# ekimb/rust-mdbg

Measured on AMD Instinct MI355X. Metric: Gbases/s ingested to k-min-mer graph, higher is better.
Workload: dtype u64

## Files before the change

### include/mdbg_hip.h

```cpp
#ifndef MDBG_HIP_H
#define MDBG_HIP_H

#include <stddef.h>
#include <stdint.h>

#ifdef __cplusplus
extern "C" {
#endif

#define MDBG_ABI_VERSION 3

enum {
    MDBG_OK = 0,
    MDBG_E_PARAM = -1,
    MDBG_E_ALPHABET = -2,
    MDBG_E_CAPACITY = -3,
    MDBG_E_DEVICE = -4,
    MDBG_E_NOMEM = -5,
    MDBG_E_STATE = -6,
    MDBG_E_IO = -7
};

#define MDBG_MAX_L 255u
#define MDBG_MAX_MINABUND 65535u
#define MDBG_FLAG_FORCE_GENERIC 1u
#define MDBG_FLAG_KEEP_READS 2u
#define MDBG_SCHEME_DENSITY 0u
#define MDBG_SCHEME_SYNCMERS 1u

typedef struct mdbg_ctx mdbg_ctx;

typedef struct mdbg_params {
    uint32_t k;
    uint32_t l;
    double density;
    uint32_t min_abundance;
    uint32_t reads_already_hpc;
    int32_t device;
    uint32_t flags;
    uint64_t table_capacity_hint;
    uint32_t scheme;
    uint32_t syncmer_s;
    uint64_t reserved[3];
} mdbg_params;

typedef struct mdbg_nodes {
    uint64_t n;
    uint32_t k;
    const uint64_t* keys;
    const uint32_t* index;
    const uint16_t* abundance;
    const uint32_t* seqlen;
    const uint16_t* shift;
    const uint64_t* shift_full;
    const uint64_t* src_read;
    const uint64_t* src_start;
    const uint64_t* src_end;
    const uint8_t* reversed;
    uint64_t n_distinct;
    uint64_t n_wrapped;
} mdbg_nodes;

typedef struct mdbg_stats {
    uint64_t n_reads, n_bases, n_minimizers, n_windows, n_distinct, table_capacity;
    uint64_t n_slow_tiles;
    uint64_t n_tiles;
    double ms_sketch, ms_insert, ms_finalize;
    double ms_sketch_tile;
    uint64_t n_sketch_tile_launches;
    uint64_t n_sketch_tile_bases;
    uint64_t tile_bases;
    uint64_t n_link_matches;
    uint64_t reserved[3];
} mdbg_stats;

mdbg_ctx* mdbg_create(const mdbg_params* p, int* err);
void mdbg_destroy(mdbg_ctx* ctx);

int mdbg_ingest_batch(mdbg_ctx* ctx, const uint8_t* bases, const uint64_t* offsets, uint64_t n_reads,
                      uint64_t first_read_ordinal);
int mdbg_ingest_batch_device(mdbg_ctx* ctx, const uint8_t* d_bases, const uint64_t* d_offsets, uint64_t n_reads,
                             uint64_t n_bases, uint64_t first_read_ordinal);

typedef struct mdbg_packed_batch {
    const uint64_t* words;
    const uint64_t* offsets;
    uint64_t n_reads;
    const uint64_t* exc_pos;
    const uint8_t* exc_val;
    uint64_t n_exc;
} mdbg_packed_batch;
int mdbg_ingest_batch_packed(mdbg_ctx* ctx, const mdbg_packed_batch* batch, uint64_t first_read_ordinal);
int mdbg_ingest_batch_packed_device(mdbg_ctx* ctx, const mdbg_packed_batch* batch, uint64_t n_bases, uint64_t first_read_ordinal);
int mdbg_sketch_packed_device(mdbg_ctx* ctx, const mdbg_packed_batch* batch, uint64_t n_bases, uint64_t first_read_ordinal);
int mdbg_pack_device(mdbg_ctx* ctx, const uint8_t* d_bases, uint64_t n_bases, uint64_t* d_words, uint64_t* d_exc_pos,
                     uint8_t* d_exc_val, uint64_t exc_cap, uint64_t* n_exc);

int mdbg_sketch_only(mdbg_ctx* ctx, const uint8_t* bases, const uint64_t* offsets, uint64_t n_reads,
                     const uint64_t** hashes, const uint64_t** positions, const uint64_t** per_read_offsets,
                     uint64_t* n_minimizers);

int mdbg_query_batch(mdbg_ctx* ctx, const uint8_t* bases, const uint64_t* offsets, uint64_t n_reads, const uint32_t** counts,
                     const uint64_t** per_read_offsets, uint64_t* n_windows);

int mdbg_finalize(mdbg_ctx* ctx, mdbg_nodes* out);
int mdbg_finalize_device(mdbg_ctx* ctx, mdbg_nodes* out);
int mdbg_finalize_gfa(mdbg_ctx* ctx, mdbg_nodes* out);
int mdbg_nodes_digest(mdbg_ctx* ctx, const mdbg_nodes* nodes, uint64_t* sum, uint64_t* xr);
int mdbg_reset(mdbg_ctx* ctx, uint32_t new_k);
int mdbg_set_lmer_filter(mdbg_ctx* ctx, const uint64_t* codes, uint64_t n);
int mdbg_mark(mdbg_ctx* ctx, uint64_t* mark);
int mdbg_rewind(mdbg_ctx* ctx, uint64_t mark);

int mdbg_get_stats(mdbg_ctx* ctx, mdbg_stats* out);
int mdbg_set_timing(mdbg_ctx* ctx, uint32_t level);
const char* mdbg_strerror(int err);
const char* mdbg_last_error(mdbg_ctx* ctx);
uint32_t mdbg_abi_version(void);
uint32_t mdbg_build_flags(void);
uint64_t mdbg_release_cached_memory(void);
void* mdbg_host_alloc(size_t bytes);
void mdbg_host_free(void* p);
int mdbg_host_is_pinned(const void* p);

int mdbg_sketch_device(mdbg_ctx* ctx, const uint8_t* d_bases, const uint64_t* d_offsets, uint64_t n_reads,
                       uint64_t n_bases, uint64_t first_read_ordinal);
int mdbg_insert_resident(mdbg_ctx* ctx);
int mdbg_route_pack(mdbg_ctx* ctx, uint32_t world, const uint64_t** d_records, uint64_t* counts);
int mdbg_arena_reserve(mdbg_ctx* ctx, uint64_t n_records, uint64_t** d_tail);
int mdbg_insert_records(mdbg_ctx* ctx, const uint64_t* d_records, uint64_t n_records);
typedef struct mdbg_routed_lists {
    uint64_t n_all, n_solid;
    const uint64_t* d_first; const uint8_t* d_solid;
    const uint64_t* d_ath; const uint32_t* d_count; const uint64_t* d_slot; const uint64_t* d_idx_all;
    uint64_t counts_all[64], counts_solid[64];
} mdbg_routed_lists;
int mdbg_routed_export(mdbg_ctx* ctx, uint32_t world, const uint64_t* span_lo, const uint32_t* span_rank, uint32_t n_spans,
                       mdbg_routed_lists* out);
int mdbg_resolve_first(mdbg_ctx* ctx, const uint64_t* d_ord, const uint8_t* d_solid, uint64_t n, uint64_t* d_rank_first,
                       uint64_t* d_rank_solid, uint64_t* total_first, uint64_t* total_solid);
int mdbg_resolve_meta(mdbg_ctx* ctx, const uint64_t* d_ord, uint64_t n, uint64_t* d_meta);
int mdbg_routed_keys(mdbg_ctx* ctx, const uint64_t* d_slot, uint64_t n, uint64_t* d_keys);
typedef struct mdbg_edge_list {
    uint64_t n;
    const uint32_t* n1; const uint8_t* o1; const uint32_t* n2; const uint8_t* o2; const uint32_t* overlap;
    uint64_t presimp_removed;
} mdbg_edge_list;
int mdbg_graph_edges(mdbg_ctx* ctx, float presimp, mdbg_edge_list* out);
int mdbg_graph_edges_device(mdbg_ctx* ctx, float presimp, mdbg_edge_list* out);

typedef struct mdbg_unitig_list {
    uint64_t n_unitigs, n_entries;
    const uint64_t* offsets;
    const uint32_t* node; const uint8_t* ori;
    const uint64_t* src_read; const uint64_t* src_begin; const uint32_t* len; const uint8_t* revcomp; const uint64_t* dst_offset;
    const uint64_t* length; const uint64_t* kc_sum; const uint8_t* circular;
    mdbg_edge_list edges;
    uint32_t n_rounds, reserved;
} mdbg_unitig_list;
int mdbg_graph_unitigs(mdbg_ctx* ctx, mdbg_unitig_list* out);
int mdbg_graph_unitigs_device(mdbg_ctx* ctx, mdbg_unitig_list* out);

#define MDBG_SIMPLIFY_TIPS 1u
#define MDBG_SIMPLIFY_BUBBLES 2u
typedef struct mdbg_simplify_step { uint32_t kind, max_nodes; uint64_t max_bases; } mdbg_simplify_step;
typedef struct mdbg_simplify_stats {
    uint32_t n_steps, n_compactions;
    const uint64_t* unitigs_removed; const uint64_t* nodes_removed;
    uint64_t total_unitigs_removed, total_nodes_removed;
    uint32_t n_rounds_total, n_syncs;
} mdbg_simplify_stats;
int mdbg_graph_simplify(mdbg_ctx* ctx, const mdbg_simplify_step* steps, uint32_t n_steps, mdbg_unitig_list* out, mdbg_simplify_stats* stats);
int mdbg_graph_simplify_device(mdbg_ctx* ctx, const mdbg_simplify_step* steps, uint32_t n_steps, mdbg_unitig_list* out, mdbg_simplify_stats* stats);

typedef struct mdbg_contig_seqs {
    uint64_t n_contigs, n_bases;
    const uint8_t*  bases;
    const uint64_t* offsets;
    const uint64_t* unitig;
} mdbg_contig_seqs;
int mdbg_graph_contigs(mdbg_ctx* ctx, uint64_t min_len, mdbg_contig_seqs* out);
int mdbg_graph_contigs_device(mdbg_ctx* ctx, uint64_t min_len, mdbg_contig_seqs* out);
int mdbg_kept_reads(mdbg_ctx* ctx, uint64_t* n_reads, uint64_t* n_bases, uint64_t* bytes);
int mdbg_contigs_ms(mdbg_ctx* ctx, double* ms);

int mdbg_set_partition(mdbg_ctx* ctx, uint32_t world, uint32_t rank);
typedef struct mdbg_sketch_store {
    uint64_t n_minimizers, n_reads;
    const uint64_t* d_hashes;
    const uint32_t* d_positions;
    const uint64_t* d_read_offsets;
} mdbg_sketch_store;
int mdbg_sketch_view(mdbg_ctx* ctx, mdbg_sketch_store* out);
int mdbg_ingest_sketch(mdbg_ctx* ctx, const uint64_t* d_hashes, const uint32_t* d_positions, const uint64_t* d_read_offsets,
                       uint64_t n_reads, uint64_t first_read_ordinal);
int mdbg_store_reserve(mdbg_ctx* ctx, uint64_t n_minimizers_total, uint64_t n_reads_total);
int mdbg_sketch_reserve(mdbg_ctx* ctx, uint64_t n_minimizers, uint64_t** d_hashes, uint32_t** d_positions, uint64_t* region);
int mdbg_sketch_commit(mdbg_ctx* ctx, uint64_t region, uint64_t n_minimizers, const uint64_t* d_read_offsets, uint64_t n_reads,
                       uint64_t first_read_ordinal, uint64_t owned_windows);
int mdbg_owner_counts(mdbg_ctx* ctx, uint32_t world, uint64_t* counts);
int mdbg_owner_lists(mdbg_ctx* ctx, uint32_t world, uint64_t* counts, const uint32_t** d_lists);
int mdbg_sketch_commit_listed(mdbg_ctx* ctx, uint64_t region, uint64_t n_minimizers, const uint64_t* d_read_offsets, uint64_t n_reads,
                              uint64_t first_read_ordinal, const uint32_t* d_list, uint64_t n_list);
typedef struct mdbg_batch_info {
    uint64_t store_offset, n_minimizers, first_slot, n_reads, first_read_ordinal;
    const uint64_t* d_hashes;
    const uint32_t* d_positions;
    const uint64_t* d_read_offsets;
} mdbg_batch_info;
int mdbg_last_batch(mdbg_ctx* ctx, mdbg_batch_info* out);
int mdbg_finalize_begin(mdbg_ctx* ctx, uint64_t** d_bm_first, uint64_t** d_bm_solid, uint64_t* n_words);
int mdbg_finalize_end(mdbg_ctx* ctx, mdbg_nodes* out, const uint64_t** d_row, uint64_t* n_nodes_global);

int mdbg_sync(mdbg_ctx* ctx);
int mdbg_copy_to_host(mdbg_ctx* ctx, void* dst, const void* d_src, uint64_t nbytes);
int mdbg_copy_to_device(mdbg_ctx* ctx, void* d_dst, const void* src, uint64_t nbytes);

typedef struct mdbg_synth_params {
    uint64_t seed;
    uint64_t genome_len;
    uint64_t n_reads;
    uint32_t mean_len, sd_len, min_len, max_len;
    uint32_t err_ppm;
    uint32_t reserved;
} mdbg_synth_params;
int mdbg_synth_reads_device(mdbg_ctx* ctx, const mdbg_synth_params* sp, uint64_t first_read,
// ... 9 lines not shown
```

### rust_mdbg_amd/api.py

```python
import ctypes as C
import os

import numpy as np

_HERE = os.path.dirname(os.path.abspath(__file__))
_LIB = None

MDBG_OK, MDBG_E_PARAM, MDBG_E_ALPHABET, MDBG_E_CAPACITY, MDBG_E_DEVICE, MDBG_E_NOMEM, MDBG_E_STATE, MDBG_E_IO = 0, -1, -2, -3, -4, -5, -6, -7
FLAG_FORCE_GENERIC = 1
FLAG_KEEP_READS = 2


class MdbgError(RuntimeError):
    def __init__(self, code, msg):
        super().__init__("mdbg error %d: %s" % (code, msg))
        self.code = code


class Params(C.Structure):
    _fields_ = [("k", C.c_uint32), ("l", C.c_uint32), ("density", C.c_double), ("min_abundance", C.c_uint32),
                ("reads_already_hpc", C.c_uint32), ("device", C.c_int32), ("flags", C.c_uint32),
                ("table_capacity_hint", C.c_uint64), ("scheme", C.c_uint32), ("syncmer_s", C.c_uint32), ("reserved", C.c_uint64 * 3)]


class Nodes(C.Structure):
    _fields_ = [("n", C.c_uint64), ("k", C.c_uint32), ("keys", C.POINTER(C.c_uint64)), ("index", C.POINTER(C.c_uint32)),
                ("abundance", C.POINTER(C.c_uint16)), ("seqlen", C.POINTER(C.c_uint32)), ("shift", C.POINTER(C.c_uint16)),
                ("shift_full", C.POINTER(C.c_uint64)), ("src_read", C.POINTER(C.c_uint64)), ("src_start", C.POINTER(C.c_uint64)),
                ("src_end", C.POINTER(C.c_uint64)), ("reversed", C.POINTER(C.c_uint8)), ("n_distinct", C.c_uint64),
                ("n_wrapped", C.c_uint64)]


class Stats(C.Structure):
    _fields_ = [("n_reads", C.c_uint64), ("n_bases", C.c_uint64), ("n_minimizers", C.c_uint64), ("n_windows", C.c_uint64),
                ("n_distinct", C.c_uint64), ("table_capacity", C.c_uint64), ("n_slow_tiles", C.c_uint64), ("n_tiles", C.c_uint64),
                ("ms_sketch", C.c_double), ("ms_insert", C.c_double), ("ms_finalize", C.c_double), ("ms_sketch_tile", C.c_double),
                ("n_sketch_tile_launches", C.c_uint64), ("n_sketch_tile_bases", C.c_uint64), ("tile_bases", C.c_uint64),
                ("n_link_matches", C.c_uint64), ("reserved", C.c_uint64 * 3)]


class RoutedLists(C.Structure):
    _fields_ = [("n_all", C.c_uint64), ("n_solid", C.c_uint64), ("d_first", C.c_void_p), ("d_solid", C.c_void_p), ("d_ath", C.c_void_p),
                ("d_count", C.c_void_p), ("d_slot", C.c_void_p), ("d_idx_all", C.c_void_p), ("counts_all", C.c_uint64 * 64),
                ("counts_solid", C.c_uint64 * 64)]


class SketchStore(C.Structure):
    _fields_ = [("n_minimizers", C.c_uint64), ("n_reads", C.c_uint64), ("d_hashes", C.c_void_p), ("d_positions", C.c_void_p),
                ("d_read_offsets", C.c_void_p)]


class BatchInfo(C.Structure):
    _fields_ = [("store_offset", C.c_uint64), ("n_minimizers", C.c_uint64), ("first_slot", C.c_uint64), ("n_reads", C.c_uint64),
                ("first_read_ordinal", C.c_uint64), ("d_hashes", C.c_void_p), ("d_positions", C.c_void_p), ("d_read_offsets", C.c_void_p)]


class EdgeList(C.Structure):
    _fields_ = [("n", C.c_uint64), ("n1", C.POINTER(C.c_uint32)), ("o1", C.POINTER(C.c_uint8)), ("n2", C.POINTER(C.c_uint32)),
                ("o2", C.POINTER(C.c_uint8)), ("overlap", C.POINTER(C.c_uint32)), ("presimp_removed", C.c_uint64)]


class UnitigList(C.Structure):
    _fields_ = [("n_unitigs", C.c_uint64), ("n_entries", C.c_uint64), ("offsets", C.POINTER(C.c_uint64)), ("node", C.POINTER(C.c_uint32)),
                ("ori", C.POINTER(C.c_uint8)), ("src_read", C.POINTER(C.c_uint64)), ("src_begin", C.POINTER(C.c_uint64)), ("len", C.POINTER(C.c_uint32)),
                ("revcomp", C.POINTER(C.c_uint8)), ("dst_offset", C.POINTER(C.c_uint64)), ("length", C.POINTER(C.c_uint64)),
                ("kc_sum", C.POINTER(C.c_uint64)), ("circular", C.POINTER(C.c_uint8)), ("edges", EdgeList), ("n_rounds", C.c_uint32),
                ("reserved", C.c_uint32)]


UNITIG_FIELDS = (("offsets", np.uint64), ("node", np.uint32), ("ori", np.uint8), ("src_read", np.uint64), ("src_begin", np.uint64), ("len", np.uint32),
                 ("revcomp", np.uint8), ("dst_offset", np.uint64), ("length", np.uint64), ("kc_sum", np.uint64), ("circular", np.uint8))
EDGE_FIELDS = (("n1", np.uint32), ("o1", np.uint8), ("n2", np.uint32), ("o2", np.uint8), ("overlap", np.uint32))


def unitig_counts(u):
    nu, ne = int(u.n_unitigs), int(u.n_entries)
    return dict(offsets=nu + 1 if nu else 0, node=ne, ori=ne, src_read=ne, src_begin=ne, len=ne, revcomp=ne, dst_offset=ne, length=nu, kc_sum=nu, circular=nu)


class ContigSeqs(C.Structure):
    _fields_ = [("n_contigs", C.c_uint64), ("n_bases", C.c_uint64), ("bases", C.POINTER(C.c_uint8)), ("offsets", C.POINTER(C.c_uint64)),
                ("unitig", C.POINTER(C.c_uint64))]


class SimplifyStep(C.Structure):
    _fields_ = [("kind", C.c_uint32), ("max_nodes", C.c_uint32), ("max_bases", C.c_uint64)]


class SimplifyStats(C.Structure):
    _fields_ = [("n_steps", C.c_uint32), ("n_compactions", C.c_uint32), ("unitigs_removed", C.POINTER(C.c_uint64)), ("nodes_removed", C.POINTER(C.c_uint64)),
                ("total_unitigs_removed", C.c_uint64), ("total_nodes_removed", C.c_uint64), ("n_rounds_total", C.c_uint32), ("n_syncs", C.c_uint32)]


MDBG_SIMPLIFY_TIPS, MDBG_SIMPLIFY_BUBBLES = 1, 2
_T, _B = (MDBG_SIMPLIFY_TIPS, 10, 50000), (MDBG_SIMPLIFY_BUBBLES, 0, 100000)
MAGIC_SIMPLIFY_STEPS = [_T, _T, _B, _B, _T, _B, _B, _B, _T, _B, _T, (MDBG_SIMPLIFY_BUBBLES, 0, 1000000), (MDBG_SIMPLIFY_TIPS, 10, 150000),
                        (MDBG_SIMPLIFY_BUBBLES, 0, 1000000)]


def simplify_steps(steps):
    steps = [tuple(int(x) for x in s) for s in steps]
    if not steps:
        return None, 0
    return (SimplifyStep * len(steps))(*[SimplifyStep(k, mn, mb) for k, mn, mb in steps]), len(steps)


def unitig_name(i, circular):
    return "utg%07d%s" % (i + 1, "c" if circular else "l")


class PackedBatch(C.Structure):
    _fields_ = [("words", C.c_void_p), ("offsets", C.c_void_p), ("n_reads", C.c_uint64), ("exc_pos", C.c_void_p),
                ("exc_val", C.c_void_p), ("n_exc", C.c_uint64)]


class SynthParams(C.Structure):
    _fields_ = [("seed", C.c_uint64), ("genome_len", C.c_uint64), ("n_reads", C.c_uint64), ("mean_len", C.c_uint32),
                ("sd_len", C.c_uint32), ("min_len", C.c_uint32), ("max_len", C.c_uint32), ("err_ppm", C.c_uint32),
                ("reserved", C.c_uint32)]


EXPORTS = ["mdbg_abi_version", "mdbg_build_flags", "mdbg_create", "mdbg_destroy", "mdbg_finalize_device", "mdbg_finalize_gfa", "mdbg_nodes_digest", "mdbg_set_timing", "mdbg_ingest_batch", "mdbg_ingest_batch_device", "mdbg_sketch_only",
           "mdbg_finalize", "mdbg_reset", "mdbg_get_stats", "mdbg_strerror", "mdbg_last_error", "mdbg_sketch_device",
           "mdbg_insert_resident", "mdbg_route_pack", "mdbg_insert_records", "mdbg_sync", "mdbg_synth_reads_device", "mdbg_copy_to_host", "mdbg_copy_to_device",
           "mdbg_routed_export", "mdbg_resolve_first", "mdbg_resolve_meta", "mdbg_routed_keys", "mdbg_arena_reserve",
           "mdbg_set_partition", "mdbg_sketch_view", "mdbg_ingest_sketch", "mdbg_finalize_begin", "mdbg_finalize_end",
           "mdbg_store_reserve", "mdbg_sketch_reserve", "mdbg_sketch_commit", "mdbg_last_batch", "mdbg_owner_counts", "mdbg_graph_edges", "mdbg_graph_edges_device", "mdbg_graph_unitigs", "mdbg_graph_unitigs_device",
           "mdbg_graph_simplify", "mdbg_graph_simplify_device", "mdbg_graph_contigs", "mdbg_graph_contigs_device", "mdbg_kept_reads", "mdbg_contigs_ms",
           "mdbg_ingest_batch_packed", "mdbg_ingest_batch_packed_device", "mdbg_sketch_packed_device", "mdbg_pack_device", "mdbg_query_batch", "mdbg_owner_lists", "mdbg_sketch_commit_listed", "mdbg_mark", "mdbg_rewind", "mdbg_set_lmer_filter",
           "mdbg_release_cached_memory", "mdbg_host_alloc", "mdbg_host_free", "mdbg_host_is_pinned", "mdbg_dbg_segments_ms"]


def lib_path():
    return os.path.join(_HERE, "libmdbg_hip.so")


def load_library():
    global _LIB
    if _LIB is not None:
        return _LIB
    p = lib_path()
    if not os.path.exists(p):
        raise ImportError("libmdbg_hip.so not built (%s); run `make -C rust_mdbg_amd/csrc`" % p)
    import sys
    if "torch" not in sys.modules and not os.environ.get("MDBG_NO_TORCH_PRELOAD"):
        import importlib.util
        if importlib.util.find_spec("torch") is not None:
            import torch
    L = C.CDLL(p)
    vp, u64, u32 = C.c_void_p, C.c_uint64, C.c_uint32
    L.mdbg_abi_version.restype = u32
    L.mdbg_build_flags.restype = u32
    L.mdbg_release_cached_memory.restype = u64
    L.mdbg_host_alloc.restype = vp
    L.mdbg_host_alloc.argtypes = [C.c_size_t]
    L.mdbg_host_free.restype = None
    L.mdbg_host_free.argtypes = [vp]
    L.mdbg_host_is_pinned.argtypes = [vp]
    L.mdbg_create.restype = vp
    L.mdbg_create.argtypes = [C.POINTER(Params), C.POINTER(C.c_int)]
    L.mdbg_destroy.restype = None
    L.mdbg_destroy.argtypes = [vp]
    L.mdbg_ingest_batch.argtypes = [vp, vp, vp, u64, u64]
    L.mdbg_ingest_batch_device.argtypes = [vp, vp, vp, u64, u64, u64]
    L.mdbg_sketch_device.argtypes = [vp, vp, vp, u64, u64, u64]
    L.mdbg_insert_resident.argtypes = [vp]
    L.mdbg_ingest_batch_packed.argtypes = [vp, C.POINTER(PackedBatch), u64]
    L.mdbg_ingest_batch_packed_device.argtypes = [vp, C.POINTER(PackedBatch), u64, u64]
    L.mdbg_sketch_packed_device.argtypes = [vp, C.POINTER(PackedBatch), u64, u64]
    L.mdbg_pack_device.argtypes = [vp, vp, u64, vp, vp, vp, u64, C.POINTER(u64)]
    L.mdbg_query_batch.argtypes = [vp, vp, vp, u64, C.POINTER(C.POINTER(u32)), C.POINTER(C.POINTER(u64)), C.POINTER(u64)]
    L.mdbg_query_batch.restype = C.c_int
    L.mdbg_sketch_only.argtypes = [vp, vp, vp, u64, C.POINTER(C.POINTER(u64)), C.POINTER(C.POINTER(u64)), C.POINTER(C.POINTER(u64)), C.POINTER(u64)]
    L.mdbg_finalize.argtypes = [vp, C.POINTER(Nodes)]
    L.mdbg_finalize_device.argtypes = [vp, C.POINTER(Nodes)]
    L.mdbg_finalize_gfa.argtypes = [vp, C.POINTER(Nodes)]
    L.mdbg_set_timing.argtypes = [vp, u32]
    L.mdbg_nodes_digest.argtypes = [vp, C.POINTER(Nodes), C.POINTER(C.c_uint64), C.POINTER(C.c_uint64)]
    L.mdbg_reset.argtypes = [vp, u32]
    L.mdbg_get_stats.argtypes = [vp, C.POINTER(Stats)]
    L.mdbg_strerror.restype = C.c_char_p
    L.mdbg_strerror.argtypes = [C.c_int]
    L.mdbg_last_error.restype = C.c_char_p
    L.mdbg_last_error.argtypes = [vp]
    L.mdbg_route_pack.argtypes = [vp, u32, C.POINTER(vp), C.POINTER(u64)]
    L.mdbg_routed_export.argtypes = [vp, u32, vp, vp, u32, C.POINTER(RoutedLists)]
    L.mdbg_resolve_first.argtypes = [vp, vp, vp, u64, vp, vp, C.POINTER(u64), C.POINTER(u64)]
    L.mdbg_resolve_meta.argtypes = [vp, vp, u64, vp]
    L.mdbg_routed_keys.argtypes = [vp, vp, u64, vp]
    L.mdbg_arena_reserve.argtypes = [vp, u64, C.POINTER(vp)]
    L.mdbg_set_partition.argtypes = [vp, u32, u32]
# ... 389 lines not shown
```

### rust_mdbg_amd/csrc/context.inc

```
namespace {
struct KeptReads {
    void* blk = nullptr; size_t cap = 0; void* xblk = nullptr; size_t xcap = 0;
    u64 n_reads = 0, n_bases = 0, n_words = 0, n_exc = 0;
    KeptReads() = default; KeptReads(const KeptReads&) = delete; KeptReads& operator=(const KeptReads&) = delete;
    ~KeptReads() { if (blk) mdbg_block_free(blk, cap); if (xblk) mdbg_block_free(xblk, xcap); }
    uint2* planes() const { return (uint2*)blk; }
    u64* offsets() const { return (u64*)blk + n_words; }
    u64* exc_pos() const { return (u64*)xblk; }
    u8* exc_val() const { return (u8*)xblk + n_exc * 8; }
    u64 bytes() const { return n_words * 8 + (n_reads + 1) * 8 + n_exc * 9; }
};
struct Batch { u64 first_ordinal; u32 n_reads; u32 slot0; u64 m0, m1; u64 owned = ~0ull;
               u64 list_off = ~0ull;
               bool mread_ok = true;
               u32 src_rank = ~0u;
               u64 n_bases = 0;
               bool partial = false;
               std::shared_ptr<KeptReads> kept; };

enum { SH_DISTINCT = 0, SH_OWNED, SH_OWNINS, SH_FIN_WRAPPED, SH_FIN_DISTINCT, N_SHARD_ARRAYS };
enum { SC_CARRY = 0, SC_NDISTINCT, SC_NWINDOWS, SC_FIN0, SC_FIN1, SC_FIN2, SC_SLOWCOUNT , SC_ERRFLAG , SC_CAPERR , SC_SLOWTOTAL, SC_BATCHWIN, SC_IMPORTERR, SC_PROBEERR , SC_OWNINS, SC_OVERMAX , SC_TOTFIRST, SC_TOTSOLID, SC_SLICEFAIL, SC_DONE , SC_N };

}

struct Stage { DevBuf bases, off, exc_pos, exc_val; hipStream_t st = nullptr; bool busy = false; };

struct mdbg_ctx {
    std::recursive_mutex mu;
    std::mutex err_mu;
    Stage stage[2]; std::mutex stage_mu; std::condition_variable stage_cv;
    mdbg_params P{};
    int dev = 0; hipStream_t stream = nullptr; std::string err; int poisoned = 0;
    u64 scal_seq = 0; bool batchwin_zero = false;
    u64* h_scal = nullptr;
    u64 bound = 0; DevBuf d_t4;
    DevBuf mh, mpos, mread, roff; u64 M = 0; u64 mcap = 0; u32 n_slots = 0;
    u64 slot_end_m = 0;
    u64 pending_m = 0;
    std::vector<Batch> batches; size_t batches_inserted = 0;
    u64 h_known = 0;
    DevBuf bread, tile_recs, slab, n_valid, n_scan, last_read, tile_base, scan_tmp, gran_sum, tile_flags, scalars, phase_dbg, shards;
    u32 slab_cap_min = 0;
    DevBuf tab, mx; u64 cap = 0;
    DevBuf arena, route_out, route_tmp, route_h, route_f; u64 n_records = 0; bool routed = false;
    DevBuf by_maps;
    DevBuf link_ctr;
    DevBuf claim;
    bool claims_ok = false;
    DevBuf bm_first, bm_solid, pre_first, pre_solid, popc_tmp, bt_dev, fin_out, solid_list, fin_order;
    DevBuf bm_local, pre_local, pre_local2;
    HostRaw<u64> h_keys, h_shift_full, h_src_read, h_src_start, h_src_end; HostRaw<u32> h_index, h_seqlen; HostRaw<u16> h_abund, h_shift; HostRaw<u8> h_rev;
    std::vector<u64> so_hash, so_pos, so_off;
    std::vector<u32> q_counts; std::vector<u64> q_off; DevBuf q_dev;
    DevBuf syn_bases, syn_off, syn_lens;
    u64 n_reads = 0, n_bases = 0, n_windows = 0, n_distinct = 0, n_slow_tiles = 0, n_tiles = 0;
    double ms_sketch = 0, ms_insert = 0, ms_finalize = 0;
    hipEvent_t ev0 = nullptr, ev1 = nullptr, ev3 = nullptr;
    bool fin_dirty = false;
    int timing = 2;
    std::vector<u8> bt_sent; const void* bt_sent_at = nullptr;
    u32 own_world = 1, own_rank = 0;
    int (*before_emit)(void* self, FinArgs& F, u64 n_solid) = nullptr; void* before_emit_self = nullptr;
    FinArgs finF{}; u64 fin_words = 0, fin_bits = 0; bool fin_open = false;
    u64 fin_rows_guess = 0;
    std::vector<u8> bt_host;
    EdgeBuffers* eb = nullptr;
    DevBuf own_hist;
    DevBuf own_lists; u64 own_lists_n = 0;
    DevBuf listed_multi; std::vector<ListedBatch> listed_multi_host;
    DevBuf own_thr; u32 thr_world = 0, thr_k = 0; double thr_bound = 0;
    DevBuf ol_cnt, ol_off, ol_tot, ol_list, ol_owner;
    DevBuf lmer_set; u64 lmer_mask = 0; bool lmer_on = false; u32 lmer_all_ones = 0;
    DevBuf w_jstar, w_count, w_ctr, w_start, w_fill, w_occ, w_sorted, w_ath;
    u64 nodes_n = 0; bool nodes_ok = false;
    HostRaw<u32> he_n1, he_n2, he_ov; HostRaw<u8> he_o1, he_o2;
    EdgeResult last_edges{}; bool edges_ok = false;
    UnitigBuffers* ub = nullptr;
    HostRaw<u64> hu_off, hu_sread, hu_sbegin, hu_dst, hu_length, hu_kc; HostRaw<u32> hu_node, hu_len, hu_n1, hu_n2, hu_ov; HostRaw<u8> hu_ori, hu_rc, hu_circ, hu_o1, hu_o2;
    std::vector<u64> hs_unitigs, hs_nodes;
    UnitigResult last_ul{}; bool ulist_ok = false;
    ContigBuffers* cb = nullptr;
    DevBuf kp_exc_pos, kp_exc_val, kp_cnt;
    HostRaw<u8> hc_bases; HostRaw<u64> hc_off, hc_unitig;
    double ms_stitch = 0;
    std::vector<hipEvent_t> tile_ev; size_t tile_ev_used = 0; double ms_tile = 0; u64 n_tile_launches = 0, n_tile_bases = 0;
};

namespace {

int fail(mdbg_ctx* c, int code, const char* what, hipError_t e = hipSuccess) {
    char buf[512];
    if (e != hipSuccess) { snprintf(buf, sizeof buf, "%s: %s", what, hipGetErrorString(e)); (void)hipGetLastError(); }
    else snprintf(buf, sizeof buf, "%s", what);
    if (c) { std::lock_guard<std::mutex> g_(c->err_mu); c->err = buf; if (code == MDBG_E_DEVICE || code == MDBG_E_ALPHABET || code == MDBG_E_NOMEM) c->poisoned = code; }
    return code;
}
#define MDBG_LOCK(c) std::lock_guard<std::recursive_mutex> lock_((c)->mu)
#define HIPCHK(c, call) do { hipError_t e_ = (call); if (e_ != hipSuccess) return fail((c), e_ == hipErrorOutOfMemory ? MDBG_E_NOMEM : MDBG_E_DEVICE, #call, e_); } while (0)
template <class T> int copy_out(mdbg_ctx* c, HostRaw<T>& h, const T* dev, size_t n, const char* what, const T** host) {
    if (!h.resize(n)) return fail(c, MDBG_E_NOMEM, what);
    if (n) { const hipError_t e = hipMemcpy(h.data(), dev, n * sizeof(T), hipMemcpyDeviceToHost); if (e != hipSuccess) return fail(c, e == hipErrorOutOfMemory ? MDBG_E_NOMEM : MDBG_E_DEVICE, what, e); }
    *host = h.data();
    return MDBG_OK;
}

u64* scal(mdbg_ctx* c) { return c->scalars.as<u64>(); }
int read_scalars(mdbg_ctx* c, u64* host, bool with_fin = false, bool zero_batchwin = false) {
    if (!c->h_scal) { HIPCHK(c, hipHostMalloc((void**)&c->h_scal, (SC_N + 1) * 8, hipHostMallocMapped)); c->h_scal[SC_N] = 0; }
    const u64 seq = ++c->scal_seq;
    PublishArgs pa{};
    pa.shards[0] = c->shards.as<u64>() + SH_DISTINCT * CTR_SHARDS; pa.idx[0] = SC_NDISTINCT; pa.n_arrays = 1;
    pa.zero_mask = 0; pa.zero_arrays = 0;
    if (with_fin) {
        pa.shards[1] = c->shards.as<u64>() + SH_FIN_WRAPPED * CTR_SHARDS; pa.idx[1] = SC_FIN1; pa.shards[2] = c->shards.as<u64>() + SH_FIN_DISTINCT * CTR_SHARDS; pa.idx[2] = SC_FIN2; pa.n_arrays = 3;
        pa.zero_mask = (1ull << SC_FIN0) | (1ull << SC_FIN1) | (1ull << SC_FIN2); pa.zero_arrays = 0x6u;
    }
    pa.scalars = scal(c); pa.n = SC_N; pa.host = c->h_scal; pa.seq = seq; pa.zero_idx = zero_batchwin ? (u32)SC_BATCHWIN : (u32)SC_N;
    c->batchwin_zero = zero_batchwin;
    launch_publish_scalars(pa, c->stream);
    volatile u64* const flag = c->h_scal + SC_N;
    bool seen = false;
    const double t0 = now_ms();
    for (u32 spins = 0; !seen; ++spins) {
        seen = __atomic_load_n(flag, __ATOMIC_ACQUIRE) == seq;
        if (seen) break;
#if defined(__x86_64__)
        __builtin_ia32_pause();
#endif
        if ((spins & 0x3FFu) != 0x3FFu) continue;
        const double waited = now_ms() - t0;
        if (waited > 0.3) std::this_thread::yield();
        if (waited > 20.0) break;
        if ((spins & 0xFFFFu) == 0xFFFFu) { const hipError_t q = hipStreamQuery(c->stream); if (q != hipErrorNotReady) break; }
    }
    if (!seen) HIPCHK(c, hipStreamSynchronize(c->stream));
    memcpy(host, c->h_scal, SC_N * 8);
    if (with_fin) c->fin_dirty = false;
    return MDBG_OK;
}
int write_scalar(mdbg_ctx* c, int idx, u64 v) {
    HIPCHK(c, hipMemcpyAsync((u64*)c->scalars.p + idx, &v, 8, hipMemcpyHostToDevice, c->stream));
    HIPCHK(c, hipStreamSynchronize(c->stream));
    return MDBG_OK;
}

enum ResultsFrom { FROM_NODES, FROM_EDGES, FROM_UNITIGS };
void invalidate_results(mdbg_ctx* c, ResultsFrom from) { if (from <= FROM_NODES) c->nodes_ok = false; if (from <= FROM_EDGES) c->edges_ok = false; c->ulist_ok = false; }
static void fill_mread_of(mdbg_ctx* c, Batch& b);
double owner_hash_bound(const mdbg_ctx* c) {
    double b;
    if (c->P.scheme == MDBG_SCHEME_SYNCMERS) { b = c->P.density * ldexp(1.0, 2 * (int)c->P.l); if (b >= 18446744073709551616.0) b = 18446744073709551615.0; }
    else b = (double)c->bound;
    return b >= 1.0 ? b : 0.0;
}
const u64* owner_thr(mdbg_ctx* c, u32 world) {
    if (world <= 1) return nullptr;
    const double b = owner_hash_bound(c);
    if (!(b >= 1.0)) return nullptr;
    if (c->thr_world != world || c->thr_k != c->P.k || c->thr_bound != b) {
        if (c->own_thr.ensure((size_t)OWNER_PARAM_WORDS * 8, 0, c->stream) != hipSuccess) return nullptr;
        launch_owner_thresholds(b, c->P.k, world, c->own_thr.as<u64>(), c->stream);
        c->thr_world = world; c->thr_k = c->P.k; c->thr_bound = b;
    }
    return c->own_thr.as<u64>();
}
u64 owner_bin_mul(const mdbg_ctx* c) {
    const double b = owner_hash_bound(c);
    if (!(b >= (double)OWNER_BINS * 4.0)) return 0;
    u64 bi = b >= 18446744073709549568.0 ? ~0ull : (u64)b;
    const unsigned __int128 q = ((unsigned __int128)OWNER_BINS << 64) / ((unsigned __int128)bi + 1);
    return q > (unsigned __int128)~0ull ? 0 : (u64)q;
}
int owner_hist_batch(mdbg_ctx* c, size_t which, u64* d_hist) {
    const u64 mul = owner_bin_mul(c);
    if (!mul || c->batches.empty()) return MDBG_OK;
    Batch& b = which == ~(size_t)0 ? c->batches.back() : c->batches[which];
    fill_mread_of(c, b);
    launch_owner_bins(c->mh.as<u64>(), c->mread.as<u32>(), c->roff.as<u64>(), b.m0, b.m1, c->P.k, mul, d_hist, c->stream);
    return MDBG_OK;
}
int owner_set_table(mdbg_ctx* c, u32 world, const u8* tab) {
    const u64 mul = owner_bin_mul(c);
    if (!mul || !owner_thr(c, world)) return MDBG_OK;
    HIPCHK(c, hipMemcpyAsync(c->own_thr.as<u64>() + OWNER_TAB_AT, tab, OWNER_BINS, hipMemcpyHostToDevice, c->stream));
    HIPCHK(c, hipMemcpyAsync(c->own_thr.as<u64>(), &mul, 8, hipMemcpyHostToDevice, c->stream));
    HIPCHK(c, hipStreamSynchronize(c->stream));
    return MDBG_OK;
}
TableArgs table_args(mdbg_ctx* c) {
    TableArgs T;
    T.tab = c->tab.as<Slot>(); T.cap = c->cap; T.mx = c->mx.as<u64>(); T.A = cascade_of(c->P.min_abundance);
    T.n_distinct = c->shards.as<u64>() + SH_DISTINCT * CTR_SHARDS;
    T.ks.mh = c->mh.as<u64>(); T.ks.arena = c->arena.as<u64>(); T.ks.k = c->P.k;
    T.own_world = c->own_world; T.own_rank = c->own_rank; T.own_thr = owner_thr(c, c->own_world);
    T.probe_err = (u32*)(scal(c) + SC_PROBEERR); T.own_inserted = c->shards.as<u64>() + SH_OWNINS * CTR_SHARDS;
    T.claim = (!c->routed && c->claims_ok) ? c->claim.as<u8>() : nullptr;
    static const bool no_chain = getenv("MDBG_NO_CHAIN") != nullptr;
    T.no_chain = no_chain ? 1u : 0u;
    static const bool weak_fp = getenv("MDBG_WEAK_FP") != nullptr;
    T.fp_mask = weak_fp ? 0x3ull : 0x3FFFFFFFull;
    static const bool count_links = getenv("MDBG_COUNT_LINKS") != nullptr;
    T.link_ctr = nullptr;
    if (count_links) {
        if (!c->link_ctr.p && c->link_ctr.ensure(8, 0, c->stream) == hipSuccess) (void)hipMemsetAsync(c->link_ctr.p, 0, 8, c->stream);
        T.link_ctr = (unsigned long long*)c->link_ctr.p;
    }
    return T;
}

u64 slots_for(u64 n) { return n + n / 2 + 1024; }

int table_reserve(mdbg_ctx* c, u64 incoming) {
    u64 need = slots_for(c->n_distinct + incoming);
    const u32 A = cascade_of(c->P.min_abundance);
    if (c->cap == 0) {
        u64 want = need;
        if (c->P.table_capacity_hint) want = std::max(want, slots_for(c->P.table_capacity_hint));
        HIPCHK(c, c->tab.ensure(want * sizeof(Slot), 0, c->stream));
        if (A > 2) HIPCHK(c, c->mx.ensure(want * (A - 2) * 8, 0, c->stream));
        c->cap = want;
        launch_clear_table(c->tab.as<Slot>(), c->cap, c->mx.as<u64>(), A > 2 ? c->cap * (A - 2) : 0, c->stream);
        c->claims_ok = !c->routed && c->claim.p != nullptr;
        return MDBG_OK;
    }
    if (need <= c->cap) return MDBG_OK;
    need = std::max(need, 2 * c->cap);
    DevBuf ntab, nmx;
    HIPCHK(c, ntab.ensure(need * sizeof(Slot), 0, c->stream));
    if (A > 2) HIPCHK(c, nmx.ensure(need * (A - 2) * 8, 0, c->stream));
    launch_clear_table(ntab.as<Slot>(), need, nmx.as<u64>(), A > 2 ? need * (A - 2) : 0, c->stream);
    TableArgs T = table_args(c);
    T.tab = ntab.as<Slot>(); T.cap = need; T.mx = nmx.as<u64>();
    launch_rehash(c->tab.as<Slot>(), c->cap, c->mx.as<u64>(), T, c->stream);
    HIPCHK(c, hipStreamSynchronize(c->stream));
    std::swap(c->tab.p, ntab.p); std::swap(c->tab.cap, ntab.cap);
    std::swap(c->mx.p, nmx.p); std::swap(c->mx.cap, nmx.cap);
    c->cap = need;
    return MDBG_OK;
}

int clear_table(mdbg_ctx* c) {
    invalidate_results(c, FROM_NODES);
    ZeroList z{};
    z.p[0] = c->shards.as<u64>() + SH_DISTINCT * CTR_SHARDS; z.n[0] = CTR_SHARDS; z.p[1] = scal(c) + SC_NDISTINCT; z.n[1] = 2;
    z.p[2] = scal(c) + SC_IMPORTERR; z.n[2] = 1; z.p[3] = scal(c) + SC_PROBEERR; z.n[3] = 1;
    if (c->cap) launch_clear_table(c->tab.as<Slot>(), c->cap, c->mx.as<u64>(), cascade_of(c->P.min_abundance) > 2 ? c->cap * (cascade_of(c->P.min_abundance) - 2) : 0, c->stream, &z);
    else launch_zero_regions(z, c->stream);
    c->n_distinct = 0; c->n_windows = 0; c->batches_inserted = 0; c->n_records = 0; c->routed = false;
    c->claims_ok = c->claim.p != nullptr;
    return MDBG_OK;
}

#define STAGE_EVENT(c, ev, s) do { if ((c)->timing >= 2) HIPCHK((c), hipEventRecord((ev), (s))); } while (0)
hipEvent_t next_tile_event(mdbg_ctx* c) {
    if (c->timing < 1) return nullptr;
    if (c->tile_ev_used == c->tile_ev.size()) { hipEvent_t e = nullptr; if (hipEventCreate(&e) != hipSuccess) return nullptr; c->tile_ev.push_back(e); }
    return c->tile_ev[c->tile_ev_used++];
}
void collect_tile_events(mdbg_ctx* c) {
    for (size_t i = 0; i + 1 < c->tile_ev_used; i += 2) {
        float ms = 0;
        if (hipEventElapsedTime(&ms, c->tile_ev[i], c->tile_ev[i + 1]) == hipSuccess) c->ms_tile += ms;
        else (void)hipGetLastError();
    }
    c->tile_ev_used = 0;
}
float ev_ms(mdbg_ctx* c) {
    float ms = 0;
    if (c->timing < 2) return 0.0f;
    (void)hipEventSynchronize(c->ev1);
    if (hipEventElapsedTime(&ms, c->ev0, c->ev1) != hipSuccess) { (void)hipGetLastError(); ms = 0; }
    return ms;
}

int check_params(const mdbg_params* p) {
    if (!p) return MDBG_E_PARAM;
    if (p->k < 2 || p->k > 4096) return MDBG_E_PARAM;
    if (p->l < 2 || p->l > MDBG_MAX_L) return MDBG_E_PARAM;
    if (p->min_abundance < 1 || p->min_abundance > MDBG_MAX_MINABUND) return MDBG_E_PARAM;
    if (!(p->density == p->density)) return MDBG_E_PARAM;
    if (p->scheme > MDBG_SCHEME_SYNCMERS) return MDBG_E_PARAM;
    if (p->scheme == MDBG_SCHEME_SYNCMERS && (p->l > 31 || p->syncmer_s > 16 || p->syncmer_s > p->l || p->l - p->syncmer_s + 1 > 32)) return MDBG_E_PARAM;
    return MDBG_OK;
}
}

extern "C" {
uint32_t mdbg_abi_version(void) { return MDBG_ABI_VERSION; }
uint32_t mdbg_build_flags(void) { return 0; }

const char* mdbg_strerror(int err) {
    switch (err) {
        case MDBG_OK: return "ok";
        case MDBG_E_PARAM: return "invalid parameter";
        case MDBG_E_ALPHABET: return "Non-ACGTN nucleotide encountered";
        case MDBG_E_CAPACITY: return "capacity limit exceeded";
        case MDBG_E_DEVICE: return "HIP device error";
        case MDBG_E_NOMEM: return "out of memory";
        case MDBG_E_STATE: return "invalid state for this call";
        case MDBG_E_IO: return "file could not be opened or written";
        default: return "unknown error";
    }
}
const char* mdbg_last_error(mdbg_ctx* ctx) { return ctx ? ctx->err.c_str() : ""; }

mdbg_ctx* mdbg_create(const mdbg_params* p, int* err) {
    int e = check_params(p);
    if (e) { if (err) *err = e; return nullptr; }
    int ndev = 0;
    if (hipGetDeviceCount(&ndev) != hipSuccess || ndev == 0) { if (err) *err = MDBG_E_DEVICE; return nullptr; }
    mdbg_ctx* c = new mdbg_ctx();
    c->P = *p;
    auto bail = [&](int code) -> mdbg_ctx* { if (err) *err = code; mdbg_destroy(c); return nullptr; };
    if (p->device >= 0) { if (hipSetDevice(p->device) != hipSuccess) return bail(MDBG_E_DEVICE); c->dev = p->device; }
    else if (hipGetDevice(&c->dev) != hipSuccess) return bail(MDBG_E_DEVICE);
    if (hipStreamCreateWithFlags(&c->stream, hipStreamNonBlocking) != hipSuccess) return bail(MDBG_E_DEVICE);
    for (auto& g : c->stage) if (hipStreamCreateWithFlags(&g.st, hipStreamNonBlocking) != hipSuccess) return bail(MDBG_E_DEVICE);
    if (hipEventCreate(&c->ev0) != hipSuccess || hipEventCreate(&c->ev1) != hipSuccess) return bail(MDBG_E_DEVICE);
    c->bound = make_hash_bound(p->density);
    if (c->d_t4.ensure((2 << (2 * BS_GS)) * 8, 0, c->stream) != hipSuccess) return bail(MDBG_E_NOMEM);
    { u64 t4[2 << (2 * BS_GS)]; bs_make_table<BS_GS>(t4); if (hipMemcpy(c->d_t4.p, t4, sizeof t4, hipMemcpyHostToDevice) != hipSuccess) return bail(MDBG_E_DEVICE); }
    if (c->scalars.ensure(SC_N * 8, 0, c->stream) != hipSuccess) return bail(MDBG_E_NOMEM);
    if (c->shards.ensure(N_SHARD_ARRAYS * CTR_SHARDS * 8, 0, c->stream) != hipSuccess) return bail(MDBG_E_NOMEM);
    if (hipMemset(c->shards.p, 0, N_SHARD_ARRAYS * CTR_SHARDS * 8) != hipSuccess) return bail(MDBG_E_DEVICE);
    if (hipMemset(c->scalars.p, 0, SC_N * 8) != hipSuccess) return bail(MDBG_E_DEVICE);
    if (c->roff.ensure(1024, 0, c->stream) != hipSuccess) return bail(MDBG_E_NOMEM);
    if (hipMemset(c->roff.p, 0, 8) != hipSuccess) return bail(MDBG_E_DEVICE);
    if (err) *err = MDBG_OK;
    return c;
}

void mdbg_destroy(mdbg_ctx* c) {
    if (!c) return;
    (void)hipSetDevice(c->dev);
    if (c->stream) (void)hipStreamSynchronize(c->stream);
    if (c->ev3) (void)hipEventDestroy(c->ev3);
    if (c->ev0) (void)hipEventDestroy(c->ev0);
    if (c->ev1) (void)hipEventDestroy(c->ev1);
    for (auto e : c->tile_ev) (void)hipEventDestroy(e);
    if (c->eb) edge_buffers_destroy(c->eb);
    if (c->ub) unitig_buffers_destroy(c->ub);
    if (c->cb) contig_buffers_destroy(c->cb);
    if (c->h_scal) (void)hipHostFree(c->h_scal);
    for (auto& g : c->stage) if (g.st) (void)hipStreamDestroy(g.st);
    if (c->stream) (void)hipStreamDestroy(c->stream);
    delete c;
}

int mdbg_sync(mdbg_ctx* c) {
    if (!c) return MDBG_E_PARAM;
    MDBG_LOCK(c);
    HIPCHK(c, hipStreamSynchronize(c->stream));
    return MDBG_OK;
}

int mdbg_copy_to_host(mdbg_ctx* c, void* dst, const void* d_src, uint64_t nbytes) {
    if (!c || (nbytes && (!dst || !d_src))) return MDBG_E_PARAM;
    MDBG_LOCK(c);
    (void)hipSetDevice(c->dev);
    HIPCHK(c, hipStreamSynchronize(c->stream));
    if (nbytes) HIPCHK(c, hipMemcpy(dst, d_src, nbytes, hipMemcpyDeviceToHost));
    return MDBG_OK;
}
int mdbg_copy_to_device(mdbg_ctx* c, void* d_dst, const void* src, uint64_t nbytes) {
    if (!c || (nbytes && (!d_dst || !src))) return MDBG_E_PARAM;
    MDBG_LOCK(c);
    (void)hipSetDevice(c->dev);
    if (nbytes) HIPCHK(c, hipMemcpy(d_dst, src, nbytes, hipMemcpyHostToDevice));
    return MDBG_OK;
}
}
```

### rust_mdbg_amd/csrc/ingest_api.inc

```
namespace {
constexpr u64 SLAB_BUDGET = 6ull << 30;
int insert_resident_impl(mdbg_ctx* c, bool allow_pending = false);
int sketch_device_impl(mdbg_ctx* c, const SketchInput& in, const u64* d_offsets, u64 n_reads, u64 n_bases, u64 first_ordinal, bool then_insert = false, bool* inserted = nullptr) {
    if (inserted) *inserted = false;
    if (c->poisoned) return fail(c, MDBG_E_STATE, "context is in an error state");
    if (n_reads == 0) return MDBG_OK;
    if (in.fmt == FMT_ASCII && !in.d_bases && n_bases) return fail(c, MDBG_E_PARAM, "null bases");
    if (in.fmt == FMT_PLANES && !in.d_planes && n_bases) return fail(c, MDBG_E_PARAM, "null packed words");
    if (!d_offsets) return fail(c, MDBG_E_PARAM, "null offsets");
    if ((((uintptr_t)in.d_bases) | ((uintptr_t)in.d_planes)) & 15) return fail(c, MDBG_E_PARAM, "device bases pointer must be 16-byte aligned");
    if (in.n_exc && (!in.d_exc_pos || !in.d_exc_val)) return fail(c, MDBG_E_PARAM, "null exception list");
    if (in.n_exc >= 0xFFFFFFF0ull) return fail(c, MDBG_E_CAPACITY, "too many exceptions");
    if (n_reads >= 0xFFFFFFF0ull || (u64)c->n_slots + n_reads >= 0xFFFFFFF0ull) return fail(c, MDBG_E_CAPACITY, "too many reads");
    if (first_ordinal + n_reads >= (1ull << (64 - WIN_BITS))) return fail(c, MDBG_E_CAPACITY, "read ordinal too large");
    hipStream_t s = c->stream;
    const bool sync = c->P.scheme == MDBG_SCHEME_SYNCMERS;
    const u64 tile_bases = TILE_STRIDE;
    const u64 n_tiles_total = (n_bases + tile_bases - 1) / tile_bases;
    if (n_tiles_total >= 0x7FFFFFF0ull) return fail(c, MDBG_E_CAPACITY, "batch too large for one call");
    u32 slot0 = 0;
    { int e = next_slot0(c, c->M, n_reads, &slot0); if (e) return e; }
    double dens2 = 2.0 * c->P.density; if (dens2 > 1.0) dens2 = 1.0; if (dens2 < 0) dens2 = 0;
    u32 slab_cap = 0, gather_tiles = 1;
    {
        const double per_base = sync ? std::min(1.0, std::max(0.0, c->P.density)) / (c->P.syncmer_s ? std::max(1.0, (double)(c->P.l - c->P.syncmer_s + 1) / 2.0) : 1.0) : dens2;
        const double e = (double)tile_bases * per_base; double v = e * 1.25 + 6.0 * sqrt(e) + 32.0; if (v > (double)tile_bases) v = (double)tile_bases; slab_cap = ((u32)v + 7u) & ~7u;
        if (e < 128.0) gather_tiles = (u32)std::max(1.0, std::min(16.0, 256.0 / std::max(e, 1.0)));
    }
    if (slab_cap < c->slab_cap_min) slab_cap = c->slab_cap_min;
    static const u32 cap0_hook = getenv("MDBG_SLAB_CAP0") ? (u32)atoi(getenv("MDBG_SLAB_CAP0")) : 0u;
    static const u64 budget_hook = getenv("MDBG_SLAB_BUDGET_MB") ? (u64)atoll(getenv("MDBG_SLAB_BUDGET_MB")) << 20 : 0ull;
    if (cap0_hook && !c->slab_cap_min) slab_cap = std::max<u32>(8u, cap0_hook & ~7u);
    if (slab_cap > (u32)tile_bases) slab_cap = (u32)tile_bases;
    if (n_tiles_total) {
        HIPCHK(c, c->bread.ensure((n_tiles_total + 2) * 4, 0, s));
        HIPCHK(c, c->tile_recs.ensure(n_tiles_total * sizeof(TileRec), 0, s));
        HIPCHK(c, c->n_valid.ensure(n_tiles_total * 4, 0, s));
        HIPCHK(c, c->n_scan.ensure(n_tiles_total * 4, 0, s));
        HIPCHK(c, c->last_read.ensure(n_tiles_total * 4, 0, s));
        if (in.n_exc) HIPCHK(c, c->tile_flags.ensure(n_tiles_total, 0, s));
    }
    u64 want = c->M + (u64)((double)n_bases * dens2 * 1.15) + 65536;
    const bool phase_dbg = getenv("MDBG_PHASE_TIMING") != nullptr;
    for (int attempt = 0; attempt < 4; ++attempt) {
        { int e = store_ensure(c, want); if (e) return e; }
        const u64 chunk = std::max<u64>(1, std::min<u64>(n_tiles_total ? n_tiles_total : 1, (budget_hook ? budget_hook : SLAB_BUDGET) / ((u64)slab_cap * sizeof(Rec))));
        std::vector<u64> part_end;
        for (u64 t0 = 0; t0 < n_tiles_total; t0 += chunk) part_end.push_back(std::min<u64>(n_tiles_total, t0 + chunk));
        u64 max_part = 0; { u64 t0 = 0; for (u64 e : part_end) { max_part = std::max(max_part, e - t0); t0 = e; } }
        if (n_tiles_total) {
            HIPCHK(c, c->slab.ensure((size_t)chunk * slab_cap * sizeof(Rec), 0, s));
            HIPCHK(c, c->tile_base.ensure((size_t)max_part * 8, 0, s));
            HIPCHK(c, c->scan_tmp.ensure(((size_t)max_part / 1024 + 2) * 8, 0, s));
        }
        u64 init[1] = {c->M};
        STAGE_EVENT(c, c->ev0, s);
        SketchInit init0{};
        init0.zero[0] = scal(c) + SC_ERRFLAG; init0.zero[1] = scal(c) + SC_SLOWTOTAL; init0.zero[2] = scal(c) + SC_OVERMAX; init0.set_p = scal(c) + SC_CARRY; init0.set_v = c->M;
        const bool fused = then_insert && inserted && n_tiles_total && part_end.size() == 1 && !phase_dbg && c->cap && c->own_world <= 1 && !c->lmer_on && !c->routed && !c->pending_m &&
                           c->batches_inserted == c->batches.size() && c->mcap > c->M && c->mcap - c->M <= 2 * (want - c->M) + (1u << 20) &&
                           want - c->M <= (48ull << 20);
        if (fused) init0.zero[3] = scal(c) + SC_BATCHWIN;
        if (!n_tiles_total) {
            ZeroList z{};
            z.p[0] = init0.zero[0]; z.n[0] = 1; z.p[1] = init0.zero[1]; z.n[1] = 1; z.p[2] = init0.zero[2]; z.n[2] = 1; z.set_p = init0.set_p; z.set_v = init0.set_v;
            launch_zero_regions(z, s);
            launch_fill_u64(c->roff.as<u64>() + slot0, n_reads + 1, c->M, s);
        }
        SketchArgs A{};
        A.bases = in.d_bases; A.planes = in.d_planes; A.fmt = in.fmt; A.n_bases = n_bases; A.offsets = d_offsets; A.n_reads = (u32)n_reads;
        A.exc_pos = in.d_exc_pos; A.exc_val = in.d_exc_val; A.n_exc = (u32)in.n_exc;
        A.l = c->P.l; A.hpc = c->P.reads_already_hpc == 0 ? 1u : 0u;
        if (n_tiles_total) {
            A.bread = c->bread.as<u32>(); A.recs = c->tile_recs.as<TileRec>(); A.n_tiles = (u32)n_tiles_total;
            A.slab = c->slab.as<Rec>(); A.slab_cap = slab_cap; A.n_valid = c->n_valid.as<u32>(); A.n_scan = c->n_scan.as<u32>(); A.last_read = c->last_read.as<u32>(); A.over_max = (u32*)(scal(c) + SC_OVERMAX);
            A.t4 = c->d_t4.as<u64>();
            A.tile_flags = in.n_exc ? c->tile_flags.as<u8>() : nullptr;
            A.err_flag = (u32*)(scal(c) + SC_ERRFLAG); A.slow_total = (unsigned long long*)(scal(c) + SC_SLOWTOTAL);
            A.read_base = slot0; A.bound = c->bound; A.btop = (u32)(c->bound >> (64 - BS_B)); A.force_slow = ((c->P.flags & 1u) || c->P.l > (u32)BS_MAX_L) ? 1u : 0u;
            A.dbg = nullptr;
            { const char* sp = getenv("MDBG_STOP_PHASE"); A.stop_phase = sp ? (u32)atoi(sp) : 0u; }
            if (phase_dbg) { HIPCHK(c, c->phase_dbg.ensure((size_t)n_tiles_total * 128, 0, s)); HIPCHK(c, hipMemsetAsync(c->phase_dbg.p, 0, (size_t)n_tiles_total * 128, s)); A.dbg = c->phase_dbg.as<u64>(); }
            const u32 n_gran = (u32)((max_part + SCAN_GRAN - 1) / SCAN_GRAN);
            HIPCHK(c, c->gran_sum.ensure((size_t)n_gran * 8 + 64, 0, s));
            A.block_sum = (unsigned long long*)c->gran_sum.as<u64>();
            init0.zero_arr = c->gran_sum.as<u64>(); init0.zero_arr_n = n_gran;
            launch_bread(d_offsets, (u32)n_reads, n_bases, A.n_tiles, c->bread.as<u32>(), c->tile_recs.as<TileRec>(), init0, s);
            if (in.n_exc) {
                HIPCHK(c, hipMemsetAsync(c->tile_flags.p, 0, n_tiles_total, s));
                launch_tile_flags(in.d_exc_pos, (u32)in.n_exc, A.n_tiles, c->tile_flags.as<u8>(), s);
            }
            if (sync) {
                A.scheme = 1; A.s = c->P.syncmer_s; A.btop = 0;
                const double v = c->P.density * (double)(1ull << (2 * c->P.l));
                A.bound = !(v > 0.0) ? 0 : (v >= 18446744073709551616.0 ? ~0ull : (u64)v);
                A.force_slow = ((c->P.flags & 1u) || c->P.syncmer_s > 13) ? 1u : 0u;
            }
            u64 t0 = 0;
            for (size_t pi = 0; pi < part_end.size(); ++pi) {
                const u32 nt = (u32)(part_end[pi] - t0);
                Rec* const part_slab = c->slab.as<Rec>();
                A.tile0 = (u32)t0; A.slab = part_slab;
                if (pi) HIPCHK(c, hipMemsetAsync(c->gran_sum.p, 0, (size_t)n_gran * 8, s));
                { hipEvent_t tb = next_tile_event(c), te = next_tile_event(c); launch_sketch(A, nt, s, tb, te); }
                GatherArgs G{};
                G.tile0 = (u32)t0; G.n = nt; G.slab = part_slab; G.slab_cap = slab_cap; G.n_valid = A.n_valid; G.n_scan = A.n_scan; G.last_read = A.last_read;
                G.out_hash = c->mh.as<u64>(); G.out_pos = c->mpos.as<u32>(); G.out_read = c->mread.as<u32>(); G.out_cap = c->mcap;
                G.m0 = c->M; G.slot0 = slot0; G.n_reads = (u32)n_reads; G.off = c->roff.as<u64>(); G.last_launch = pi + 1 == part_end.size() ? 1u : 0u;
                G.tiles_per_wave = gather_tiles;
                launch_gather(G, c->scan_tmp.as<u64>(), c->tile_base.as<u64>(), scal(c) + SC_CARRY, s, c->gran_sum.as<u64>());
                c->n_tile_launches += 1;
                t0 = part_end[pi];
            }
            c->n_tile_bases += n_bases;
            if (phase_dbg) {
                std::vector<u64> h((size_t)A.n_tiles * 16);
                (void)hipStreamSynchronize(s);
                (void)hipMemcpy(h.data(), A.dbg, h.size() * 8, hipMemcpyDeviceToHost);
                double ph[7] = {0, 0, 0, 0, 0, 0, 0}, nc = 0, nv = 0; u64 nfast = 0;
                for (u32 t = 0; t < A.n_tiles; ++t) {
                    const u64* q = &h[(size_t)t * 16];
                    if (!q[7]) continue;
                    ++nfast;
                    ph[0] += (double)(q[1] - q[0]); ph[1] += (double)(q[2] - q[1]); ph[2] += (double)(q[3] - q[2]); ph[3] += (double)(q[4] - q[3]);
                    ph[4] += (double)(q[5] - q[4]); ph[5] += (double)(q[7] - q[5]);
                    nc += (double)q[9]; nv += (double)q[10];
                }
                const double n = nfast ? (double)nfast : 1.0;
                fprintf(stderr, "[mdbg phase timing] tiles=%u fast=%llu avg cycles: load=%.0f compact=%.0f hash=%.0f exact=%.0f rank=%.0f write=%.0f ; candidates=%.1f valid=%.1f slab_cap=%u\n",
                        A.n_tiles, (unsigned long long)nfast, ph[0] / n, ph[1] / n, ph[2] / n, ph[3] / n, ph[4] / n, ph[5] / n, nc / n, nv / n, slab_cap);
            }
        }
        STAGE_EVENT(c, c->ev1, s);
        u32* const ins_flags = (u32*)(scal(c) + SC_CAPERR);
        if (fused) {
            launch_count_reserve(c->roff.as<u64>(), slot0, (u32)n_reads, c->P.k, scal(c) + SC_BATCHWIN, (u32*)(scal(c) + SC_DONE), c->shards.as<u64>() + SH_DISTINCT * CTR_SHARDS, scal(c) + SC_NDISTINCT,
                                 c->cap, ins_flags + 1, scal(c) + SC_CARRY, c->mcap, (const u32*)(scal(c) + SC_OVERMAX), s);
            if (!c->ev3) HIPCHK(c, hipEventCreate(&c->ev3));
            launch_insert_windows(table_args(c), c->mh.as<u64>(), c->mread.as<u32>(), c->roff.as<u64>(), c->M, c->mcap, slot0, first_ordinal, scal(c) + SC_NWINDOWS, ins_flags, s, scal(c) + SC_CARRY);
            STAGE_EVENT(c, c->ev3, s);
        }
        u64 sc[SC_N];
        int e = read_scalars(c, sc, false, true); if (e) return e;
        c->ms_sketch += ev_ms(c);
        collect_tile_events(c);
        u64 m_new = sc[SC_CARRY];
        const u32 over = (u32)sc[SC_OVERMAX];
        if (over || m_new > c->mcap) {
            if (over) { slab_cap = std::min<u32>((u32)tile_bases, (over + over / 8 + 15u) & ~7u); c->slab_cap_min = slab_cap; }
            if (m_new > c->mcap) want = m_new + 65536;
            c->n_tile_launches -= part_end.size(); c->n_tile_bases -= n_tiles_total ? n_bases : 0;
            continue;
        }
        if (m_new >= 0xFFFFFFF0ull) return fail(c, MDBG_E_CAPACITY, "more than 2^32 minimizers resident on one device");
        if ((u32)sc[SC_ERRFLAG]) {
            u64 which = ~0ull;
            HIPCHK(c, hipMemcpyAsync(scal(c) + SC_SLOWTOTAL, &which, 8, hipMemcpyHostToDevice, s));
            launch_alphabet_rule(A, (unsigned long long*)(scal(c) + SC_SLOWTOTAL), s);
            HIPCHK(c, hipMemcpyAsync(&which, scal(c) + SC_SLOWTOTAL, 8, hipMemcpyDeviceToHost, s));
            HIPCHK(c, hipStreamSynchronize(s));
            if (which != ~0ull) {
                char buf[160]; snprintf(buf, sizeof buf, "Non-ACGTN nucleotide in read %llu of the batch (ordinal %llu)", (unsigned long long)which, (unsigned long long)(first_ordinal + which));
                return fail(c, MDBG_E_ALPHABET, buf);
            }
        }
        const u64 slow_total = sc[SC_SLOWTOTAL];
        if (c->lmer_on && m_new > c->M) {
            const u32 nb = lmer_filter_blocks(m_new - c->M);
            HIPCHK(c, c->slab.ensure((size_t)nb * 256 * sizeof(Rec), 0, s));
            HIPCHK(c, c->n_valid.ensure((size_t)nb * 4, 0, s)); HIPCHK(c, c->tile_base.ensure((size_t)nb * 8, 0, s)); HIPCHK(c, c->scan_tmp.ensure(((size_t)nb / 1024 + 2) * 8, 0, s));
            LmerFilterArgs L{};
            L.set = c->lmer_set.as<u64>(); L.set_mask = c->lmer_mask; L.has_all_ones = c->lmer_all_ones;
            L.mh = c->mh.as<u64>(); L.mpos = c->mpos.as<u32>(); L.mread = c->mread.as<u32>(); L.m0 = c->M; L.m1 = m_new;
            L.offsets = d_offsets; L.slot0 = slot0; L.l = c->P.l; L.hpc = c->P.reads_already_hpc == 0 ? 1u : 0u;
            L.slab = c->slab.as<Rec>(); L.n_valid = c->n_valid.as<u32>();
            launch_lmer_filter(L, in.fmt, in.d_bases, in.d_planes, in.d_exc_pos, in.d_exc_val, (u32)in.n_exc, s);
            HIPCHK(c, hipMemcpyAsync(scal(c) + SC_CARRY, init, 8, hipMemcpyHostToDevice, s));
            GatherArgs G{};
            G.tile0 = 0; G.n = nb; G.slab = L.slab; G.slab_cap = 256; G.n_valid = L.n_valid;
            G.out_hash = c->mh.as<u64>(); G.out_pos = c->mpos.as<u32>(); G.out_read = c->mread.as<u32>(); G.out_cap = c->mcap;
            G.m0 = c->M; G.slot0 = slot0; G.n_reads = (u32)n_reads; G.off = c->roff.as<u64>(); G.last_launch = 1; G.tiles_per_wave = 1;
            launch_gather(G, c->scan_tmp.as<u64>(), c->tile_base.as<u64>(), scal(c) + SC_CARRY, s);
            int e2 = read_scalars(c, sc); if (e2) return e2;
            m_new = sc[SC_CARRY];
        }
        Batch b; b.first_ordinal = first_ordinal; b.n_reads = (u32)n_reads; b.slot0 = slot0; b.m0 = c->M; b.m1 = m_new; b.n_bases = n_bases;
        invalidate_results(c, FROM_UNITIGS);
        if (c->P.flags & MDBG_FLAG_KEEP_READS) { int ke = keep_batch(c, in, d_offsets, n_reads, n_bases, b.kept); if (ke) return ke; }
        store_append(c, b);
        c->n_reads += n_reads; c->n_bases += n_bases; c->n_tiles += n_tiles_total; c->n_slow_tiles += slow_total;
        if (fused) {
            invalidate_results(c, FROM_NODES);
            if (sc[SC_CAPERR] >> 32) return MDBG_OK;
            c->batches_inserted = c->batches.size();
            *inserted = true;
            if ((u32)sc[SC_PROBEERR]) return fail(c, MDBG_E_PARAM, "the table filled up during insertion");
            float ms = 0;
            if (c->timing >= 2) { if (hipEventElapsedTime(&ms, c->ev1, c->ev3) == hipSuccess) c->ms_insert += ms; else (void)hipGetLastError(); }
            c->n_windows += sc[SC_BATCHWIN];
            c->n_distinct = sc[SC_NDISTINCT];
            if (sc[SC_IMPORTERR]) return fail(c, MDBG_E_PARAM, "read offsets of an imported sketch are not consistent with its size");
            if ((u32)sc[SC_CAPERR]) return fail(c, MDBG_E_CAPACITY, "a read has more than 2^26 minimizers");
        }
        return MDBG_OK;
    }
    return fail(c, MDBG_E_CAPACITY, "minimizer store could not be sized");
}
int sketch_device_impl(mdbg_ctx* c, const u8* d_bases, const u64* d_offsets, u64 n_reads, u64 n_bases, u64 first_ordinal, bool then_insert = false, bool* inserted = nullptr) {
    SketchInput in; in.fmt = FMT_ASCII; in.d_bases = d_bases;
    return sketch_device_impl(c, in, d_offsets, n_reads, n_bases, first_ordinal, then_insert, inserted);
}

int insert_resident_impl(mdbg_ctx* c, bool allow_pending) {
    if (c->poisoned) return fail(c, MDBG_E_STATE, "context is in an error state");
    if (c->routed) return fail(c, MDBG_E_STATE, "table holds routed records; local insertion is not allowed");
    if (c->pending_m && !allow_pending) return fail(c, MDBG_E_STATE, "reserved sketch regions have not been committed");
    hipStream_t s = c->stream;
    const size_t first = c->batches_inserted, last = c->batches.size();
    invalidate_results(c, FROM_NODES);
    bool any = false;
    for (size_t i = first; i < last; ++i) any = any || c->batches[i].m1 > c->batches[i].m0;
    c->batches_inserted = last;
    if (!any) return MDBG_OK;
    u64 sc[SC_N];
    bool counts_known = c->own_world > 1;
    u64 known = 0;
    for (size_t i = first; i < last; ++i) { const Batch& b = c->batches[i]; if (b.m1 == b.m0) continue; if (b.owned == ~0ull) counts_known = false; else known += b.owned; }
    for (size_t i = first; i < last; ++i) {
        Batch& b = c->batches[i];
        if (!counts_known || !(b.list_off != ~0ull && b.owned != ~0ull && c->own_world > 1)) fill_mread_of(c, b);
    }
    if (counts_known) {
        c->h_known = known;
        HIPCHK(c, hipMemcpyAsync(scal(c) + SC_BATCHWIN, &c->h_known, 8, hipMemcpyHostToDevice, s));
        HIPCHK(c, hipMemsetAsync(c->shards.as<u64>() + SH_OWNINS * CTR_SHARDS, 0, CTR_SHARDS * 8, s));
    } else {
        if (!c->batchwin_zero) HIPCHK(c, hipMemsetAsync(scal(c) + SC_BATCHWIN, 0, 8, s));
        if (c->own_world > 1) HIPCHK(c, hipMemsetAsync(c->shards.as<u64>() + SH_OWNED * CTR_SHARDS, 0, 2 * CTR_SHARDS * 8, s));
        for (size_t i = first; i < last; ++i) {
            const Batch& b = c->batches[i];
            if (b.m1 == b.m0) continue;
            if (c->own_world > 1)
                launch_count_owned_windows(c->mh.as<u64>(), c->mread.as<u32>(), c->roff.as<u64>(), b.m0, b.m1, c->P.k, c->own_world, owner_thr(c, c->own_world), c->own_rank,
                                           c->shards.as<u64>() + SH_OWNED * CTR_SHARDS, s);
            else launch_count_windows(c->roff.as<u64>(), b.slot0, b.n_reads, c->P.k, scal(c) + SC_BATCHWIN, s);
        }
        if (c->own_world > 1) launch_sum_shards(c->shards.as<u64>() + SH_OWNED * CTR_SHARDS, 1, scal(c) + SC_BATCHWIN, s);
    }
    c->batchwin_zero = false;
    int e;
    u32* const flags = (u32*)(scal(c) + SC_CAPERR);
    u64 total_idx = 0;
    for (size_t i = first; i < last; ++i) total_idx += c->batches[i].m1 - c->batches[i].m0;
    u64 slice = 32ull << 20;
    { const char* sv = getenv("MDBG_INSERT_SLICE"); if (sv) { const u64 v = strtoull(sv, nullptr, 10); if (v) slice = std::max<u64>(v, (u64)OWN_SPAN); } }
    slice = (slice + OWN_SPAN - 1) / OWN_SPAN * OWN_SPAN;
    if (c->own_world <= 1 && total_idx > 2 * slice) {
        struct Sl { size_t b; u64 a, hi; };
        std::vector<Sl> sl;
        for (size_t i = first; i < last; ++i) { const Batch& b = c->batches[i]; for (u64 a = b.m0; a < b.m1; a += slice) sl.push_back({i, a, std::min(a + slice, b.m1)}); }
        if (c->cap < slots_for(c->n_distinct + slice)) { e = table_reserve(c, slice); if (e) return e; }
        size_t next = 0;
        for (;;) {
            { ZeroList z{}; z.p[0] = scal(c) + SC_CAPERR; z.n[0] = 0; z.set_p = scal(c) + SC_SLICEFAIL; z.set_v = ~0ull; launch_zero_regions(z, s); }
            HIPCHK(c, hipMemsetAsync(flags + 1, 0, 4, s));
            STAGE_EVENT(c, c->ev0, s);
            for (size_t j = next; j < sl.size(); ++j) {
                const Batch& b = c->batches[sl[j].b];
                launch_slice_check(c->shards.as<u64>(), scal(c) + SC_NDISTINCT, sl[j].hi - sl[j].a, c->cap, flags + 1, scal(c) + SC_SLICEFAIL, (u64)j, s);
                launch_insert_windows(table_args(c), c->mh.as<u64>(), c->mread.as<u32>(), c->roff.as<u64>(), sl[j].a, b.m1, b.slot0, b.first_ordinal,
                                      scal(c) + SC_NWINDOWS, flags, s, nullptr, sl[j].hi - sl[j].a);
            }
            STAGE_EVENT(c, c->ev1, s);
            e = read_scalars(c, sc); if (e) return e;
            c->ms_insert += ev_ms(c);
            c->n_distinct = sc[SC_NDISTINCT];
            if (!(sc[SC_CAPERR] >> 32)) break;
            if (sc[SC_SLICEFAIL] >= sl.size() || sc[SC_SLICEFAIL] < next) return fail(c, MDBG_E_DEVICE, "slice bookkeeping of the insertion is inconsistent");
            next = (size_t)sc[SC_SLICEFAIL];
            e = table_reserve(c, slice); if (e) return e;
        }
        if ((u32)sc[SC_PROBEERR]) return fail(c, MDBG_E_PARAM, "the table filled up during insertion");
        c->n_windows += sc[SC_BATCHWIN];
        if (sc[SC_IMPORTERR]) return fail(c, MDBG_E_PARAM, "read offsets of an imported sketch are not consistent with its size");
        if ((u32)sc[SC_CAPERR]) return fail(c, MDBG_E_CAPACITY, "a read has more than 2^26 minimizers");
        return MDBG_OK;
    }
    if (c->cap == 0) {
        e = read_scalars(c, sc); if (e) return e;
        c->n_distinct = sc[SC_NDISTINCT];
        if (sc[SC_IMPORTERR]) return fail(c, MDBG_E_PARAM, "read offsets of an imported sketch are not consistent with its size");
        if (!sc[SC_BATCHWIN]) {
            if (c->claim.p) for (size_t i = first; i < last; ++i) { const Batch& b = c->batches[i]; if (b.m1 > b.m0) HIPCHK(c, hipMemsetAsync(c->claim.as<u8>() + b.m0, 0, b.m1 - b.m0, s)); }
            return MDBG_OK;
        }
        e = table_reserve(c, sc[SC_BATCHWIN]); if (e) return e;
    }
    for (;;) {
        launch_reserve_check(c->shards.as<u64>(), scal(c) + SC_NDISTINCT, scal(c) + SC_BATCHWIN, c->cap, flags + 1, s);
        STAGE_EVENT(c, c->ev0, s);
        auto list_of = [&](const Batch& b) { return c->own_lists.as<u32>() + b.list_off; };
        auto seg_of = [&](const Batch& b) { return c->own_lists.as<u32>() + b.list_off + 2 * b.owned; };
        auto per_entry = [&](const Batch& b) { return listed_per_entry(table_args(c), b.m0, b.m1, b.owned, seg_of(b) != nullptr); };
        std::vector<ListedBatch> multi; u64 multi_total = 0;
        for (size_t i = first; i < last; ++i) {
            const Batch& b = c->batches[i];
            if (b.list_off != ~0ull && b.owned != ~0ull && b.owned && c->own_world > 1 && per_entry(b)) {
                ListedBatch lb{}; lb.start = multi_total; lb.m0 = b.m0; lb.m1 = b.m1; lb.first_ordinal = b.first_ordinal; lb.list = list_of(b);
                lb.slot0 = b.slot0; lb.n_reads = b.n_reads;
                multi.push_back(lb); multi_total += b.owned;
            }
        }
        if (multi.size() < 2) { multi.clear(); multi_total = 0; }
        if (c->claims_ok && c->claim.p && c->own_world > 1)
            for (size_t i = first; i < last; ++i) {
                const Batch& b = c->batches[i];
                if (b.list_off != ~0ull && b.owned != ~0ull && b.m1 > b.m0 && (!b.owned || per_entry(b)))
                    HIPCHK(c, hipMemsetAsync(c->claim.as<u8>() + b.m0, 0, b.m1 - b.m0, s));
            }
        if (!multi.empty()) {
            ListedBatch end{}; end.start = multi_total; multi.push_back(end);
            HIPCHK(c, c->listed_multi.ensure(multi.size() * sizeof(ListedBatch), 0, s));
            c->listed_multi_host = multi;
            HIPCHK(c, hipMemcpyAsync(c->listed_multi.p, c->listed_multi_host.data(), multi.size() * sizeof(ListedBatch), hipMemcpyHostToDevice, s));
            launch_insert_listed_multi(table_args(c), c->mh.as<u64>(), c->mread.as<u32>(), c->roff.as<u64>(), c->listed_multi.as<ListedBatch>(), (u32)multi.size() - 1, multi_total, flags, s);
        }
        for (size_t i = first; i < last; ++i) {
            const Batch& b = c->batches[i];
            if (multi_total && b.list_off != ~0ull && b.owned != ~0ull && b.owned && c->own_world > 1 && per_entry(b)) continue;
            if (b.list_off != ~0ull && b.owned != ~0ull && c->own_world > 1)
                launch_insert_listed(table_args(c), c->mh.as<u64>(), c->mread.as<u32>(), c->roff.as<u64>(), b.m0, b.m1, list_of(b), seg_of(b), b.owned, b.slot0, b.n_reads, b.first_ordinal, flags, s);
            else
                launch_insert_windows(table_args(c), c->mh.as<u64>(), c->mread.as<u32>(), c->roff.as<u64>(), b.m0, b.m1, b.slot0, b.first_ordinal,
                                      scal(c) + SC_NWINDOWS, flags, s);
        }
        STAGE_EVENT(c, c->ev1, s);
        if (c->own_world > 1) launch_sum_shards(c->shards.as<u64>() + SH_OWNINS * CTR_SHARDS, 1, scal(c) + SC_OWNINS, s);
        e = read_scalars(c, sc); if (e) return e;
        if (!(sc[SC_CAPERR] >> 32)) break;
// ... 174 lines not shown
    if (!c) return MDBG_E_PARAM;
    u64 nb = 0;
    StageHold hold;
    if (n_reads) { int e = stage_host_batch(c, bases, offsets, n_reads, &nb, hold); if (e) return e; }
    MDBG_LOCK(c);
    (void)hipSetDevice(c->dev);
    if (c->poisoned) return fail(c, MDBG_E_STATE, "context is in an error state");
    c->so_hash.clear(); c->so_pos.clear(); c->so_off.assign(n_reads + 1, 0);
    if (n_reads) {
        const StoreRollback tmp(c); const u64 M0 = tmp.s.M;
        const int e = sketch_device_impl(c, hold.g->bases.as<u8>(), hold.g->off.as<u64>(), n_reads, nb, 0);
        if (e) { if (e == MDBG_E_ALPHABET) c->poisoned = 0; return e; }
        const u64 m = c->M - M0;
        c->so_hash.resize(m); std::vector<u32> p32(m);
        bool ok = hipStreamSynchronize(c->stream) == hipSuccess;
        if (ok && m) ok = hipMemcpy(c->so_hash.data(), c->mh.as<u64>() + M0, m * 8, hipMemcpyDeviceToHost) == hipSuccess &&
                          hipMemcpy(p32.data(), c->mpos.as<u32>() + M0, m * 4, hipMemcpyDeviceToHost) == hipSuccess;
        if (ok) ok = hipMemcpy(c->so_off.data(), c->roff.as<u64>() + c->batches.back().slot0, (n_reads + 1) * 8, hipMemcpyDeviceToHost) == hipSuccess;
        if (!ok) return fail(c, MDBG_E_DEVICE, "sketch_only: copy to the host");
        c->so_pos.resize(m);
        for (u64 i = 0; i < m; ++i) c->so_pos[i] = p32[i];
        for (auto& o : c->so_off) o -= M0;
    }
    if (hashes) *hashes = c->so_hash.data();
    if (positions) *positions = c->so_pos.data();
    if (per_read_offsets) *per_read_offsets = c->so_off.data();
    if (n_minimizers) *n_minimizers = c->so_hash.size();
    return MDBG_OK;
}

int mdbg_query_batch(mdbg_ctx* c, const uint8_t* bases, const uint64_t* offsets, uint64_t n_reads, const uint32_t** counts,
                     const uint64_t** per_read_offsets, uint64_t* n_windows) {
    if (!c) return MDBG_E_PARAM;
    u64 nb = 0;
    StageHold hold;
    if (n_reads) { int e = stage_host_batch(c, bases, offsets, n_reads, &nb, hold); if (e) return e; }
    MDBG_LOCK(c);
    (void)hipSetDevice(c->dev);
    if (c->poisoned) return fail(c, MDBG_E_STATE, "context is in an error state");
    if (c->routed) return fail(c, MDBG_E_STATE, "not available for a routed table");
    if (c->own_world > 1) return fail(c, MDBG_E_STATE, "not available for a partitioned table: k-min-mers owned by other ranks would read as absent");
    c->q_counts.clear(); c->q_off.assign(n_reads + 1, 0);
    if (n_reads) {
        const StoreRollback tmp(c); const u64 M0 = tmp.s.M;
        const int e = sketch_device_impl(c, hold.g->bases.as<u8>(), hold.g->off.as<u64>(), n_reads, nb, 0);
        if (e) { if (e == MDBG_E_ALPHABET) c->poisoned = 0; return e; }
        const Batch b = c->batches.back();
        const u64 m = b.m1 - b.m0;
        hipStream_t s = c->stream;
        std::vector<u32> per_min(m);
        std::vector<u64> roffs(n_reads + 1);
        if (m) {
            if (c->q_dev.ensure(m * 4, 0, s) != hipSuccess) return fail(c, MDBG_E_NOMEM, "query buffer");
            launch_query_windows(table_args(c), c->P.min_abundance, c->mh.as<u64>(), c->mread.as<u32>(), c->roff.as<u64>(), b.m0, b.m1, c->q_dev.as<u32>(), s);
            if (hipMemcpyAsync(per_min.data(), c->q_dev.p, m * 4, hipMemcpyDeviceToHost, s) != hipSuccess) return fail(c, MDBG_E_DEVICE, "copy");
        }
        if (hipMemcpyAsync(roffs.data(), c->roff.as<u64>() + b.slot0, (n_reads + 1) * 8, hipMemcpyDeviceToHost, s) != hipSuccess ||
            hipStreamSynchronize(s) != hipSuccess) return fail(c, MDBG_E_DEVICE, "copy");
        const u64 k = c->P.k;
        for (u64 r = 0; r < n_reads; ++r) {
            const u64 rs = roffs[r] - M0, re = roffs[r + 1] - M0;
            if (re - rs > k) for (u64 i = rs; i + k <= re; ++i) c->q_counts.push_back(per_min[i]);
            c->q_off[r + 1] = c->q_counts.size();
        }
    }
    if (counts) *counts = c->q_counts.data();
    if (per_read_offsets) *per_read_offsets = c->q_off.data();
    if (n_windows) *n_windows = c->q_counts.size();
    return MDBG_OK;
}

int mdbg_reset(mdbg_ctx* c, uint32_t new_k) {
    if (!c) return MDBG_E_PARAM;
    MDBG_LOCK(c);
    (void)hipSetDevice(c->dev);
    if (c->poisoned == MDBG_E_DEVICE) return fail(c, MDBG_E_STATE, "context is in an error state");
    if (new_k != 0 && new_k != c->P.k) for (const Batch& b : c->batches) if (b.partial)
        return fail(c, MDBG_E_STATE, "a resident foreign sketch holds only the hashes of this k's windows (mdbg_dist segments): ingest again, or exchange whole sketches (mdbg_dist_set_exchange)");
    c->poisoned = 0;
    int e = clear_table(c); if (e) return e;
    c->ms_sketch = c->ms_insert = c->ms_finalize = 0; c->ms_tile = 0; c->n_tile_launches = 0; c->n_tile_bases = 0;
    if (c->link_ctr.p) (void)hipMemsetAsync(c->link_ctr.p, 0, 8, c->stream);
    if (new_k == 0) { store_truncate(c, 0); c->n_tiles = c->n_slow_tiles = 0; return MDBG_OK; }
    if (new_k < 2 || new_k > 4096) return fail(c, MDBG_E_PARAM, "bad k");
    if (new_k != c->P.k) for (Batch& b : c->batches) { b.owned = ~0ull; b.list_off = ~0ull; }
    c->P.k = new_k;
    return insert_resident_impl(c);
}

int mdbg_set_lmer_filter(mdbg_ctx* c, const uint64_t* codes, uint64_t n) {
    if (!c || (n && !codes)) return MDBG_E_PARAM;
    MDBG_LOCK(c);
    (void)hipSetDevice(c->dev);
    if (c->poisoned) return fail(c, MDBG_E_STATE, "context is in an error state");
    if (!c->batches.empty()) return fail(c, MDBG_E_STATE, "set the l-mer filter before the first batch (or after mdbg_reset(ctx, 0))");
    if (!codes) { c->lmer_on = false; return MDBG_OK; }
    if (c->P.scheme != MDBG_SCHEME_DENSITY) return fail(c, MDBG_E_PARAM, "the l-mer filter belongs to the density scheme (src/read.rs:200-205)");
    if (c->P.l > 32) return fail(c, MDBG_E_PARAM, "the l-mer filter needs l <= 32");
    if (n >= (1ull << 40)) return fail(c, MDBG_E_CAPACITY, "l-mer set too large");
    u64 cap = 1024; while (cap < 2 * n + 2) cap <<= 1;
    std::vector<u64> tab(cap, LMERSET_EMPTY);
    const u64 mask = cap - 1, code_mask = c->P.l == 32 ? ~0ull : ((1ull << (2 * c->P.l)) - 1);
    u32 all_ones = 0;
    for (u64 i = 0; i < n; ++i) {
        const u64 code = codes[i];
        if (code & ~code_mask) return fail(c, MDBG_E_PARAM, "an l-mer code has bits above 2*l");
        if (code == LMERSET_EMPTY) { all_ones = 1; continue; }
        for (u64 h = lmerset_home(code, mask);; h = (h + 1) & mask) { if (tab[h] == code) break; if (tab[h] == LMERSET_EMPTY) { tab[h] = code; break; } }
    }
    HIPCHK(c, c->lmer_set.ensure(cap * 8, 0, c->stream));
    HIPCHK(c, hipMemcpyAsync(c->lmer_set.p, tab.data(), cap * 8, hipMemcpyHostToDevice, c->stream));
    HIPCHK(c, hipStreamSynchronize(c->stream));
    c->lmer_mask = mask; c->lmer_all_ones = all_ones; c->lmer_on = true;
    return MDBG_OK;
}

int mdbg_mark(mdbg_ctx* c, uint64_t* mark) {
    if (!c || !mark) return MDBG_E_PARAM;
    MDBG_LOCK(c);
    if (c->pending_m) return fail(c, MDBG_E_STATE, "reserved sketch regions have not been committed");
    *mark = c->batches.size();
    return MDBG_OK;
}

int mdbg_rewind(mdbg_ctx* c, uint64_t mark) {
    if (!c) return MDBG_E_PARAM;
    MDBG_LOCK(c);
    (void)hipSetDevice(c->dev);
    if (c->poisoned == MDBG_E_DEVICE) return fail(c, MDBG_E_STATE, "context is in an error state");
    if (c->pending_m) return fail(c, MDBG_E_STATE, "reserved sketch regions have not been committed");
    if (mark > c->batches.size()) return fail(c, MDBG_E_PARAM, "not a mark of this context");
    c->poisoned = 0;
    int e = clear_table(c); if (e) return e;
    store_truncate(c, (size_t)mark);
    return MDBG_OK;
}

int mdbg_set_timing(mdbg_ctx* c, uint32_t level) {
    if (!c || level > 2) return MDBG_E_PARAM;
    MDBG_LOCK(c);
    c->timing = (int)level;
    return MDBG_OK;
}

int mdbg_get_stats(mdbg_ctx* c, mdbg_stats* o) {
    if (!c || !o) return MDBG_E_PARAM;
    MDBG_LOCK(c);
    memset(o, 0, sizeof *o);
    o->n_reads = c->n_reads; o->n_bases = c->n_bases; o->n_minimizers = c->M; o->n_windows = c->n_windows; o->n_distinct = c->n_distinct;
    o->table_capacity = c->cap; o->n_slow_tiles = c->n_slow_tiles; o->n_tiles = c->n_tiles;
    o->ms_sketch = c->ms_sketch; o->ms_insert = c->ms_insert; o->ms_finalize = c->ms_finalize;
    o->ms_sketch_tile = c->ms_tile; o->n_sketch_tile_launches = c->n_tile_launches; o->n_sketch_tile_bases = c->n_tile_bases;
    o->tile_bases = TILE_STRIDE;
    if (c->link_ctr.p) {
        (void)hipSetDevice(c->dev);
        HIPCHK(c, hipStreamSynchronize(c->stream));
        HIPCHK(c, hipMemcpy(&o->n_link_matches, c->link_ctr.p, 8, hipMemcpyDeviceToHost));
    }
    return MDBG_OK;
}

int mdbg_synth_reads_device(mdbg_ctx* c, const mdbg_synth_params* sp, uint64_t first_read, const uint8_t** d_bases, const uint64_t** d_offsets, uint64_t* n_bases) {
    if (!c || !sp) return MDBG_E_PARAM;
    MDBG_LOCK(c);
    (void)hipSetDevice(c->dev);
    if (sp->n_reads == 0 || sp->n_reads > 0x7FFFFFFFull || sp->genome_len == 0 || sp->min_len == 0 || sp->min_len > sp->max_len) return fail(c, MDBG_E_PARAM, "bad synth parameters");
    SynthP P; P.seed = sp->seed; P.genome_len = sp->genome_len; P.first_read = first_read; P.mean_len = sp->mean_len; P.sd_len = sp->sd_len;
    P.min_len = sp->min_len; P.max_len = sp->max_len; P.thr24 = (u32)(((u64)sp->err_ppm << 24) / 1000000ull);
    hipStream_t s = c->stream;
    HIPCHK(c, c->syn_lens.ensure(sp->n_reads * 8, 0, s));
    HIPCHK(c, c->syn_off.ensure((sp->n_reads + 1) * 8, 0, s));
    launch_synth(P, sp->n_reads, c->syn_lens.as<u64>(), c->syn_off.as<u64>(), nullptr, 0, s);
    u64 nb = 0;
    HIPCHK(c, hipMemcpyAsync(&nb, c->syn_off.as<u64>() + sp->n_reads, 8, hipMemcpyDeviceToHost, s));
    HIPCHK(c, hipStreamSynchronize(s));
    HIPCHK(c, c->syn_bases.ensure(nb + 64, 0, s));
    launch_synth(P, sp->n_reads, c->syn_lens.as<u64>(), c->syn_off.as<u64>(), c->syn_bases.as<u8>(), 1, s);
    HIPCHK(c, hipStreamSynchronize(s));
    if (d_bases) *d_bases = c->syn_bases.as<u8>();
    if (d_offsets) *d_offsets = c->syn_off.as<u64>();
    if (n_bases) *n_bases = nb;
    return MDBG_OK;
}
}
```

### rust_mdbg_amd/csrc/sketch.hip

```cpp
#include "mdbg_dev.h"
#include "bs_core.h"

enum { FMT_ASCII = 0, FMT_PLANES = 1 };
constexpr int SCAN_GRAN_LOG = 6, SCAN_GRAN = 1 << SCAN_GRAN_LOG;
struct TileRec;

struct SketchArgs {
    const u8* bases;
    const uint2* planes;
    u32 fmt;
    u64 n_bases;
    const u64* offsets; u32 n_reads;
    const u32* bread;
    const TileRec* recs;
    u32 n_tiles;
    u32 tile0, tile_end;
    Rec* slab; u32 slab_cap;
    u32* n_valid;
    u32* n_scan;
    u32* last_read;
    u32* over_max;
    unsigned long long* block_sum;
    const u64* t4;
    const u8* tile_flags;
    const u64* exc_pos; const u8* exc_val; u32 n_exc;
    u32* err_flag; unsigned long long* slow_total;
    u32 read_base;
    u64 bound; u32 l; u32 hpc; u32 btop;
    u32 scheme, s;
    u32 force_slow;
    u64* dbg;
    u32 stop_phase;
};

__device__ inline u32 find_read(const u64* __restrict__ off, u32 lo, u32 hi, u64 p) {
    while (lo < hi) { u32 mid = lo + ((hi - lo + 1) >> 1); if (off[mid] <= p) lo = mid; else hi = mid - 1; }
    return lo;
}


constexpr int TREC_N = 7;
struct __attribute__((aligned(16))) TileRec { u32 rl, rh; int64_t start0; int32_t rel[TREC_N - 1]; int64_t first_base; };
static_assert(sizeof(TileRec) == 48, "three 16-byte words");
struct SketchInit { u64* zero[4]; u64* set_p; u64 set_v; u64* zero_arr; u32 zero_arr_n; };
__global__ void tile_rec_kernel(const u64* __restrict__ off, u32 n_reads, u64 n_bases, u32 n_tiles, u32* __restrict__ bread, TileRec* __restrict__ recs, SketchInit init,
                                int64_t stride, int64_t halo) {
    const u32 t = blockIdx.x * blockDim.x + threadIdx.x;
    if (t == 0) { for (int i = 0; i < 4; ++i) if (init.zero[i]) *init.zero[i] = 0; if (init.set_p) *init.set_p = init.set_v; }
    if (t < init.zero_arr_n) init.zero_arr[t] = 0;
    if (t >= n_tiles + 2) return;
    auto first_pos = [&](u32 e) -> u64 {
        int64_t p = (int64_t)e * stride - halo;
        if (p < 0) p = 0;
        if ((u64)p >= n_bases) p = n_bases ? (int64_t)n_bases - 1 : 0;
        return (u64)p;
    };
    const u64 p0 = first_pos(t), p2 = first_pos(t + 2);
    u32 lo0 = 0, hi0 = n_reads - 1, lo2 = 0, hi2 = n_reads - 1;
    while (lo0 < hi0 || lo2 < hi2) {
        const u32 m0 = lo0 + ((hi0 - lo0 + 1) >> 1), m2 = lo2 + ((hi2 - lo2 + 1) >> 1);
        const u64 v0 = off[m0], v2 = off[m2];
        if (lo0 < hi0) { if (v0 <= p0) lo0 = m0; else hi0 = m0 - 1; }
        if (lo2 < hi2) { if (v2 <= p2) lo2 = m2; else hi2 = m2 - 1; }
    }
    bread[t] = lo0;
    if (t >= n_tiles) return;
    const int64_t raw0 = (int64_t)t * stride - halo;
    TileRec r;
    r.rl = lo0; r.rh = lo2;
    r.start0 = (int64_t)off[r.rl] - raw0;
    for (int i = 0; i < TREC_N - 1; ++i) {
        int64_t v = r.rl + 1 + i <= r.rh ? (int64_t)off[r.rl + 1 + i] - raw0 : 0x7FFFFFFF;
        r.rel[i] = (int32_t)(v > 0x7FFFFFFF ? 0x7FFFFFFF : v);
    }
    r.first_base = (int64_t)off[0];
    recs[t] = r;
}

struct AsciiSrc {
    const u8* b;
    __device__ u8 at(u64 q) const { return b[q]; }
    __device__ void chunk16(u64 q0, u64 n_bases, u64& lo, u64& hi) const {
        if (q0 + 16 <= n_bases) { const uint4 v = *(const uint4*)(b + q0); lo = (u64)v.x | (u64)v.y << 32; hi = (u64)v.z | (u64)v.w << 32; return; }
        lo = hi = 0;
        for (int i = 0; i < 16 && q0 + i < n_bases; ++i) { const u64 c = b[q0 + i]; if (i < 8) lo |= c << (8 * i); else hi |= c << (8 * (i - 8)); }
    }
};
struct PlaneSrc {
    const uint2* w; const u64* exc_pos; const u8* exc_val; u32 n_exc;
    __device__ u8 at(u64 q) const {
        if (n_exc) {
            u32 lo = 0, hi = n_exc;
            while (lo < hi) { const u32 mid = (lo + hi) >> 1; if (exc_pos[mid] < q) lo = mid + 1; else hi = mid; }
            if (lo < n_exc && exc_pos[lo] == q) return exc_val[lo];
        }
        const uint2 p = w[q >> 5];
        const u32 c = ((p.x >> (q & 31)) & 1u) | (((p.y >> (q & 31)) & 1u) << 1);
        return (u8)(0x47544341u >> (8 * c));
    }
    __device__ void chunk16(u64 q0, u64 n_bases, u64& lo, u64& hi) const {
        lo = hi = 0;
        if (n_exc) { for (int i = 0; i < 16 && q0 + i < n_bases; ++i) { const u64 c = at(q0 + i); if (i < 8) lo |= c << (8 * i); else hi |= c << (8 * (i - 8)); } return; }
        const uint2 p = w[q0 >> 5];
        const u32 sh = (u32)(q0 & 31), p0 = p.x >> sh, p1 = p.y >> sh;
#pragma unroll
        for (int i = 0; i < 16; ++i) {
            const u32 c = ((p0 >> i) & 1u) | (((p1 >> i) & 1u) << 1);
            const u64 ch = (0x47544341u >> (8 * c)) & 0xFFu;
            if (i < 8) lo |= ch << (8 * i); else hi |= ch << (8 * (i - 8));
        }
    }
};

template <bool HPC, class Src>
__device__ inline bool kept_at(const Src& s, u64 rlo, u64 p) {
    if (!HPC || p == rlo) return true;
    const u8 c = s.at(p);
    return !(c == s.at(p - 1) && in_hpc_set(c));
}
template <bool HPC, class Src>
__device__ inline bool walk_lmer(const Src& s, u64 rlo, u64 p, u32 l, u64& start, u64& hash) {
    u64 q = p, fh = 0, rh = 0;
    for (int j = (int)l - 1;; --j) {
        const u8 c = s.at(q);
        fh ^= rol64(nt_h_ascii(c), l - 1 - j);
        rh ^= rol64(nt_rc_ascii(c), j);
        if (j == 0) break;
        if (q == rlo) return false;
        u64 q2 = q - 1;
        if (HPC) { const u8 c2 = s.at(q2); if (in_hpc_set(c2)) while (q2 > rlo && s.at(q2 - 1) == c2) --q2; }
        q = q2;
    }
    start = q; hash = fh < rh ? fh : rh;
    return true;
}

constexpr int WPT = TILE_WPT;
constexpr int DPAD = 4;
constexpr int TILE_HW = TILE_HALO / 32;
constexpr int TILE_QCAP = 704;
constexpr int TILE_RS_CAP = 32;
static_assert(TILE_RAW_WORDS == WPT * TILE_THREADS && TILE_HW % WPT == 0 && TILE_HW % 2 == 0 && (TILE_RAW_WORDS - TILE_HW) % 2 == 0,
              "the halo is a whole number of threads; 16-byte aligned word pairs per thread");

struct __attribute__((aligned(16))) TileLds {
    u32 dense[2 * (DPAD + TILE_RAW_WORDS + 4)];
    u32 kw[TILE_RAW_WORDS];
    u16 rpre[TILE_RAW_WORDS + 8];
    struct { u32 cand[TILE_RAW_WORDS + 8]; u16 cpre[TILE_RAW_WORDS + 8]; u16 list[TILE_QCAP]; u16 surv[TILE_THREADS]; } c;
    int64_t rs0;
    int32_t rs_rel[TILE_RS_CAP];
    u32 misc[32];
};
constexpr int T3_WORDS = 2 << (2 * BS_GS);
template <int SCHEME> struct TileLdsS : TileLds {};
template <> struct TileLdsS<1> : TileLds {
    u32 dstart[TILE_RAW_WORDS + 8];
};
constexpr int SYNC_SLOW_THREADS = 128;
static_assert(sizeof(TileLdsS<1>) >= 32 * SYNC_SLOW_THREADS * 4, "the ring of the generic syncmer machine fits the tile state");
constexpr int TILE_STAGE_AT = 2 * (DPAD + TILE_RAW_WORDS + 4) + TILE_RAW_WORDS - 2 * TILE_RAW_WORDS;
static_assert(TILE_STAGE_AT >= TILE_RAW_WORDS && TILE_STAGE_AT % 4 == 0 && offsetof(TileLds, kw) == sizeof(u32) * 2 * (DPAD + TILE_RAW_WORDS + 4), "stage = dense[AT ..) + kw[]");
static_assert((2 * (DPAD + TILE_RAW_WORDS + 4) - TILE_STAGE_AT) == 4 * TILE_THREADS, "one 16-byte store per thread");
static_assert((sizeof(TileLds) + T3_WORDS * 8) * 6 <= 160 * 1024, "6 workgroups per CU");
static_assert((TILE_RAW_WORDS + 8) * 2 >= TILE_THREADS * 8 && ((TILE_RAW_WORDS + 8) * 4) % 8 == 0 && offsetof(TileLds, c) % 16 == 0, "cpre holds one u64 per thread");
static_assert(TILE_RS_CAP > TREC_N, "the read starts of a tile record fit rs_rel");

__device__ inline u32 ascii16_to_hp(uint4 v, u32& bad) {
    const u32 w[4] = {v.x, v.y, v.z, v.w};
    u32 a0h = 0, a0l = 0, a1h = 0, a1l = 0;
#pragma unroll
    for (int d = 0; d < 4; ++d) {
        const u32 sel = w[d] & 0x06060606u;
        const u32 recon = __builtin_amdgcn_perm(0x00470054u, 0x00430041u, sel);
        bad |= recon ^ w[d];
        const u32 m0 = w[d] & 0x02020202u, m1 = w[d] & 0x04040404u;
        const u32 wt = (d & 1) ? 0x01020408u : 0x10204080u;
        if (d < 2) { a0h = __builtin_amdgcn_udot4(m0, wt, a0h, false); a1h = __builtin_amdgcn_udot4(m1, wt, a1h, false); }
        else       { a0l = __builtin_amdgcn_udot4(m0, wt, a0l, false); a1l = __builtin_amdgcn_udot4(m1, wt, a1l, false); }
    }
    const u32 t0 = (a0h << 8) + a0l;
    const u32 t1 = (a1h << 8) + a1l;
    return (t0 << 15) | (t1 >> 2);
}

__device__ inline u32 range_mask(int64_t a, int64_t b) {
    if (a < 0) a = 0;
    if (b > 32) b = 32;
    if (a >= b) return 0;
    const u32 from_a = 0xFFFFFFFFu >> (u32)a;
    const u32 from_b = b == 32 ? 0u : 0xFFFFFFFFu >> (u32)b;
    return from_a & ~from_b;
}

__device__ inline u32 dpp_wave_shr1(u32 x) {
    return (u32)__builtin_amdgcn_mov_dpp((int)x, 0x138 , 0xF, 0xF, true);
}

__device__ inline u32 lds_fetch_add(u32* p, u32 v) {
    u32 r;
    const u32 addr = (u32)(uintptr_t)(__attribute__((address_space(3))) u32*)p;
    asm volatile("ds_add_rtn_u32 %0, %1, %2\n\ts_waitcnt lgkmcnt(0)" : "=v"(r) : "v"(addr), "v"(v) : "memory");
    return r;
}

__device__ inline void put_rec(const SketchArgs& a, Rec* slab, u32 rank, u64 hash, u32 pos, u32 read) {
    if (rank < a.slab_cap) { Rec r; r.hash = hash; r.pos = pos; r.read = read; slab[rank] = r; }
}
constexpr u32 LAST_NONE = 0xFFFFFFFFu, LAST_IN_SLAB = 0xFFFFFFFEu;
__device__ inline void put_count(const SketchArgs& a, u32 gt, u32 n, bool last_known = false) {
    a.n_valid[gt] = n;
    if (a.block_sum && n) atomicAdd(a.block_sum + ((gt - a.tile0) >> SCAN_GRAN_LOG), (unsigned long long)n);
    if (a.last_read && !(last_known && n)) a.last_read[gt] = n ? LAST_IN_SLAB : LAST_NONE;
    if (a.n_scan) a.n_scan[gt] = 0;
    if (n > a.slab_cap) atomicMax(a.over_max, n);
}

template <bool HPC, class Src>
__device__ void slow_tile(const SketchArgs& a, const Src& src, u32 gt, Rec* slab, TileLds& S) {
    constexpr int TT = TILE_THREADS;
    const int tid = threadIdx.x % TT;
    const u64 t_lo = (u64)gt * TILE_STRIDE;
    u64 t_hi = t_lo + TILE_STRIDE; if (t_hi > a.n_bases) t_hi = a.n_bases;
    const u32 rl = a.bread[gt], rh_ = a.bread[gt + 2];
    const u64 first_base = a.offsets[0];
    u32* tmp = S.misc;
    if (tid == 0) atomicAdd(a.slow_total, 1ull);
    u32 running = 0;
    for (u64 p0 = t_lo; p0 < t_hi; p0 += TT) {
        const u64 p = p0 + tid;
        u32 sel = 0; u64 hash = 0, start = 0; u32 r = 0; u64 rlo = 0;
        if (p < t_hi && p >= first_base) {
            r = find_read(a.offsets, rl, rh_, p);
            rlo = a.offsets[r];
            const u8 c = src.at(p);
            if (c != 'A' && c != 'C' && c != 'G' && c != 'T' && c != 'N') *a.err_flag = 1;
            if (kept_at<HPC>(src, rlo, p) && walk_lmer<HPC>(src, rlo, p, a.l, start, hash) && hash <= a.bound) sel = 1;
        }
        u32 total;
        const u32 rank = tile_excl_scan(sel, tmp, total);
        if (sel) put_rec(a, slab, running + rank, hash, (u32)(start - rlo), r + a.read_base);
        running += total;
    }
    if (tid == 0) put_count(a, gt, running);
}

constexpr int SYNC_KEEP = 8;
__device__ inline u64 sync_hash(u64 key, u64 mask) {
    key = (~key + (key << 21)) & mask;
    key = key ^ key >> 24;
    key = ((key + (key << 3)) + (key << 8)) & mask;
    key = key ^ key >> 14;
    key = ((key + (key << 2)) + (key << 4)) & mask;
    key = key ^ key >> 28;
    key = (key + (key << 31)) & mask;
    return key;
}
__device__ inline u32 sync_hash32(u32 key, u32 mask) {
    key = (~key + (key << 21)) & mask;
    key = key ^ key >> 24;
    key = ((key + (key << 3)) + (key << 8)) & mask;
    key = key ^ key >> 14;
    key = ((key + (key << 2)) + (key << 4)) & mask;
    key = key ^ key >> 28;
    key = (key + (key << 31)) & mask;
    return key;
}
__device__ inline u32 nt4_code(u8 c) {
    switch (c) {
        case 0: case 'A': case 'a': return 0;
        case 1: case 'C': case 'c': return 1;
        case 2: case 'G': case 'g': return 2;
        case 3: case 'T': case 't': case 'U': case 'u': return 3;
        default: return 4;
    }
}

template <bool HPC, class Src>
__device__ __attribute__((noinline)) void sync_slow_tile(const SketchArgs& a, const Src& src, u32 gt, Rec* slab, u32 (*dq)[SYNC_SLOW_THREADS], u32* sc_tmp) {
    constexpr int TT = SYNC_SLOW_THREADS;
    constexpr u32 SEG = (TILE_STRIDE + TT - 1) / TT;
    u32& any_over = sc_tmp[8];
    const int tid = threadIdx.x;
    if (tid == 0) atomicAdd(a.slow_total, 1ull);
    const u32 l = a.l, sm = a.s, w = l - sm + 1, t = (w + 1) / 2;
    const u64 smask = sm ? ((1ull << (2 * sm)) - 1) : 0, lmask = (1ull << (2 * l)) - 1;
    const u64 lshift = (u64)(l - 1) * 2, sshift = sm ? (u64)(sm - 1) * 2 : 0;
    const u64 first_base = a.offsets[0];
    const u64 t_lo = (u64)gt * TILE_STRIDE; u64 t_hi = t_lo + TILE_STRIDE; if (t_hi > a.n_bases) t_hi = a.n_bases;
    u64 own_lo = t_lo + (u64)tid * SEG, own_hi = own_lo + SEG;
    if (own_lo < first_base) own_lo = first_base;
    if (own_hi > t_hi) own_hi = t_hi;
    if (tid >= TT) own_lo = own_hi = t_hi;
    if (tid == 0) any_over = 0;
    __syncthreads();

    Rec keep[SYNC_KEEP]; u32 n_mine = 0;
    auto run = [&](bool write, u32 base) {
        n_mine = 0;
        if (own_lo >= own_hi) return;
        u32 r = find_read(a.offsets, 0, a.n_reads - 1, own_lo);
        for (u64 look = 96;; look *= 4) {
            u64 rlo = a.offsets[r], rhi = a.offsets[r + 1];
            u64 q = own_lo > rlo + look ? own_lo - look : rlo;
            bool conv = q == rlo;
            u32 rr = r;
            u64 xl0 = 0, xl1 = 0, min_val = ~0ull; u32 xs0 = 0, xs1 = 0, lp = 0, cnt = 0, min_idx = 0, warm = 0;
            u8 prev = q > rlo ? src.at(q - 1) : 0;
            bool restart = false;
            u64 clo = 0, chi = 0, cbase = ~0ull;
            for (; q < own_hi; ++q) {
                while (q >= rhi) { ++rr; rlo = rhi; rhi = a.offsets[rr + 1]; lp = 0; cnt = 0; xl0 = xl1 = xs0 = xs1 = 0; min_val = ~0ull; conv = true; }
                if (q == own_lo && !conv) { restart = true; break; }
                if ((q & ~15ull) != cbase) { cbase = q & ~15ull; src.chunk16(cbase, a.n_bases, clo, chi); }
                const u32 bi = (u32)(q & 15);
                const u8 c = (u8)(((bi & 8) ? chi : clo) >> (8 * (bi & 7)));
                const bool kept = !HPC || q == rlo || !(c == prev && in_hpc_set(c));
                prev = c;
                if (!kept) continue;
                const u32 code = nt4_code(c);
                if (code >= 4) { lp = 0; cnt = 0; xl0 = xl1 = xs0 = xs1 = 0; min_val = ~0ull; conv = true; continue; }
                xl0 = (xl0 << 2 | code) & lmask; xl1 = xl1 >> 2 | (u64)(3 - code) << lshift;
                if (sm) { xs0 = (xs0 << 2 | code) & (u32)smask; xs1 = xs1 >> 2 | (3 - code) << (u32)sshift; }
                ++lp; ++warm;
                bool cand = false;
                if (sm == 0) cand = lp >= l;
                else if (lp >= sm) {
                    const u32 hs = sync_hash32(xs0 < xs1 ? xs0 : xs1, (u32)smask);
                    ++cnt;
                    dq[cnt & 31][tid] = hs;
                    if (cnt >= w) {
                        if (cnt == w) {
                            min_val = ~0ull;
                            for (u32 j = cnt - w + 1; j <= cnt; ++j) { const u32 v = dq[j & 31][tid]; if (v < min_val) { min_val = v; min_idx = j; } }
                        } else if (min_idx == cnt - w) {
                            min_val = ~0ull;
                            for (u32 j = cnt; j + w > cnt; --j) { const u32 v = dq[j & 31][tid]; if (v < min_val) { min_val = v; min_idx = j; } }
                        } else if (hs < min_val) { min_val = hs; min_idx = cnt; }
                        if (!conv && warm > l) {
                            u32 ties = 0;
                            for (u32 j = cnt - w + 1; j <= cnt; ++j) ties += dq[j & 31][tid] == (u32)min_val;
                            conv = ties == 1;
                        }
                        cand = min_idx == cnt - w + t;
                    }
                }
                if (sm == 0 && !conv && warm > l) conv = true;
                if (cand && q >= own_lo) {
                    const u64 hl = sync_hash(xl0 < xl1 ? xl0 : xl1, lmask);
                    if (hl <= a.bound) {
                        u64 st = q;
                        for (u32 j = 1; j < l; ++j) {
                            u64 q2 = st - 1;
                            if (HPC) { const u8 c2 = src.at(q2); if (in_hpc_set(c2)) while (q2 > rlo && src.at(q2 - 1) == c2) --q2; }
                            st = q2;
                        }
                        Rec rec; rec.hash = hl; rec.pos = (u32)(st - rlo); rec.read = rr + a.read_base;
                        if (write) { if (base + n_mine < a.slab_cap) slab[base + n_mine] = rec; }
                        else if (n_mine < SYNC_KEEP) keep[n_mine] = rec;
                        ++n_mine;
                    }
                }
            }
            if (!restart) break;
            n_mine = 0;
        }
    };
    run(false, 0);
    if (n_mine > SYNC_KEEP) any_over = 1;
    u32 total;
    const u32 base = block_excl_scan_256(n_mine, sc_tmp, total);
    if (!any_over) {
        for (u32 i = 0; i < n_mine; ++i) if (base + i < a.slab_cap) slab[base + i] = keep[i];
    } else run(true, base);
    if (tid == 0) put_count(a, gt, total);
}


struct CandOut { u64 hash; u32 pos, read; };

#define MDBG_HOT(cond, value) (cond)
template <int L, int SCHEME = 0, int WMAX = 1>
__global__ __launch_bounds__(TILE_THREADS, SCHEME ? 5 : 6) void sketch_bs_kernel(SketchArgs a) {
    constexpr int TT = TILE_THREADS, RW = TILE_RAW_WORDS, HW = TILE_HW, QCAP = TILE_QCAP, RS_CAP = TILE_RS_CAP, STAGE_AT = TILE_STAGE_AT;
    __shared__ TileLdsS<SCHEME> S;
    __shared__ __attribute__((aligned(16))) u64 S_t3[T3_WORDS];
    __shared__ u32 sync_tmp[SCHEME ? 16 : 1];
    const u32 Lr = SCHEME ? a.l : (u32)L;
    const int tid = (int)threadIdx.x, lane = tid & 63, wv = tid >> 6;
    const int64_t nb = (int64_t)a.n_bases;
    const int64_t n_pairs = (nb + 31) >> 5;
    const bool hpc = MDBG_HOT(a.hpc != 0, true);
    typedef u32 u32x4 __attribute__((ext_vector_type(4)));
    const u32 wg = blockIdx.x, gt = a.tile0 + wg;
    Rec* const slab = a.slab + (size_t)wg * a.slab_cap;
#define MDBG_STAMP(i) do { if (a.dbg && tid == 0) a.dbg[(size_t)gt * 16 + (i)] = __builtin_readcyclecounter(); } while (0)
    MDBG_STAMP(0);
    const int64_t raw0 = (int64_t)gt * TILE_STRIDE - TILE_HALO;
    const bool interior = MDBG_HOT(raw0 >= 0 && raw0 + RW * 32 <= nb, true);
    const TileRec* const rec = a.recs + gt;
    auto uniform64 = [](int64_t v) -> int64_t {
        return (int64_t)((u64)(u32)__builtin_amdgcn_readfirstlane((int)((u64)v >> 32)) << 32 | (u32)__builtin_amdgcn_readfirstlane((int)(u32)(u64)v));
    };
    const int64_t first_base = uniform64(rec->first_base);

    u32 x0[WPT], x1[WPT], pv0 = 0, pv1 = 0;
    constexpr int CPT = RW * 2 / TT;
    uint4 av[CPT]; uint2 pr[WPT];
    const int64_t pi0 = raw0 / 32 + (int64_t)WPT * tid;
    if (MDBG_HOT(a.fmt == FMT_ASCII, false)) {
        if (interior) {
            const u32x4* src = (const u32x4*)(a.bases + raw0);
#pragma unroll
            for (int g = 0; g < CPT; ++g) { const u32x4 q = __builtin_nontemporal_load(src + tid + TT * g); av[g] = make_uint4(q.x, q.y, q.z, q.w); }
        }
    } else {
        if (interior) {
            const u32x4* src = (const u32x4*)(a.planes + pi0);
#pragma unroll
            for (int i = 0; i < WPT / 2; ++i) { const u32x4 q = __builtin_nontemporal_load(src + i); pr[2 * i] = make_uint2(q.x, q.y); pr[2 * i + 1] = make_uint2(q.z, q.w); }
        } else {
#pragma unroll
            for (int i = 0; i < WPT; ++i) { const int64_t pi = pi0 + i; pr[i] = (pi >= 0 && pi < n_pairs) ? a.planes[pi] : make_uint2(0u, 0u); }
        }
        if (tid && pi0 - 1 >= 0 && pi0 - 1 < n_pairs) { const uint2 q = a.planes[pi0 - 1]; pv0 = q.x >> 31; pv1 = q.y >> 31; }
    }
    const u32 rl = (u32)__builtin_amdgcn_readfirstlane((int)rec->rl), rh_ = (u32)__builtin_amdgcn_readfirstlane((int)rec->rh);
    static_assert((2 * (DPAD + RW + 4)) % 4 == 0, "the dense stream is a whole number of 16-byte words");
    for (int i = tid; i < 2 * (DPAD + RW + 4) / 4; i += TT) ((uint4*)S.dense)[i] = make_uint4(0u, 0u, 0u, 0u);
    if (SCHEME == 0) {
        static_assert(T3_WORDS % 128 == 0, "the table is copied 16 bytes per lane");
        for (int i = tid; i < T3_WORDS / 2; i += TT) ((uint4*)S_t3)[i] = ((const uint4*)a.t4)[i];
    } else {
        u32 v = 0;
        for (int i = 0; i < 8; ++i) v |= ((u32)tid >> i & 1u) << (2 * i);
        ((u16*)S_t3)[tid] = (u16)v;
    }
    if (tid == 0) { S.misc[8] = a.force_slow | ((a.tile_flags && a.tile_flags[gt]) ? 1u : 0u); S.misc[9] = 0; S.misc[11] = 0; S.misc[17] = 0; S.misc[18] = 0; S.misc[19] = 0; S.misc[20] = 0; }
    __syncthreads();
    if (MDBG_HOT(rh_ - rl < (u32)TREC_N, true)) {
        if ((u32)tid <= rh_ - rl) {
            const int64_t rel = tid == 0 ? rec->start0 : (int64_t)rec->rel[tid - 1];
            if (tid == 0) S.rs0 = rel; else S.rs_rel[tid] = (int32_t)rel;
            if (rel >= 0 && rel < RW * 32) atomicOr(&S.dense[rel >> 5], 0x80000000u >> (rel & 31));
        }
    } else for (u32 r = rl + tid; r <= rh_ && r < a.n_reads; r += TT) {
        const int64_t rel = (int64_t)a.offsets[r] - raw0;
        if (r == rl) S.rs0 = rel; else if (r - rl < RS_CAP) S.rs_rel[r - rl] = (int32_t)(rel > 0x7FFFFFFF ? 0x7FFFFFFF : rel);
        if (rel >= 0 && rel < RW * 32) atomicOr(&S.dense[rel >> 5], 0x80000000u >> (rel & 31));
    }
    u32* const stage = S.dense + STAGE_AT;
    if (MDBG_HOT(a.fmt == FMT_ASCII, false)) {
        u32 bad_any = 0;
        if (interior) {
#pragma unroll
            for (int g = 0; g < CPT; ++g) stage[tid + TT * g] = ascii16_to_hp(av[g], bad_any);
        } else {
#pragma unroll 1
            for (int g = 0; g < CPT; ++g) {
                const int ci = tid + TT * g;
                const int64_t pos = raw0 + 16 * (int64_t)ci;
                u32 w4[4] = {0x41414141u, 0x41414141u, 0x41414141u, 0x41414141u};
                if (pos >= 0 && pos + 16 <= nb) { const uint4 q = *(const uint4*)(a.bases + pos); w4[0] = q.x; w4[1] = q.y; w4[2] = q.z; w4[3] = q.w; }
                else for (int i = 0; i < 16; ++i) if (pos + i >= 0 && pos + i < nb) w4[i >> 2] = (w4[i >> 2] & ~(0xFFu << (8 * (i & 3)))) | ((u32)a.bases[pos + i] << (8 * (i & 3)));
                stage[ci] = ascii16_to_hp(make_uint4(w4[0], w4[1], w4[2], w4[3]), bad_any);
            }
        }
        if (bad_any) {
            S.misc[8] = 1;
            for (int g = 0; g < CPT; ++g) {
                const int64_t pos = raw0 + 16 * (int64_t)(tid + TT * g);
                for (int i = 0; i < 16; ++i) {
                    const int64_t q = pos + i;
                    if (SCHEME == 0 && q >= 0 && q < nb) { const u8 c = a.bases[q]; if (c != 'A' && c != 'C' && c != 'G' && c != 'T' && c != 'N') *a.err_flag = 1; }
                }
            }
        }
        __syncthreads();
#pragma unroll
        for (int i = 0; i < WPT; ++i) {
            const uint2 h = *(const uint2*)(stage + 2 * (WPT * tid + i));
            x0[i] = (h.x & 0xFFFF0000u) | (h.y >> 16); x1[i] = (h.x << 16) | (h.y & 0xFFFFu);
        }
        if (tid) { const u32 hp = stage[2 * WPT * tid - 1]; pv0 = hp >> 16; pv1 = hp; }
        __syncthreads();
        static_assert((2 * (DPAD + RW + 4) - STAGE_AT) == 4 * TT && STAGE_AT % 4 == 0, "one 16-byte store per thread");
        ((uint4*)(S.dense + STAGE_AT))[tid] = make_uint4(0u, 0u, 0u, 0u);
    } else {
#pragma unroll
        for (int i = 0; i < WPT; ++i) { x0[i] = __brev(pr[i].x); x1[i] = __brev(pr[i].y); }
        __syncthreads();
    }
    MDBG_STAMP(1);
    if (MDBG_HOT(a.stop_phase == 1, false)) { if (tid == 0) a.n_valid[gt] = x0[0] == 0x12345u; return; }

    u32 kw[WPT], n_kept[WPT], mine = 0;
    {
        const int64_t lo = first_base - raw0, hi = nb - raw0;
        if (MDBG_HOT(interior && lo <= 0 && hpc, true)) {
            const uint4 st = *(const uint4*)(S.dense + WPT * tid);
            *(uint4*)(S.dense + WPT * tid) = make_uint4(0u, 0u, 0u, 0u);
            const u32 sb[WPT] = {st.x, st.y, st.z, st.w};
#pragma unroll
            for (int i = 0; i < WPT; ++i) {
                const u32 d0 = bs_alignbit(i ? x0[i - 1] : pv0, x0[i], 1), d1 = bs_alignbit(i ? x1[i - 1] : pv1, x1[i], 1);
                u32 k = (x0[i] ^ d0) | (x1[i] ^ d1) | sb[i];
                if (i == 0) k |= tid == 0 ? 0x80000000u : 0u;
                kw[i] = k; n_kept[i] = bs_popc(k); mine += n_kept[i];
            }
        } else {
#pragma unroll
        for (int i = 0; i < WPT; ++i) {
            const int w = WPT * tid + i;
            const u32 vm = interior && lo <= 0 ? 0xFFFFFFFFu : range_mask(lo - 32 * (int64_t)w, hi - 32 * (int64_t)w);
            u32 k = vm;
            if (hpc) {
                const u32 d0 = bs_alignbit(i ? x0[i - 1] : pv0, x0[i], 1), d1 = bs_alignbit(i ? x1[i - 1] : pv1, x1[i], 1);
                k = ((x0[i] ^ d0) | (x1[i] ^ d1) | S.dense[w]) & vm;
                if (w == 0) k |= 0x80000000u & vm;
            }
            S.dense[w] = 0;
            kw[i] = k; n_kept[i] = bs_popc(k); mine += n_kept[i];
        }
        }
        if (hpc) {
#pragma unroll
            for (int i = 0; i < WPT; ++i) bs_compress2(kw[i], x0[i], x1[i]);
        } else {
#pragma unroll
            for (int i = 0; i < WPT; ++i) if (kw[i] != 0xFFFFFFFFu) bs_compress2(kw[i], x0[i], x1[i]);
        }
    }
    u32 H;
    u32 off = tile_excl_scan(mine, S.misc, H);
    static_assert(HW % WPT == 0, "the halo is a whole number of threads");
    if (tid == HW / WPT) S.misc[11] = off;
    if (tid == TT - 1) S.rpre[RW] = (u16)H;
    static_assert(WPT == 4, "one 16-byte store of keep masks and one 8-byte store of prefixes per thread");
    *(uint4*)(S.kw + WPT * tid) = make_uint4(kw[0], kw[1], kw[2], kw[3]);
    {
        const u32 o1 = off + n_kept[0], o2 = o1 + n_kept[1], o3 = o2 + n_kept[2];
        *(uint2*)(S.rpre + WPT * tid) = make_uint2(off | o1 << 16, o2 | o3 << 16);
    }
#pragma unroll
    for (int i = 0; i < WPT; ++i) {
        const u32 n = n_kept[i];
        {
            const u32 wi = off >> 5, s = off & 31;
            unsigned long long* dst = (unsigned long long*)(S.dense + 2 * (DPAD + wi));
            atomicOr(dst, (unsigned long long)(x0[i] >> s) | ((unsigned long long)(x1[i] >> s) << 32));
            atomicOr(dst + 1, (unsigned long long)bs_alignbit(x0[i], 0u, s) | ((unsigned long long)bs_alignbit(x1[i], 0u, s) << 32));
        }
        off += n;
    }
    __syncthreads();
    MDBG_STAMP(2);
    if (MDBG_HOT(a.stop_phase == 2, false)) { if (tid == 0) a.n_valid[gt] = 0; return; }
    const u32 Hh = S.misc[11];
    const bool true_start = raw0 <= first_base;
    auto run_slow_tile = [&]() {
        if constexpr (SCHEME == 0) {
            if (a.fmt == FMT_ASCII) { AsciiSrc src{a.bases}; if (hpc) slow_tile<true>(a, src, gt, slab, S); else slow_tile<false>(a, src, gt, slab, S); }
            else { PlaneSrc src{a.planes, a.exc_pos, a.exc_val, a.tile_flags && a.tile_flags[gt] ? a.n_exc : 0u}; if (hpc) slow_tile<true>(a, src, gt, slab, S); else slow_tile<false>(a, src, gt, slab, S); }
        } else {
            if (a.fmt == FMT_ASCII) { AsciiSrc src{a.bases}; if (hpc) sync_slow_tile<true>(a, src, gt, slab, (u32(*)[SYNC_SLOW_THREADS])&S, sync_tmp); else sync_slow_tile<false>(a, src, gt, slab, (u32(*)[SYNC_SLOW_THREADS])&S, sync_tmp); }
            else { PlaneSrc src{a.planes, a.exc_pos, a.exc_val, a.tile_flags && a.tile_flags[gt] ? a.n_exc : 0u}; if (hpc) sync_slow_tile<true>(a, src, gt, slab, (u32(*)[SYNC_SLOW_THREADS])&S, sync_tmp); else sync_slow_tile<false>(a, src, gt, slab, (u32(*)[SYNC_SLOW_THREADS])&S, sync_tmp); }
        }
    };
    if (MDBG_HOT(S.misc[8] || (!true_start && Hh < Lr), false)) { __syncthreads(); run_slow_tile(); return; }

    const u32 e_lo = Hh > Lr - 1 ? Hh : Lr - 1;
    const u32 n_out = H ? ((H + BS_B - 2) >> 5) + 1 : 0;
    const u32 n_rs = rh_ - rl + 1;
    if constexpr (SCHEME == 0) {
        u32 bmask[BS_B];
#pragma unroll
        for (int i = 0; i < BS_B; ++i) bmask[i] = ((a.btop >> (BS_B - 1 - i)) & 1u) ? 0xFFFFFFFFu : 0u;
        const u32 n_steps = (n_out + 62) / 63;
        const bool zero_test = MDBG_HOT(a.btop == 0, true);
        const u32 wv_s = (u32)__builtin_amdgcn_readfirstlane(wv);
        const int nb_addr = 4 * ((lane + 63) & 63);
        const int x_lo = __builtin_amdgcn_readfirstlane((int)e_lo + BS_B - 1), x_hi = __builtin_amdgcn_readfirstlane((int)H + BS_B - 1);
        for (u32 st = wv_s; st < n_steps; st += TT / 64) {
            const int D = (int)(63 * st) + lane - 1;
            const u32* dw = S.dense + 2 * (DPAD + (D < RW + 3 ? D : RW + 3));
            const uint2 c = *(const uint2*)dw, p = *(const uint2*)(dw - 2);
            uint2 q = make_uint2(0u, 0u);
            if (L + BS_B - 2 >= 32) q = *(const uint2*)(dw - 4);
            u32 W[BS_B], Wp[BS_B], inv;
            bs_strand_planes<L, true>(c.x, c.y, p.x, p.y, q.x, q.y, W, inv);
#pragma unroll
            for (int i = 0; i < BS_B - 1; ++i) Wp[i] = (u32)__builtin_amdgcn_ds_bpermute(nb_addr, (int)W[i]);
            Wp[BS_B - 1] = 0;
            u32 cand = zero_test ? bs_strand_compare<true, true>(W, Wp, inv, bmask) : bs_strand_compare<true, false>(W, Wp, inv, bmask);
            bs_strand_planes<L, false>(c.x, c.y, p.x, p.y, q.x, q.y, W, inv);
            Wp[0] = 0;
#pragma unroll
            for (int i = 1; i < BS_B; ++i) Wp[i] = (u32)__builtin_amdgcn_ds_bpermute(nb_addr, (int)W[i]);
            cand |= zero_test ? bs_strand_compare<false, true>(W, Wp, inv, bmask) : bs_strand_compare<false, false>(W, Wp, inv, bmask);
            const int Dw0 = (int)(63 * st) - 1;
            if (32 * Dw0 < x_lo || 32 * (Dw0 + 64) > x_hi) cand &= range_mask((int64_t)x_lo - 32 * (int64_t)D, (int64_t)x_hi - 32 * (int64_t)D);
            if (lane && (u32)D < n_out) S.c.cand[D] = cand;
        }
        for (u32 D = n_out + tid; D < RW + 8; D += TT) S.c.cand[D] = 0;
    } else {
        const u32 l = a.l, sm = a.s, w = l - sm + 1, t = (w + 1) / 2;
        const u32 smask = sm ? (sm >= 16 ? 0xFFFFFFFFu : (1u << (2 * sm)) - 1u) : 0u, sshift = sm ? 2 * (sm - 1) : 0;
        for (int i = tid; i < RW + 8; i += TT) { S.dstart[i] = 0; S.c.cand[i] = 0; }
        __syncthreads();
        auto mark_start = [&](int64_t rel) {
            if (rel < 0 || rel >= (int64_t)RW * 32) return;
            const u32 rw = (u32)rel >> 5, rb = (u32)rel & 31;
            const u32 dp = S.rpre[rw] + (rb ? bs_popc(S.kw[rw] >> (32 - rb)) : 0u);
            if (dp < H && ((S.kw[rw] << rb) & 0x80000000u)) atomicOr(&S.dstart[dp >> 5], 0x80000000u >> (dp & 31));
        };
        if (n_rs <= RS_CAP) { for (u32 i = tid; i < n_rs; i += TT) mark_start(i ? (int64_t)S.rs_rel[i] : S.rs0); }
        else for (u32 r = rl + tid; r <= rh_ && r < a.n_reads; r += TT) mark_start((int64_t)a.offsets[r] - raw0);
        __syncthreads();
        constexpr int SG = 16;
        constexpr int NH = WMAX + SG - 1;
        const bool use_lut = sm != 0 && sm <= 4;
        u16* const lut = (u16*)S_t3 + 256;
        u32* const lut32 = (u32*)S.c.list;
        static_assert(sizeof(S.c.list) >= 256 * 4 && offsetof(TileLds, c) % 4 == 0 && (sizeof(S.c.cand) + sizeof(S.c.cpre)) % 4 == 0, "the packed s-mer table fits the candidate list");
        if (use_lut) {
            const u32 ia = (u32)tid >> sm, ib = (u32)tid & ((1u << sm) - 1u);
            u32 fw = 0, rc = 0;
            for (u32 j = 0; j < sm; ++j) {
                const u32 c = ((ia >> (sm - 1 - j)) & 1u) << 1 | ((ib >> (sm - 1 - j)) & 1u);
                fw |= c << (2 * (sm - 1 - j)); rc |= (3u - c) << (2 * j);
            }
            const u32 hv = sync_hash32(fw < rc ? fw : rc, smask);
            lut[tid] = (u16)hv;
            lut32[tid] = (hv << 6) * 0x10001u;
        }
        __syncthreads();
        {
            const u32 n_own = H > e_lo ? H - e_lo : 0u;
            const u32 Qw = (((n_own + TT / 64 - 1) / (TT / 64)) + (64u * SG - 1u)) & ~(64u * SG - 1u);
            const u32 wv_s = (u32)__builtin_amdgcn_readfirstlane(wv);
            const u32 Awv = e_lo + wv_s * Qw, Bwv = Awv + Qw < H ? Awv + Qw : H;
            int32_t carry = 4096;
            bool need_slow = false;
            auto word64 = [](u32 x, u32 y, u32 z, u32 r) -> u64 {
                const u32 hi = r ? (x << r) | (y >> (32u - r)) : x, lo = r ? (y << r) | (z >> (32u - r)) : y;
                return (u64)hi << 32 | lo;
            };
            const u32 fm = sm ? (1u << sm) - 1u : 0u;
            auto put_cands = [&](u32 bits, int32_t p0_) {
                if (!bits) return;
                const u32 x0c = (u32)p0_ + BS_B - 1;
                const u64 cb = ((u64)__brev(bits) << 32) >> (x0c & 31u);
                if ((u32)(cb >> 32)) atomicOr(&S.c.cand[x0c >> 5], (u32)(cb >> 32));
                if ((u32)cb) atomicOr(&S.c.cand[(x0c >> 5) + 1], (u32)cb);
            };
            if (Awv < H) for (int32_t rd = -1; (int64_t)Awv + (int64_t)rd * (64 * SG) < (int64_t)Bwv; ++rd) {
                const int32_t p0 = (int32_t)Awv + rd * (64 * SG) + lane * SG;
                const int32_t qb = p0 - (int32_t)(l - 1);
                const int32_t wi = qb >> 5; const u32 rr = (u32)qb & 31u;
                u32 pl1[3], pl0[3], stw[3];
#pragma unroll
                for (int j = 0; j < 3; ++j) {
                    const int32_t D = wi + j;
                    const int32_t Dc = D < -DPAD ? -DPAD : D > RW + 3 ? RW + 3 : D, Ds = D < 0 ? 0 : D > RW + 3 ? RW + 3 : D;
                    const uint2 dw = *(const uint2*)(S.dense + 2 * (DPAD + Dc));
                    const u32 st = S.dstart[Ds];
                    pl1[j] = D == Dc ? dw.y : 0u; pl0[j] = D == Dc ? dw.x ^ dw.y : 0u;
                    stw[j] = D == Ds ? st : 0u;
                }
                const u64 W1 = word64(pl1[0], pl1[1], pl1[2], rr), W0 = word64(pl0[0], pl0[1], pl0[2], rr), WS = word64(stw[0], stw[1], stw[2], rr);
                const int32_t n_mine = (int32_t)Bwv - p0;
                const u32 own = n_mine >= SG ? (1u << SG) - 1u : n_mine <= 0 ? 0u : (1u << n_mine) - 1u;
                const int32_t i_hi = (int32_t)H - qb;
                const u64 LIVE = (qb <= -64 ? 0ull : qb < 0 ? ~0ull >> (u32)(-qb) : ~0ull) & (i_hi >= 64 ? ~0ull : i_hi <= 0 ? 0ull : ~(~0ull >> (u32)i_hi));
                auto andrun = [](u64 V, u32 n) -> u64 {
                    if (n == 0) return ~0ull;
                    u32 pw = 1;
                    for (; 2 * pw <= n; pw *= 2) V &= V << pw;
                    return V & (V << (n - pw));
                };
                u32 vmask = (1u << SG) - 1u, fmask = 0;
                const bool rare = __any((int)(LIVE != ~0ull || WS != 0ull)) != 0;
                if (rare) {
                    const u64 OKW = andrun(LIVE, l) & andrun(~(WS << 1), l - 1);
                    vmask = __brev((u32)(OKW >> 32)) & ((1u << SG) - 1u);
                    fmask = vmask & __brev((u32)(WS >> 32));
                }
                if (sm == 0) {
                    if (rd >= 0) put_cands(vmask & own, p0);
                    continue;
                }
                if (use_lut && !rare) {
                    typedef unsigned short us2 __attribute__((ext_vector_type(2)));
                    auto pkmin = [](u32 x, u32 y) -> u32 { return __builtin_bit_cast(u32, __builtin_elementwise_min(__builtin_bit_cast(us2, x), __builtin_bit_cast(us2, y))); };
                    constexpr int32_t ANY = 1 << 20;
                    const u64 Z1 = W1 >> (14u - sm), Z0 = W0 >> (14u - sm);
                    u32 e[NH];
#pragma unroll
                    for (int ii = 0; ii < NH; ++ii) {
                        const u32 ka = (u32)(Z1 >> (48 - ii)) & (fm << 2), kb = (u32)(Z0 >> (48 - ii)) & (fm << 2);
                        e[ii] = *(const u32*)((const char*)lut32 + (ka << sm | kb)) | ((u32)(63 - ii) << 16 | (u32)ii);
                    }
                    u32 m[SG];
                    if constexpr (WMAX > 2) {
                        constexpr int B = WMAX - 1;
                        u32 sx[NH], px[NH];
#pragma unroll
                        for (int i = NH - 1; i >= 0; --i) sx[i] = (i % B == B - 1 || i == NH - 1) ? e[i] : pkmin(e[i], sx[(i + 1) % NH]);
#pragma unroll
                        for (int i = 0; i < NH; ++i) px[i] = i % B == 0 ? e[i] : pkmin(e[i], px[(i + NH - 1) % NH]);
#pragma unroll
                        for (int jj = 0; jj < SG; ++jj) m[jj] = pkmin(sx[jj], px[jj + B]);
                    } else {
#pragma unroll
                        for (int jj = 0; jj < SG; ++jj) { u32 x = e[jj]; for (int d = 1; d < WMAX; ++d) x = pkmin(x, e[jj + d]); m[jj] = x; }
                    }
// ... 116 lines not shown
                    for (;;) {
                        bool chg = false;
                        if (!indep) { int32_t tt = Tin; u32 c2 = 0, u2 = 0;
#pragma unroll
                            for (int jj = 0; jj < SG; ++jj) step(jj, tt, c2, u2);
                            chg = tt != Tout; Tout = tt; }
                        if (!__any((int)chg)) break;
                        Tin = shift_in(Tout);
                    }
                }
                carry = __builtin_amdgcn_readlane(Tout, 63);
                if (rd >= 0) {
                    const u32 k8 = K & ((1u << SG) - 1u);
                    const u32 dep = k8 ? (k8 & (0u - k8)) - 1u : (1u << SG) - 1u;
                    if (Tin != UNKI && dep) {
                        int32_t tt = Tin; u32 c2 = 0, u2 = 0;
#pragma unroll
                        for (int jj = 0; jj < SG; ++jj) { if (!__any((int)((dep >> jj) & 1u))) break; if ((dep >> jj) & 1u) step(jj, tt, c2, u2); }
                        cbits |= c2 & dep; ubits = (ubits & ~dep) | (u2 & dep);
                    }
                    need_slow = need_slow || (ubits & vmask & own) != 0u;
                    put_cands(cbits & vmask & own, p0);
                }
            }
            if (need_slow) S.misc[9] = 1;
        }
        __syncthreads();
        if (S.misc[9]) { __syncthreads(); run_slow_tile(); return; }
    }
    __syncthreads();
    auto expand_list = [&]() {
        const uint4 cw = *(const uint4*)(S.c.cand + WPT * tid);
        const u32 w5[5] = {cw.x, cw.y, cw.z, cw.w, tid == TT - 1 ? S.c.cand[RW] : 0u};
        const u32 c = bs_popc(cw.x) + bs_popc(cw.y) + bs_popc(cw.z) + bs_popc(cw.w) + bs_popc(w5[4]);
        const u32 inc_c = wave_incl_scan(c);
        u32 wbase = 0;
        if (lane == 63) wbase = lds_fetch_add(&S.misc[17], inc_c);
        wbase = (u32)__builtin_amdgcn_readlane((int)wbase, 63);
        if (c) {
            u32 slot = wbase + inc_c - c;
#pragma unroll
            for (int i = 0; i < 5; ++i) {
                u32 w = w5[i];
                while (w) {
                    const u32 b = (u32)__clz(w); w &= ~(0x80000000u >> b);
                    if (slot < QCAP) S.c.list[slot] = (u16)(32 * (WPT * tid + i) + b - (BS_B - 1));
                    ++slot;
                }
            }
        }
    };
    expand_list();
    __syncthreads();
    MDBG_STAMP(3);
    if (MDBG_HOT(a.stop_phase == 3, false)) { if (tid == 0) a.n_valid[gt] = 0; return; }

    auto count_words = [&]() -> u32 {
        const uint4 cw = *(const uint4*)(S.c.cand + WPT * tid);
        const u32 c0 = bs_popc(cw.x), c1 = bs_popc(cw.y), c2 = bs_popc(cw.z), c3 = bs_popc(cw.w);
        const u32 last = tid == TT - 1 ? bs_popc(S.c.cand[RW]) : 0u;
        u32 total;
        const u32 o = tile_excl_scan(c0 + c1 + c2 + c3 + last, S.misc, total);
        const u32 o1 = o + c0, o2 = o1 + c1, o3 = o2 + c2;
        *(uint2*)(S.c.cpre + WPT * tid) = make_uint2(o | o1 << 16, o2 | o3 << 16);
        if (tid == TT - 1) S.c.cpre[RW] = (u16)(o3 + c3);
        __syncthreads();
        return total;
    };
    const float raw_per_dense = (float)RW / (float)(H ? H : 1u);
    auto dense_to_raw = [&](u32 r) -> u32 {
        u32 w = (u32)((float)r * raw_per_dense);
        w = w < (u32)RW - 1u ? w : (u32)RW - 1u;
        while (S.rpre[w] > r) --w;
        while (S.rpre[w + 1] <= r) ++w;
        return 32 * w + bs_select_msb(S.kw[w], r - S.rpre[w]);
    };
    auto exact = [&](u32 e) -> u64 {
        const u32 wi = e >> 5, s = e & 31;
        const u32* dw = S.dense + 2 * (DPAD + wi);
        const u32 v0 = bs_alignbit(dw[-2], dw[0], 31 - s), v1 = bs_alignbit(dw[-1], dw[1], 31 - s);
        if constexpr (SCHEME == 0) return bs_exact_hash<BS_GS, L>(v0, v1, S_t3);
        else {
            const u32 lm = Lr >= 32 ? 0xFFFFFFFFu : (1u << Lr) - 1u;
            const u32 r0 = (v0 ^ v1) & lm, r1 = v1 & lm;
            const u16* sp = (const u16*)S_t3;
            const u32 lo = ((u32)sp[r0 & 255u] | (u32)sp[(r0 >> 8) & 255u] << 16) | ((u32)sp[r1 & 255u] | (u32)sp[(r1 >> 8) & 255u] << 16) << 1;
            const u32 hi = ((u32)sp[(r0 >> 16) & 255u] | (u32)sp[r0 >> 24] << 16) | ((u32)sp[(r1 >> 16) & 255u] | (u32)sp[r1 >> 24] << 16) << 1;
            const u64 lmask = (1ull << (2 * Lr)) - 1ull;
            const u64 xl0 = (u64)hi << 32 | lo;
            const u64 cm = ~xl0 & lmask;
            u64 y = (u64)__brev((u32)cm) << 32 | (u64)__brev((u32)(cm >> 32));
            y = ((y >> 1) & 0x5555555555555555ull) | ((y & 0x5555555555555555ull) << 1);
            const u64 xl1 = y >> (64 - 2 * Lr);
            return sync_hash(xl0 < xl1 ? xl0 : xl1, lmask);
        }
    };
    auto place = [&](u32 e, u64 h, CandOut& o) -> bool {
        const u32 sd = e - (Lr - 1);
        const int64_t rel_start = dense_to_raw(sd);
        u32 r; int64_t q0, q1;
        if (MDBG_HOT(n_rs <= RS_CAP, true)) {
            u32 i = 0;
            while (i + 1 < n_rs && (int64_t)S.rs_rel[i + 1] <= rel_start) ++i;
            r = rl + i; q0 = i ? (int64_t)S.rs_rel[i] : S.rs0; q1 = i + 1 < n_rs ? (int64_t)S.rs_rel[i + 1] : (int64_t)RW * 32;
        } else {
            r = find_read(a.offsets, rl, rh_, (u64)(raw0 + rel_start)); q0 = (int64_t)a.offsets[r] - raw0;
            q1 = r < rh_ ? (int64_t)a.offsets[r + 1] - raw0 : (int64_t)RW * 32;
        }
        bool crosses = false;
        if (q1 < (int64_t)RW * 32) {
            const u32 w = (u32)q1 >> 5, b = (u32)q1 & 31;
            const u32 ds = S.rpre[w] + (b ? bs_popc(S.kw[w] >> (32 - b)) : 0u);
            crosses = ds <= e;
        }
        o.hash = h; o.pos = (u32)(rel_start - q0); o.read = r + a.read_base;
        return !crosses;
    };
    auto clear_bit = [&](u32 e) { const u32 x = e + BS_B - 1; atomicAnd(&S.c.cand[x >> 5], ~(0x80000000u >> (x & 31))); };
    auto rank_of = [&](u32 e) -> u32 { const u32 x = e + BS_B - 1, D = x >> 5, b = x & 31; return S.c.cpre[D] + (b ? bs_popc(S.c.cand[D] >> (32 - b)) : 0u); };

    auto process_list = [&](u32 n) -> u32 {
        constexpr int NR = (QCAP + TT - 1) / TT;
        CandOut keep[NR] = {}; u32 keep_e[NR] = {}; u32 keep_ok = 0;
        u64* const s_h = (u64*)S.c.cpre;
#pragma unroll
        for (int i = 0; i < NR; ++i) {
            if ((u32)(TT * i) < n) {
                if (i) __syncthreads();
                const u32 j = tid + TT * i;
                bool pass = false; u32 e = 0; u64 h = 0;
                if (j < n) { e = S.c.list[j]; h = exact(e); pass = h <= a.bound; if (!pass) clear_bit(e); }
                const u64 bal = __ballot(pass);
                if (bal) {
                    u32 base = 0;
                    if (lane == 0) base = atomicAdd(&S.misc[18 + i], (u32)__popcll(bal));
                    base = (u32)__builtin_amdgcn_readfirstlane((int)base);
                    if (pass) { const u32 slot = base + __builtin_amdgcn_mbcnt_hi((u32)(bal >> 32), __builtin_amdgcn_mbcnt_lo((u32)bal, 0u)); S.c.surv[slot] = (u16)e; s_h[slot] = h; }
                }
                __syncthreads();
                const u32 n_surv = S.misc[18 + i];
                if ((u32)tid < n_surv) {
                    e = S.c.surv[tid];
                    keep_e[i] = e;
                    if (place(e, s_h[tid], keep[i])) keep_ok |= 1u << i; else clear_bit(e);
                }
            }
        }
        __syncthreads();
        MDBG_STAMP(4);
        if (MDBG_HOT(a.stop_phase == 4, false)) return 0u;
        const u32 left = count_words();
        MDBG_STAMP(5);
        if (MDBG_HOT(a.stop_phase == 5, false)) return 0u;
#pragma unroll
        for (int i = 0; i < NR; ++i) if ((keep_ok >> i) & 1u) {
            const u32 rank = rank_of(keep_e[i]);
            put_rec(a, slab, rank, keep[i].hash, keep[i].pos, keep[i].read);
            if (rank + 1 == left && a.last_read) a.last_read[gt] = keep[i].read;
        }
        return left;
    };

    const u32 n_cand = S.misc[17];
    if (MDBG_HOT(n_cand <= QCAP, true)) {
        const u32 nv = n_cand ? process_list(n_cand) : 0;
        if (tid == 0) { put_count(a, gt, nv, true); if (a.dbg) { a.dbg[(size_t)gt * 16 + 9] = n_cand; a.dbg[(size_t)gt * 16 + 10] = nv; } }
    } else {
        __syncthreads();
        if constexpr (SCHEME == 1) {
            {
                const uint4 cw = *(const uint4*)(S.c.cand + WPT * tid);
                u32 w5[5] = {cw.x, cw.y, cw.z, cw.w, tid == TT - 1 ? S.c.cand[RW] : 0u};
#pragma unroll
                for (int i = 0; i < 5; ++i) {
                    u32 w = w5[i], keep = w;
                    while (w) {
                        const u32 b = (u32)__clz(w), bit = 0x80000000u >> b; w &= ~bit;
                        if (exact((u32)(32 * (WPT * tid + i)) + b - (BS_B - 1)) > a.bound) keep &= ~bit;
                    }
                    w5[i] = keep;
                }
                *(uint4*)(S.c.cand + WPT * tid) = make_uint4(w5[0], w5[1], w5[2], w5[3]);
                if (tid == TT - 1) S.c.cand[RW] = w5[4];
                if (tid == 0) S.misc[17] = 0;
            }
            __syncthreads();
            expand_list();
            __syncthreads();
            const u32 n2 = S.misc[17];
            if (n2 <= QCAP) {
                const u32 nv = n2 ? process_list(n2) : 0;
                if (tid == 0) { put_count(a, gt, nv, true); if (a.dbg) { a.dbg[(size_t)gt * 16 + 9] = n_cand; a.dbg[(size_t)gt * 16 + 10] = nv; } }
                return;
            }
            __syncthreads();
        }
        const u32 C = count_words();
        const u32 per = (C + TT - 1) / TT;
        const u32 r0 = (u32)tid * per < C ? (u32)tid * per : C, r1 = r0 + per < C ? r0 + per : C;
        u32 surv = 0;
        if (r0 < r1) {
            u32 lo = 0, hi = RW;
            while (lo < hi) { const u32 mid = (lo + hi + 1) >> 1; if (S.c.cpre[mid] <= r0) lo = mid; else hi = mid - 1; }
            u32 D = lo, w = S.c.cand[D];
            for (u32 skip = r0 - S.c.cpre[D]; skip; --skip) w &= ~(0x80000000u >> (u32)__clz(w));
            for (u32 r = r0; r < r1; ++r) {
                while (!w) { ++D; w = S.c.cand[D]; }
                const u32 b = (u32)__clz(w); w &= ~(0x80000000u >> b);
                const u32 e = 32 * D + b - (BS_B - 1);
                const u64 h = exact(e);
                CandOut o{}; bool ok = false;
                if (h <= a.bound) ok = place(e, h, o);
                Rec rec; rec.hash = ok ? o.hash : 0ull; rec.pos = ok ? o.pos : 0u; rec.read = ok ? o.read : 0xFFFFFFFFu;
                surv += ok ? 1u : 0u;
                if (r < a.slab_cap) slab[r] = rec;
            }
        }
        u32 nv;
        tile_excl_scan(surv, S.misc, nv);
        if (tid == 0) {
            a.n_valid[gt] = nv; if (a.n_scan) a.n_scan[gt] = C;
            if (a.block_sum && nv) atomicAdd(a.block_sum + ((gt - a.tile0) >> SCAN_GRAN_LOG), (unsigned long long)nv);
            if (a.last_read) a.last_read[gt] = nv ? LAST_IN_SLAB : LAST_NONE;
            if (C > a.slab_cap) atomicMax(a.over_max, C);
            if (a.dbg) { a.dbg[(size_t)gt * 16 + 9] = n_cand; a.dbg[(size_t)gt * 16 + 10] = nv; }
        }
    }
    MDBG_STAMP(7);
#undef MDBG_STAMP
}

__global__ __launch_bounds__(256) void tile_scan_sums_kernel(u32 n, const u32* __restrict__ n_valid, u64* __restrict__ block_sum) {
    __shared__ u32 ws[4];
    const u32 i0 = blockIdx.x * 1024 + threadIdx.x * 4;
    u32 v = 0;
#pragma unroll
    for (int q = 0; q < 4; ++q) if (i0 + q < n) v += n_valid[i0 + q];
    for (int d = 32; d; d >>= 1) v += __shfl_down(v, d, 64);
    if ((threadIdx.x & 63) == 0) ws[threadIdx.x >> 6] = v;
    __syncthreads();
    if (threadIdx.x == 0) block_sum[blockIdx.x] = (u64)ws[0] + ws[1] + ws[2] + ws[3];
}
__global__ __launch_bounds__(256) void tile_scan_top_kernel(u32 n_blocks, u64* __restrict__ block_sum, u64* __restrict__ carry) {
    __shared__ u64 ws[4]; __shared__ u64 run;
    const int tid = threadIdx.x, lane = tid & 63, wv = tid >> 6;
    if (tid == 0) run = carry[0];
    __syncthreads();
    for (u32 i0 = 0; i0 < n_blocks; i0 += 256) {
        const u32 i = i0 + tid;
        const u64 v = i < n_blocks ? block_sum[i] : 0;
        u64 inc = v;
        for (int d = 1; d < 64; d <<= 1) { const u64 o = __shfl_up(inc, d, 64); if (lane >= d) inc += o; }
        if (lane == 63) ws[wv] = inc;
        __syncthreads();
        u64 b = run, tot = 0;
        for (int q = 0; q < 4; ++q) { if (q < wv) b += ws[q]; tot += ws[q]; }
        if (i < n_blocks) block_sum[i] = b + inc - v;
        __syncthreads();
        if (tid == 0) run += tot;
        __syncthreads();
    }
    if (tid == 0) carry[0] = run;
}
__global__ __launch_bounds__(256) void tile_scan_final_kernel(u32 n, const u32* __restrict__ n_valid, const u64* __restrict__ block_base, u64* __restrict__ tile_base,
                                                              u32 self_base, const u64* __restrict__ carry) {
    __shared__ u32 tmp[8];
    __shared__ u64 ws[4];
    const u32 i0 = blockIdx.x * 1024 + threadIdx.x * 4;
    u32 v[4], mine = 0;
#pragma unroll
    for (int q = 0; q < 4; ++q) { v[q] = i0 + q < n ? n_valid[i0 + q] : 0u; mine += v[q]; }
    u64 bb;
    if (self_base) {
        u64 x = 0;
        if (self_base == 2) { const u32 ng = blockIdx.x * (1024 / SCAN_GRAN); for (u32 g = threadIdx.x; g < ng; g += 256) x += block_base[g]; }
        else {
#pragma unroll
            for (u32 q = 0; q < 4; ++q) if (4 * threadIdx.x + q < blockIdx.x) x += block_base[4 * threadIdx.x + q];
        }
        for (int d = 32; d; d >>= 1) x += __shfl_down(x, d, 64);
        if ((threadIdx.x & 63) == 0) ws[threadIdx.x >> 6] = x;
        __syncthreads();
        bb = carry[0] + ws[0] + ws[1] + ws[2] + ws[3];
    } else bb = block_base[blockIdx.x];
    u32 total;
    u64 b = bb + block_excl_scan_256(mine, tmp, total);

#pragma unroll
    for (int q = 0; q < 4; ++q) { if (i0 + q < n) tile_base[i0 + q] = b; b += v[q]; }
}
struct GatherArgs {
    u32 tile0, n; const Rec* slab; u32 slab_cap; const u32* n_valid; const u32* n_scan; const u64* tile_base;
    const u32* last_read;
    u64* out_hash; u32* out_pos; u32* out_read; u64 out_cap;
    u64 m0; u32 slot0, n_reads; u64* off; u32 last_launch;
    u64* carry;
    u32 tiles_per_wave;
};
constexpr u32 REC_REJECTED = 0xFFFFFFFFu;
__global__ __launch_bounds__(256) void gather_kernel(GatherArgs g) {
    const u32 b = blockIdx.x * 4 + (threadIdx.x >> 6);
    if (b >= g.n) return;
    const u32 lane = threadIdx.x & 63;
    const Rec* s = g.slab + (size_t)b * g.slab_cap;
    const u32 nv = g.n_valid[g.tile0 + b];
    const u32 ns = g.n_scan ? g.n_scan[g.tile0 + b] : 0u;
    const u64 base = g.tile_base[b];
    u32 lr = LAST_IN_SLAB;
    if (g.last_read && b) lr = g.last_read[g.tile0 + b - 1];
    Rec pre[2];
#pragma unroll
    for (int u = 0; u < 2; ++u) { pre[u] = Rec{}; if (64 * u + lane < g.slab_cap) pre[u] = s[64 * u + lane]; }
    const u32 slots = ns ? ns : nv;
    const bool tail = g.last_launch && b == g.n - 1;
    if (g.carry && b == g.n - 1 && lane == 0) *g.carry = base + nv;
    if ((!nv && !tail) || slots > g.slab_cap) return;
    int64_t prev = (int64_t)g.slot0 - 1;
    if (b && lr < LAST_IN_SLAB) prev = (int64_t)lr;
    else {
        int64_t q = (int64_t)b - 1;
        while (q >= 0 && g.n_valid[g.tile0 + q] == 0) --q;
        if (q >= 0) {
            const u32 lq = g.last_read ? g.last_read[g.tile0 + q] : LAST_IN_SLAB;
            if (lq < LAST_IN_SLAB) prev = (int64_t)lq;
            else {
                const u32 cq = g.n_valid[g.tile0 + q], sq = g.n_scan ? g.n_scan[g.tile0 + q] : 0u;
                int64_t j = (int64_t)(sq ? sq : cq) - 1;
                if (j < (int64_t)g.slab_cap) {
                    const Rec* t = g.slab + (size_t)q * g.slab_cap;
                    while (j >= 0 && t[j].read == REC_REJECTED) --j;
                    if (j >= 0) prev = (int64_t)t[j].read;
                }
            }
        } else { const u64 b0 = g.tile_base[0]; if (b0 > g.m0 && b0 <= g.out_cap) prev = (int64_t)g.out_read[b0 - 1]; }
    }
    const int64_t lo = (int64_t)g.slot0 - 1, hi = (int64_t)g.slot0 + g.n_reads;
    if (prev < lo) prev = lo;
    u64 out = base;
    for (u32 j0 = 0; j0 < slots; j0 += 64) {
        const u32 j = j0 + lane;
        Rec r{}; r.read = REC_REJECTED;
        if (j < slots) r = pre[0];
        pre[0] = pre[1];
        if (j + 128 < slots && j + 128 < g.slab_cap) pre[1] = s[j + 128];
        const bool valid = r.read != REC_REJECTED;
        const u64 bal = __ballot(valid);
        const u64 lower = bal & ((1ull << lane) - 1ull);
        const u32 from_lane = __shfl(r.read, lower ? 63 - __clzll((long long)lower) : 0, 64);
        const int64_t pr = lower ? (int64_t)from_lane : prev;
        const u32 last_valid = __shfl(r.read, bal ? 63 - __clzll((long long)bal) : 0, 64);
        if (valid) {
            const u64 idx = out + (u64)__popcll(lower);
            if (idx < g.out_cap) { g.out_hash[idx] = r.hash; g.out_pos[idx] = r.pos; g.out_read[idx] = r.read; }
            int64_t cur = (int64_t)r.read; if (cur > hi) cur = hi;
            for (int64_t x = pr + 1; x <= cur; ++x) g.off[x] = idx;
        }
        if (bal) prev = (int64_t)last_valid;
        out += (u64)__popcll(bal);
    }
    if (tail) {
        int64_t last = prev < lo ? lo : prev;
        for (int64_t x = last + 1 + lane; x <= hi; x += 64) g.off[x] = out;
    }
}

__global__ __launch_bounds__(256) void gather_multi_kernel(GatherArgs g) {
    const u32 T0 = g.tiles_per_wave;
    const u32 b0 = (blockIdx.x * 4 + (threadIdx.x >> 6)) * T0;
    if (b0 >= g.n) return;
    const u32 lane = threadIdx.x & 63;
    const u32 T = g.n - b0 < T0 ? g.n - b0 : T0;
    u32 nv = 0, ns = 0;
    if (lane < T) { nv = g.n_valid[g.tile0 + b0 + lane]; ns = g.n_scan ? g.n_scan[g.tile0 + b0 + lane] : 0u; }
    const u64 base = g.tile_base[b0];
    u32 lr = LAST_IN_SLAB;
    if (g.last_read && b0) lr = g.last_read[g.tile0 + b0 - 1];
    u32 slots = ns ? ns : nv;
    if (slots > g.slab_cap) slots = 0;
    const u32 inc = wave_incl_scan(slots);
    const u32 S = (u32)__builtin_amdgcn_readlane((int)inc, 63);
    const u32 nv_all = (u32)__builtin_amdgcn_readlane((int)wave_incl_scan(nv), 63);
    const bool tail = g.last_launch && b0 + T == g.n;
    if (g.carry && b0 + T == g.n && lane == 0) *g.carry = base + nv_all;
    if (!S && !tail) return;
    const Rec* const s0 = g.slab + (size_t)b0 * g.slab_cap;
    auto fetch = [&](u32 j) -> Rec {
        Rec r{}; r.read = REC_REJECTED;
        u32 ti = 0, ex = 0;
        for (u32 t = 0; t + 1 < T; ++t) { const u32 it = (u32)__builtin_amdgcn_readlane((int)inc, (int)t); if (j >= it) { ti = t + 1; ex = it; } }
        if (j < S) r = s0[(size_t)ti * g.slab_cap + (j - ex)];
        return r;
    };
    Rec cur = fetch(lane);
    int64_t prev = (int64_t)g.slot0 - 1;
    if (b0 && lr < LAST_IN_SLAB) prev = (int64_t)lr;
    else {
        int64_t q = (int64_t)b0 - 1;
        while (q >= 0 && g.n_valid[g.tile0 + q] == 0) --q;
        if (q >= 0) {
            const u32 lq = g.last_read ? g.last_read[g.tile0 + q] : LAST_IN_SLAB;
            if (lq < LAST_IN_SLAB) prev = (int64_t)lq;
            else {
                const u32 cq = g.n_valid[g.tile0 + q], sq = g.n_scan ? g.n_scan[g.tile0 + q] : 0u;
                int64_t j = (int64_t)(sq ? sq : cq) - 1;
                if (j < (int64_t)g.slab_cap) {
                    const Rec* t = g.slab + (size_t)q * g.slab_cap;
                    while (j >= 0 && t[j].read == REC_REJECTED) --j;
                    if (j >= 0) prev = (int64_t)t[j].read;
                }
            }
        } else { const u64 bb = g.tile_base[0]; if (bb > g.m0 && bb <= g.out_cap) prev = (int64_t)g.out_read[bb - 1]; }
    }
    const int64_t lo = (int64_t)g.slot0 - 1, hi = (int64_t)g.slot0 + g.n_reads;
    if (prev < lo) prev = lo;
    u64 out = base;
    for (u32 j0 = 0; j0 < S; j0 += 64) {
        const Rec r = cur;
        if (j0 + 64 < S) cur = fetch(j0 + 64 + lane);
        const bool valid = r.read != REC_REJECTED;
        const u64 bal = __ballot(valid);
        const u64 lower = bal & ((1ull << lane) - 1ull);
        const u32 from_lane = __shfl(r.read, lower ? 63 - __clzll((long long)lower) : 0, 64);
        const int64_t pr = lower ? (int64_t)from_lane : prev;
        const u32 last_valid = __shfl(r.read, bal ? 63 - __clzll((long long)bal) : 0, 64);
        if (valid) {
            const u64 idx = out + (u64)__popcll(lower);
            if (idx < g.out_cap) { g.out_hash[idx] = r.hash; g.out_pos[idx] = r.pos; g.out_read[idx] = r.read; }
            int64_t c = (int64_t)r.read; if (c > hi) c = hi;
            for (int64_t x = pr + 1; x <= c; ++x) g.off[x] = idx;
        }
        if (bal) prev = (int64_t)last_valid;
        out += (u64)__popcll(bal);
    }
    if (tail) {
        int64_t last = prev < lo ? lo : prev;
        for (int64_t x = last + 1 + lane; x <= hi; x += 64) g.off[x] = out;
    }
}

template <class Src>
__global__ __launch_bounds__(256) void alphabet_rule_kernel(Src src, const u64* __restrict__ off, u32 n_reads, u32 l, u32 hpc,
                                                            unsigned long long* __restrict__ which) {
    const u32 r = blockIdx.x * 4 + (threadIdx.x >> 6);
    if (r >= n_reads) return;
    const u32 lane = threadIdx.x & 63;
    const u64 a = off[r], b = off[r + 1];
    u64 kept = 0; bool bad = false;
    for (u64 p = a + lane; p < b; p += 64) {
        const u8 c = src.at(p);
        bad |= !(c == 'A' || c == 'C' || c == 'G' || c == 'T' || c == 'N');
        if (!hpc || p == a || !(c == src.at(p - 1) && in_hpc_set(c))) ++kept;
    }
    for (int d = 32; d; d >>= 1) kept += __shfl_down(kept, d, 64);
    const bool any_bad = __ballot(bad) != 0;
    if (lane == 0 && any_bad && kept >= l) atomicMin(which, (unsigned long long)r);
}

__global__ void tile_flags_kernel(const u64* __restrict__ exc_pos, u32 n_exc, u32 n_tiles, u8* __restrict__ flags, u64 stride, u64 halo) {
    const u32 i = blockIdx.x * blockDim.x + threadIdx.x;
    if (i >= n_exc) return;
    const u64 p = exc_pos[i];
    const u64 t = p / stride;
    if (t < n_tiles) flags[t] = 1;
    if (t + 1 < n_tiles && p + halo >= (t + 1) * stride) flags[t + 1] = 1;
}

__global__ __launch_bounds__(256) void pack_planes_kernel(const u8* __restrict__ bases, u64 n_bases, uint2* __restrict__ words,
                                                          u64* __restrict__ exc_pos, u8* __restrict__ exc_val, u64 exc_cap,
                                                          unsigned long long* __restrict__ n_exc) {
    const u64 w = (u64)blockIdx.x * blockDim.x + threadIdx.x;
    const u64 p0 = w * 32;
    if (p0 >= n_bases) return;
    u32 bad = 0, hp[2];
#pragma unroll
    for (int h = 0; h < 2; ++h) {
        const u64 p = p0 + 16 * h;
        u32 w4[4] = {0x41414141u, 0x41414141u, 0x41414141u, 0x41414141u};
        if (p + 16 <= n_bases) { const uint4 q = *(const uint4*)(bases + p); w4[0] = q.x; w4[1] = q.y; w4[2] = q.z; w4[3] = q.w; }
        else for (int i = 0; i < 16; ++i) if (p + i < n_bases) w4[i >> 2] = (w4[i >> 2] & ~(0xFFu << (8 * (i & 3)))) | ((u32)bases[p + i] << (8 * (i & 3)));
        hp[h] = ascii16_to_hp(make_uint4(w4[0], w4[1], w4[2], w4[3]), bad);
    }
    words[w] = make_uint2(__brev((hp[0] & 0xFFFF0000u) | (hp[1] >> 16)), __brev((hp[0] << 16) | (hp[1] & 0xFFFFu)));
    if (bad) {
        for (int i = 0; i < 32 && p0 + i < n_bases; ++i) {
            const u8 c = bases[p0 + i];
            if (c != 'A' && c != 'C' && c != 'G' && c != 'T') {
                const u64 slot = atomicAdd(n_exc, 1ull);
                if (slot < exc_cap) { exc_pos[slot] = p0 + i; exc_val[slot] = c; }
            }
        }
    }
}
void launch_pack_planes(const u8* bases, u64 n_bases, uint2* words, u64* exc_pos, u8* exc_val, u64 exc_cap, unsigned long long* n_exc, hipStream_t s) {
    const u64 nw = (n_bases + 31) / 32;
    if (nw) hipLaunchKernelGGL(pack_planes_kernel, dim3((unsigned)((nw + 255) / 256)), dim3(256), 0, s, bases, n_bases, words, exc_pos, exc_val, exc_cap, n_exc);
}

void launch_bread(const u64* offsets, u32 n_reads, u64 n_bases, u32 n_tiles, u32* bread, TileRec* recs, const SketchInit& init, hipStream_t s) {
    const u32 n = n_tiles + 2;
    hipLaunchKernelGGL(tile_rec_kernel, dim3((n + 255) / 256), dim3(256), 0, s, offsets, n_reads, n_bases, n_tiles, bread, recs, init, (int64_t)TILE_STRIDE, (int64_t)TILE_HALO);
}
void launch_tile_flags(const u64* exc_pos, u32 n_exc, u32 n_tiles, u8* flags, hipStream_t s) {
    if (n_exc) hipLaunchKernelGGL(tile_flags_kernel, dim3((n_exc + 255) / 256), dim3(256), 0, s, exc_pos, n_exc, n_tiles, flags, (u64)TILE_STRIDE, (u64)TILE_HALO);
}
void launch_alphabet_rule(const SketchArgs& a, unsigned long long* which, hipStream_t s) {
    if (!a.n_reads) return;
    const dim3 g((a.n_reads + 3) / 4), b(256);
    if (a.fmt == FMT_ASCII) hipLaunchKernelGGL(alphabet_rule_kernel<AsciiSrc>, g, b, 0, s, AsciiSrc{a.bases}, a.offsets, a.n_reads, a.l, a.hpc, which);
    else hipLaunchKernelGGL(alphabet_rule_kernel<PlaneSrc>, g, b, 0, s, PlaneSrc{a.planes, a.exc_pos, a.exc_val, a.n_exc}, a.offsets, a.n_reads, a.l, a.hpc, which);
}

void launch_sketch(SketchArgs a, u32 n_tiles, hipStream_t s, hipEvent_t ev_begin, hipEvent_t ev_end) {
    if (!n_tiles) return;
    a.tile_end = a.tile0 + n_tiles;
    if (ev_begin) (void)hipEventRecord(ev_begin, s);
    if (a.scheme == 1) {
        switch (a.l - a.s + 1) {
#define MDBG_W(n) case n: hipLaunchKernelGGL((sketch_bs_kernel<0, 1, n>), dim3(n_tiles), dim3(TILE_THREADS), 0, s, a); break;
            MDBG_W(1) MDBG_W(2) MDBG_W(3) MDBG_W(4) MDBG_W(5) MDBG_W(6) MDBG_W(7) MDBG_W(8) MDBG_W(9) MDBG_W(10) MDBG_W(11) MDBG_W(12) MDBG_W(13) MDBG_W(14) MDBG_W(15) MDBG_W(16)
            MDBG_W(17) MDBG_W(18) MDBG_W(19) MDBG_W(20) MDBG_W(21) MDBG_W(22) MDBG_W(23) MDBG_W(24) MDBG_W(25) MDBG_W(26) MDBG_W(27) MDBG_W(28) MDBG_W(29) MDBG_W(30) MDBG_W(31)
#undef MDBG_W
            default: hipLaunchKernelGGL((sketch_bs_kernel<0, 1, 32>), dim3(n_tiles), dim3(TILE_THREADS), 0, s, a); break;
        }
    }
    else switch (a.l) {
#define MDBG_L(n) case n: hipLaunchKernelGGL((sketch_bs_kernel<n>), dim3(n_tiles), dim3(TILE_THREADS), 0, s, a); break;
        MDBG_L(2) MDBG_L(3) MDBG_L(4) MDBG_L(5) MDBG_L(6) MDBG_L(7) MDBG_L(8) MDBG_L(9) MDBG_L(10) MDBG_L(11) MDBG_L(12) MDBG_L(13)
        MDBG_L(14) MDBG_L(15) MDBG_L(16) MDBG_L(17) MDBG_L(18) MDBG_L(19) MDBG_L(20) MDBG_L(21) MDBG_L(22) MDBG_L(23) MDBG_L(24)
        MDBG_L(25) MDBG_L(26) MDBG_L(27) MDBG_L(28) MDBG_L(29) MDBG_L(30) MDBG_L(31) MDBG_L(32)
#undef MDBG_L
        default: hipLaunchKernelGGL((sketch_bs_kernel<32>), dim3(n_tiles), dim3(TILE_THREADS), 0, s, a); break;
    }
    if (ev_end) (void)hipEventRecord(ev_end, s);
}

void launch_excl_scan_u32(const u32* v, u32 n, u64* scan_tmp, u64* out, u64* carry, hipStream_t s) {
    if (!n) return;
    const u32 nb = (n + 1023) / 1024;
    hipLaunchKernelGGL(tile_scan_sums_kernel, dim3(nb), dim3(256), 0, s, n, v, scan_tmp);
    hipLaunchKernelGGL(tile_scan_top_kernel, dim3(1), dim3(256), 0, s, nb, scan_tmp, carry);
    hipLaunchKernelGGL(tile_scan_final_kernel, dim3(nb), dim3(256), 0, s, n, v, scan_tmp, out, 0u, carry);
}
void launch_gather(const GatherArgs& g, u64* scan_tmp, u64* tile_base, u64* carry, hipStream_t s, const u64* gran_sum = nullptr) {
    if (!g.n) return;
    const u32 n = g.n, nb = (n + 1023) / 1024;
    const u32 self_base = nb <= 1024 ? 1u : 0u;
    if (gran_sum && self_base) hipLaunchKernelGGL(tile_scan_final_kernel, dim3(nb), dim3(256), 0, s, n, g.n_valid + g.tile0, gran_sum, tile_base, 2u, carry);
    else {
        hipLaunchKernelGGL(tile_scan_sums_kernel, dim3(nb), dim3(256), 0, s, n, g.n_valid + g.tile0, scan_tmp);
        if (!self_base) hipLaunchKernelGGL(tile_scan_top_kernel, dim3(1), dim3(256), 0, s, nb, scan_tmp, carry);
        hipLaunchKernelGGL(tile_scan_final_kernel, dim3(nb), dim3(256), 0, s, n, g.n_valid + g.tile0, scan_tmp, tile_base, self_base, carry);
    }
    GatherArgs a = g; a.tile_base = tile_base; a.carry = self_base ? carry : nullptr;
    if (a.tiles_per_wave > 1) { const u32 nw = (n + a.tiles_per_wave - 1) / a.tiles_per_wave; hipLaunchKernelGGL(gather_multi_kernel, dim3((nw + 3) / 4), dim3(256), 0, s, a); }
    else hipLaunchKernelGGL(gather_kernel, dim3((n + 3) / 4), dim3(256), 0, s, a);
}

constexpr u64 LMERSET_EMPTY = ~0ull;
struct LmerFilterArgs {
    const u64* set; u64 set_mask; u32 has_all_ones;
    const u64* mh; const u32* mpos; const u32* mread; u64 m0, m1;
    const u64* offsets; u32 slot0; u32 l; u32 hpc;
    Rec* slab; u32* n_valid;
};
__host__ __device__ inline u64 lmerset_home(u64 code, u64 mask) { return fmix64(code) & mask; }
template <bool HPC, class Src>
__device__ inline bool lmer_code_at(const Src& s, u64 rlo, u64 rhi, u64 p, u32 l, u64& code) {
    u64 q = p, c64 = 0;
    for (u32 j = 0; j < l; ++j) {
        if (q >= rhi) return false;
        const u8 c = s.at(q);
        if (c != 'A' && c != 'C' && c != 'G' && c != 'T') return false;
        c64 = (c64 << 2) | (u64)((c >> 1) & 3);
        ++q;
        if (HPC) while (q < rhi && s.at(q) == c) ++q;
    }
    code = c64;
    return true;
}
template <bool HPC, class Src>
__global__ __launch_bounds__(256) void lmer_filter_kernel(LmerFilterArgs a, Src src) {
    __shared__ u32 tmp[8];
    const u64 i = a.m0 + (u64)blockIdx.x * 256 + threadIdx.x;
    u32 keep = 0; Rec rec{};
    if (i < a.m1) {
        rec.hash = a.mh[i]; rec.pos = a.mpos[i]; rec.read = a.mread[i];
        const u32 r = rec.read - a.slot0;
        const u64 rlo = a.offsets[r], rhi = a.offsets[r + 1];
        u64 code;
        if (lmer_code_at<HPC>(src, rlo, rhi, rlo + rec.pos, a.l, code)) {
            if (code == LMERSET_EMPTY) keep = a.has_all_ones;
            else for (u64 h = lmerset_home(code, a.set_mask);; h = (h + 1) & a.set_mask) {
                const u64 v = a.set[h];
                if (v == code) { keep = 1; break; }
                if (v == LMERSET_EMPTY) break;
            }
        }
    }
    u32 total;
    const u32 rank = block_excl_scan_256(keep, tmp, total);
    if (keep) a.slab[(size_t)blockIdx.x * 256 + rank] = rec;
    if (threadIdx.x == 0) a.n_valid[blockIdx.x] = total;
}
u32 lmer_filter_blocks(u64 n_minimizers) { return (u32)((n_minimizers + 255) / 256); }
void launch_lmer_filter(const LmerFilterArgs& a, u32 fmt, const u8* bases, const uint2* planes, const u64* exc_pos, const u8* exc_val, u32 n_exc, hipStream_t s) {
    const u32 nb = lmer_filter_blocks(a.m1 - a.m0);
    if (!nb) return;
    if (fmt == FMT_ASCII) {
        const AsciiSrc src{bases};
        if (a.hpc) hipLaunchKernelGGL((lmer_filter_kernel<true, AsciiSrc>), dim3(nb), dim3(256), 0, s, a, src);
        else hipLaunchKernelGGL((lmer_filter_kernel<false, AsciiSrc>), dim3(nb), dim3(256), 0, s, a, src);
    } else {
        const PlaneSrc src{planes, exc_pos, exc_val, n_exc};
        if (a.hpc) hipLaunchKernelGGL((lmer_filter_kernel<true, PlaneSrc>), dim3(nb), dim3(256), 0, s, a, src);
        else hipLaunchKernelGGL((lmer_filter_kernel<false, PlaneSrc>), dim3(nb), dim3(256), 0, s, a, src);
    }
}

u64 make_hash_bound(double density) {
    const double v = density * 18446744073709551616.0;
    return !(v > 0.0) ? 0 : (v >= 18446744073709551616.0 ? ~0ull : (u64)v);
}
```

### rust_mdbg_amd/csrc/store.inc

```
namespace {
int store_ensure(mdbg_ctx* c, u64 want_m) {
    if (want_m <= c->mcap) return MDBG_OK;
    if (c->pending_m) return fail(c, MDBG_E_STATE, "the sketch store would have to move while reserved regions are pending (commit them, or size the store up front with mdbg_store_reserve)");
    hipStream_t s = c->stream;
    HIPCHK(c, c->mh.ensure(want_m * 8, c->M * 8, s));
    HIPCHK(c, c->mpos.ensure(want_m * 4, c->M * 4, s));
    HIPCHK(c, c->mread.ensure(want_m * 4, c->M * 4, s));
    HIPCHK(c, c->claim.ensure(want_m + 128, c->M, s));
    c->mcap = want_m;
    return MDBG_OK;
}
int next_slot0(mdbg_ctx* c, u64 m0, u64 n_reads, u32* slot0) {
    if (!c->batches.empty() && c->slot_end_m != m0) c->n_slots += 1;
    if ((u64)c->n_slots + n_reads >= 0xFFFFFFF0ull) return fail(c, MDBG_E_CAPACITY, "too many reads");
    *slot0 = c->n_slots;
    HIPCHK(c, c->roff.ensure(((u64)c->n_slots + n_reads + 2) * 8, ((u64)c->n_slots + 1) * 8, c->stream));
    return MDBG_OK;
}
void store_append(mdbg_ctx* c, const Batch& b) { c->batches.push_back(b); c->n_slots = b.slot0 + b.n_reads; c->slot_end_m = b.m1; c->M = std::max(c->M, b.m1); }
u64 store_reserve_region(mdbg_ctx* c, u64 n) { const u64 region = c->M; c->M += n; c->pending_m += n; return region; }
void store_commit_region(mdbg_ctx* c, u64 n) { c->pending_m -= n; }
struct StoreSnapshot { u64 M, slot_end_m; u32 n_slots; size_t n_batches; u64 n_reads, n_bases, n_tiles, n_slow_tiles; double ms_sketch, ms_tile; u64 n_tile_launches, n_tile_bases; };
StoreSnapshot store_snapshot(const mdbg_ctx* c) { return {c->M, c->slot_end_m, c->n_slots, c->batches.size(), c->n_reads, c->n_bases, c->n_tiles, c->n_slow_tiles, c->ms_sketch, c->ms_tile, c->n_tile_launches, c->n_tile_bases}; }
void store_restore(mdbg_ctx* c, const StoreSnapshot& s) {
    c->M = s.M; c->n_slots = s.n_slots; c->slot_end_m = s.slot_end_m; c->batches.resize(s.n_batches);
    c->n_reads = s.n_reads; c->n_bases = s.n_bases; c->n_tiles = s.n_tiles; c->n_slow_tiles = s.n_slow_tiles;
    c->ms_sketch = s.ms_sketch; c->ms_tile = s.ms_tile; c->n_tile_launches = s.n_tile_launches; c->n_tile_bases = s.n_tile_bases;
}
struct StoreRollback { mdbg_ctx* const c; const StoreSnapshot s; explicit StoreRollback(mdbg_ctx* c_) : c(c_), s(store_snapshot(c_)) {} ~StoreRollback() { store_restore(c, s); } };
void store_truncate(mdbg_ctx* c, size_t n_batches) {
    for (size_t i = n_batches; i < c->batches.size(); ++i) { c->n_reads -= std::min<u64>(c->n_reads, c->batches[i].n_reads); c->n_bases -= std::min<u64>(c->n_bases, c->batches[i].n_bases); }
    c->batches.resize(n_batches); c->batches_inserted = 0;
    if (n_batches) { const Batch& b = c->batches.back(); c->M = b.m1; c->n_slots = b.slot0 + b.n_reads; c->slot_end_m = b.m1; }
    else { c->M = 0; c->n_slots = 0; c->slot_end_m = 0; c->pending_m = 0; c->own_lists_n = 0; }
}

struct SketchInput {
    u32 fmt = FMT_ASCII;
    const u8* d_bases = nullptr;
    const uint2* d_planes = nullptr;
    const u64* d_exc_pos = nullptr; const u8* d_exc_val = nullptr; u64 n_exc = 0;
};

int keep_batch(mdbg_ctx* c, const SketchInput& in, const u64* d_offsets, u64 n_reads, u64 n_bases, std::shared_ptr<KeptReads>& out) {
    hipStream_t s = c->stream;
    std::shared_ptr<KeptReads> k = std::make_shared<KeptReads>();
    k->n_reads = n_reads; k->n_bases = n_bases; k->n_words = (n_bases + 31) / 32;
    HIPCHK(c, mdbg_block_alloc(&k->blk, k->n_words * 8 + (n_reads + 1) * 8, &k->cap));
    HIPCHK(c, hipMemcpyAsync(k->offsets(), d_offsets, (n_reads + 1) * 8, hipMemcpyDeviceToDevice, s));
    if (in.fmt == FMT_PLANES) {
        if (k->n_words) HIPCHK(c, hipMemcpyAsync(k->planes(), in.d_planes, k->n_words * 8, hipMemcpyDeviceToDevice, s));
        k->n_exc = in.n_exc;
        if (k->n_exc) {
            HIPCHK(c, mdbg_block_alloc(&k->xblk, k->n_exc * 9, &k->xcap));
            HIPCHK(c, hipMemcpyAsync(k->exc_pos(), in.d_exc_pos, k->n_exc * 8, hipMemcpyDeviceToDevice, s));
            HIPCHK(c, hipMemcpyAsync(k->exc_val(), in.d_exc_val, k->n_exc, hipMemcpyDeviceToDevice, s));
        }
        HIPCHK(c, hipStreamSynchronize(s));
    } else if (k->n_words) {
        HIPCHK(c, c->kp_cnt.ensure(8, 0, s));
        u64 cap = std::max<u64>(c->kp_exc_pos.cap / 8, 4096), n = 0;
        for (int attempt = 0; attempt < 2; ++attempt) {
            HIPCHK(c, c->kp_exc_pos.ensure(cap * 8, 0, s)); HIPCHK(c, c->kp_exc_val.ensure(cap, 0, s));
            HIPCHK(c, hipMemsetAsync(c->kp_cnt.p, 0, 8, s));
            launch_pack_planes(in.d_bases, n_bases, k->planes(), c->kp_exc_pos.as<u64>(), c->kp_exc_val.as<u8>(), cap, (unsigned long long*)c->kp_cnt.p, s);
            HIPCHK(c, hipMemcpyAsync(&n, c->kp_cnt.p, 8, hipMemcpyDeviceToHost, s));
            HIPCHK(c, hipStreamSynchronize(s));
            if (n <= cap) break;
            cap = n;
        }
        if (n > cap) return fail(c, MDBG_E_DEVICE, "the exception count of a kept batch changed between two passes");
        k->n_exc = n;
        if (n) {
            HIPCHK(c, mdbg_block_alloc(&k->xblk, n * 9, &k->xcap));
            if (!c->cb) c->cb = contig_buffers_create();
            HIPCHK(c, sort_exceptions(c->cb, c->kp_exc_pos.as<u64>(), c->kp_exc_val.as<u8>(), k->exc_pos(), k->exc_val(), n, s));
        }
    } else HIPCHK(c, hipStreamSynchronize(s));
    out = std::move(k);
    return MDBG_OK;
}

static void fill_mread_of(mdbg_ctx* c, Batch& b) {
    if (b.mread_ok) return;
    launch_fill_mread(c->roff.as<u64>(), b.slot0, b.n_reads, c->mread.as<u32>(), c->stream);
    b.mread_ok = true;
}
}
```

Before: 2531.

## Write sketch minimizers directly to the store via decoupled look-back prefix

Adds a direct-store path to the sketch kernel. Each tile takes a dynamic ticket, publishes its minimizer count, and resolves its output offset with a wave-wide decoupled look-back over the status words. It then writes hash, position and read straight into the global store, skipping the slab, the block-sum scan and the gather kernel. A small kernel rebuilds the per-read offsets afterwards. Tiles that overflow or cannot resolve a prefix poison their status, and the host then disables the direct path and retries the batch, at the cost of spin-waiting between tiles and a re-run when that happens.

New measurement: 1961. -22.5%, worse.

```diff
diff --git a/include/mdbg_hip.h b/include/mdbg_hip.h
--- a/include/mdbg_hip.h
+++ b/include/mdbg_hip.h
@@ -71,7 +71,9 @@
     uint64_t n_sketch_tile_bases;
     uint64_t tile_bases;
     uint64_t n_link_matches;
-    uint64_t reserved[3];
+    uint64_t direct_store_last;
+    uint64_t n_direct_retries;
+    uint64_t reserved[1];
 } mdbg_stats;
 
 mdbg_ctx* mdbg_create(const mdbg_params* p, int* err);
diff --git a/rust_mdbg_amd/api.py b/rust_mdbg_amd/api.py
--- a/rust_mdbg_amd/api.py
+++ b/rust_mdbg_amd/api.py
@@ -36,7 +36,7 @@
                 ("n_distinct", C.c_uint64), ("table_capacity", C.c_uint64), ("n_slow_tiles", C.c_uint64), ("n_tiles", C.c_uint64),
                 ("ms_sketch", C.c_double), ("ms_insert", C.c_double), ("ms_finalize", C.c_double), ("ms_sketch_tile", C.c_double),
                 ("n_sketch_tile_launches", C.c_uint64), ("n_sketch_tile_bases", C.c_uint64), ("tile_bases", C.c_uint64),
-                ("n_link_matches", C.c_uint64), ("reserved", C.c_uint64 * 3)]
+                ("n_link_matches", C.c_uint64), ("direct_store_last", C.c_uint64), ("n_direct_retries", C.c_uint64), ("reserved", C.c_uint64 * 1)]
 
 
 class RoutedLists(C.Structure):
diff --git a/rust_mdbg_amd/csrc/context.inc b/rust_mdbg_amd/csrc/context.inc
--- a/rust_mdbg_amd/csrc/context.inc
+++ b/rust_mdbg_amd/csrc/context.inc
@@ -41,6 +41,7 @@
     u64 h_known = 0;
     DevBuf bread, tile_recs, slab, n_valid, n_scan, last_read, tile_base, scan_tmp, gran_sum, tile_flags, scalars, phase_dbg, shards;
     u32 slab_cap_min = 0;
+    DevBuf lb; bool direct_store = true, direct_off = false, direct_last = false; u64 n_direct_retries = 0;
     DevBuf tab, mx; u64 cap = 0;
     DevBuf arena, route_out, route_tmp, route_h, route_f; u64 n_records = 0; bool routed = false;
     DevBuf by_maps;
@@ -318,6 +319,7 @@
     for (auto& g : c->stage) if (hipStreamCreateWithFlags(&g.st, hipStreamNonBlocking) != hipSuccess) return bail(MDBG_E_DEVICE);
     if (hipEventCreate(&c->ev0) != hipSuccess || hipEventCreate(&c->ev1) != hipSuccess) return bail(MDBG_E_DEVICE);
     c->bound = make_hash_bound(p->density);
+    { const char* e = getenv("MDBG_NO_DIRECT_STORE"); c->direct_store = !(e && *e && strcmp(e, "0") != 0); }
     if (c->d_t4.ensure((2 << (2 * BS_GS)) * 8, 0, c->stream) != hipSuccess) return bail(MDBG_E_NOMEM);
     { u64 t4[2 << (2 * BS_GS)]; bs_make_table<BS_GS>(t4); if (hipMemcpy(c->d_t4.p, t4, sizeof t4, hipMemcpyHostToDevice) != hipSuccess) return bail(MDBG_E_DEVICE); }
     if (c->scalars.ensure(SC_N * 8, 0, c->stream) != hipSuccess) return bail(MDBG_E_NOMEM);
diff --git a/rust_mdbg_amd/csrc/ingest_api.inc b/rust_mdbg_amd/csrc/ingest_api.inc
--- a/rust_mdbg_amd/csrc/ingest_api.inc
+++ b/rust_mdbg_amd/csrc/ingest_api.inc
@@ -48,7 +48,12 @@
         std::vector<u64> part_end;
         for (u64 t0 = 0; t0 < n_tiles_total; t0 += chunk) part_end.push_back(std::min<u64>(n_tiles_total, t0 + chunk));
         u64 max_part = 0; { u64 t0 = 0; for (u64 e : part_end) { max_part = std::max(max_part, e - t0); t0 = e; } }
-        if (n_tiles_total) {
+        static const bool stop_hook = getenv("MDBG_STOP_PHASE") != nullptr;
+        const bool direct = c->direct_store && !c->direct_off && !sync && n_tiles_total && part_end.size() == 1 && (c->bound >> (64 - BS_B)) <= 1 && c->P.l <= (u32)BS_MAX_L && !(c->P.flags & 1u) &&
+                            !phase_dbg && !stop_hook && !cap0_hook;
+        const u64 lb_words = n_tiles_total + (u64)LB_SHARDS * LB_TICKET_STRIDE / 2;
+        if (n_tiles_total && direct) HIPCHK(c, c->lb.ensure((size_t)lb_words * 8, 0, s));
+        else if (n_tiles_total) {
             HIPCHK(c, c->slab.ensure((size_t)chunk * slab_cap * sizeof(Rec), 0, s));
             HIPCHK(c, c->tile_base.ensure((size_t)max_part * 8, 0, s));
             HIPCHK(c, c->scan_tmp.ensure(((size_t)max_part / 1024 + 2) * 8, 0, s));
@@ -82,9 +87,16 @@
             { const char* sp = getenv("MDBG_STOP_PHASE"); A.stop_phase = sp ? (u32)atoi(sp) : 0u; }
             if (phase_dbg) { HIPCHK(c, c->phase_dbg.ensure((size_t)n_tiles_total * 128, 0, s)); HIPCHK(c, hipMemsetAsync(c->phase_dbg.p, 0, (size_t)n_tiles_total * 128, s)); A.dbg = c->phase_dbg.as<u64>(); }
             const u32 n_gran = (u32)((max_part + SCAN_GRAN - 1) / SCAN_GRAN);
-            HIPCHK(c, c->gran_sum.ensure((size_t)n_gran * 8 + 64, 0, s));
-            A.block_sum = (unsigned long long*)c->gran_sum.as<u64>();
-            init0.zero_arr = c->gran_sum.as<u64>(); init0.zero_arr_n = n_gran;
+            if (direct) {
+                A.slab = nullptr; A.slab_cap = 0xFFFFFFFFu; A.n_scan = nullptr; A.last_read = nullptr; A.block_sum = nullptr;
+                A.lb_status = c->lb.as<u64>(); A.lb_ticket = (u32*)(c->lb.as<u64>() + n_tiles_total);
+                A.out_hash = c->mh.as<u64>(); A.out_pos = c->mpos.as<u32>(); A.out_read = c->mread.as<u32>(); A.out_cap = c->mcap; A.m0 = c->M; A.carry = scal(c) + SC_CARRY;
+                init0.zero_arr = c->lb.as<u64>(); init0.zero_arr_n = (u32)lb_words;
+            } else {
+                HIPCHK(c, c->gran_sum.ensure((size_t)n_gran * 8 + 64, 0, s));
+                A.block_sum = (unsigned long long*)c->gran_sum.as<u64>();
+                init0.zero_arr = c->gran_sum.as<u64>(); init0.zero_arr_n = n_gran;
+            }
             launch_bread(d_offsets, (u32)n_reads, n_bases, A.n_tiles, c->bread.as<u32>(), c->tile_recs.as<TileRec>(), init0, s);
             if (in.n_exc) {
                 HIPCHK(c, hipMemsetAsync(c->tile_flags.p, 0, n_tiles_total, s));
@@ -102,7 +114,15 @@
                 Rec* const part_slab = c->slab.as<Rec>();
                 A.tile0 = (u32)t0; A.slab = part_slab;
                 if (pi) HIPCHK(c, hipMemsetAsync(c->gran_sum.p, 0, (size_t)n_gran * 8, s));
-                { hipEvent_t tb = next_tile_event(c), te = next_tile_event(c); launch_sketch(A, nt, s, tb, te); }
+                { hipEvent_t tb = next_tile_event(c), te = next_tile_event(c); launch_sketch(A, nt, s, tb, te, direct); }
+                if (direct) {
+                    ReadOffsetsArgs R{};
+                    R.mread = c->mread.as<u32>(); R.m0 = c->M; R.m1 = scal(c) + SC_CARRY; R.cap = c->mcap; R.slot0 = slot0; R.n_reads = (u32)n_reads; R.off = c->roff.as<u64>();
+                    launch_read_offsets(R, c->mcap - c->M, s);
+                    c->n_tile_launches += 1;
+                    t0 = part_end[pi];
+                    continue;
+                }
                 GatherArgs G{};
                 G.tile0 = (u32)t0; G.n = nt; G.slab = part_slab; G.slab_cap = slab_cap; G.n_valid = A.n_valid; G.n_scan = A.n_scan; G.last_read = A.last_read;
                 G.out_hash = c->mh.as<u64>(); G.out_pos = c->mpos.as<u32>(); G.out_read = c->mread.as<u32>(); G.out_cap = c->mcap;
@@ -147,7 +167,8 @@
         u64 m_new = sc[SC_CARRY];
         const u32 over = (u32)sc[SC_OVERMAX];
         if (over || m_new > c->mcap) {
-            if (over) { slab_cap = std::min<u32>((u32)tile_bases, (over + over / 8 + 15u) & ~7u); c->slab_cap_min = slab_cap; }
+            if (over && direct) { c->direct_off = true; c->n_direct_retries += 1; }
+            else if (over) { slab_cap = std::min<u32>((u32)tile_bases, (over + over / 8 + 15u) & ~7u); c->slab_cap_min = slab_cap; }
             if (m_new > c->mcap) want = m_new + 65536;
             c->n_tile_launches -= part_end.size(); c->n_tile_bases -= n_tiles_total ? n_bases : 0;
             continue;
@@ -165,6 +186,7 @@
             }
         }
         const u64 slow_total = sc[SC_SLOWTOTAL];
+        if (direct && slow_total > 8) c->direct_off = true;
         if (c->lmer_on && m_new > c->M) {
             const u32 nb = lmer_filter_blocks(m_new - c->M);
             HIPCHK(c, c->slab.ensure((size_t)nb * 256 * sizeof(Rec), 0, s));
@@ -185,6 +207,7 @@
             m_new = sc[SC_CARRY];
         }
         Batch b; b.first_ordinal = first_ordinal; b.n_reads = (u32)n_reads; b.slot0 = slot0; b.m0 = c->M; b.m1 = m_new; b.n_bases = n_bases;
+        c->direct_last = direct;
         invalidate_results(c, FROM_UNITIGS);
         if (c->P.flags & MDBG_FLAG_KEEP_READS) { int ke = keep_batch(c, in, d_offsets, n_reads, n_bases, b.kept); if (ke) return ke; }
         store_append(c, b);
@@ -665,6 +688,7 @@
     o->ms_sketch = c->ms_sketch; o->ms_insert = c->ms_insert; o->ms_finalize = c->ms_finalize;
     o->ms_sketch_tile = c->ms_tile; o->n_sketch_tile_launches = c->n_tile_launches; o->n_sketch_tile_bases = c->n_tile_bases;
     o->tile_bases = TILE_STRIDE;
+    o->direct_store_last = c->direct_last ? 1u : 0u; o->n_direct_retries = c->n_direct_retries;
     if (c->link_ctr.p) {
         (void)hipSetDevice(c->dev);
         HIPCHK(c, hipStreamSynchronize(c->stream));
diff --git a/rust_mdbg_amd/csrc/lookback.h b/rust_mdbg_amd/csrc/lookback.h
--- /dev/null
+++ b/rust_mdbg_amd/csrc/lookback.h
@@ -0,0 +1,52 @@
+#pragma once
+#include <stdint.h>
+
+#if defined(__HIPCC__)
+#define LB_HD __host__ __device__ __forceinline__
+#else
+#define LB_HD inline
+#endif
+
+typedef uint32_t lb_u32;
+typedef uint64_t lb_u64;
+
+constexpr int LB_WIDTH = 64;
+enum : lb_u32 { LB_EMPTY = 0, LB_AGGREGATE = 1, LB_INCLUSIVE = 2, LB_POISON = 3 };
+constexpr int LB_STATE_SHIFT = 62;
+constexpr lb_u64 LB_VALUE_MASK = (1ull << LB_STATE_SHIFT) - 1;
+
+LB_HD lb_u64 lb_pack(lb_u32 state, lb_u64 value) { return (lb_u64)state << LB_STATE_SHIFT | (value & LB_VALUE_MASK); }
+LB_HD lb_u32 lb_state(lb_u64 w) { return (lb_u32)(w >> LB_STATE_SHIFT); }
+LB_HD lb_u64 lb_value(lb_u64 w) { return w & LB_VALUE_MASK; }
+
+LB_HD lb_u64 lb_publish_word(bool have_base, lb_u64 base, lb_u64 count) { return have_base ? lb_pack(LB_INCLUSIVE, base + count) : lb_pack(LB_AGGREGATE, count); }
+
+enum : int { LB_WAIT = 0, LB_DONE = 1, LB_MORE = 2, LB_FAIL = 3 };
+LB_HD int lb_decide(lb_u64 empty, lb_u64 inclusive, lb_u64 poison, lb_u64 valid, lb_u64& take) {
+    const lb_u64 first_inc = inclusive & valid & (0ull - (inclusive & valid));
+    const lb_u64 needed = (first_inc ? (first_inc - 1ull) | first_inc : ~0ull) & valid;
+    take = 0;
+    if (poison & needed) return LB_FAIL;
+    if (empty & needed) return LB_WAIT;
+    take = needed;
+    return first_inc ? LB_DONE : LB_MORE;
+}
+
+constexpr lb_u32 LB_MAX_POLLS = 1u << 20;
+constexpr int LB_POLL_SLEEP = 8;
+
+struct LbWalk {
+    int64_t first;
+    lb_u64 prefix;
+    lb_u32 polls;
+};
+LB_HD void lb_walk_begin(LbWalk& w, lb_u64 tile) { w.first = (int64_t)tile - 1; w.prefix = 0; w.polls = 0; }
+LB_HD lb_u64 lb_valid_mask(const LbWalk& w) { return w.first + 1 >= LB_WIDTH ? ~0ull : (1ull << (w.first + 1)) - 1ull; }
+LB_HD int lb_walk_step(LbWalk& w, int verdict, lb_u64 sum, lb_u32 max_polls = LB_MAX_POLLS) {
+    if (verdict == LB_FAIL) return LB_FAIL;
+    if (verdict == LB_WAIT) return ++w.polls >= max_polls ? LB_FAIL : LB_WAIT;
+    w.prefix += sum;
+    if (verdict == LB_DONE) return LB_DONE;
+    w.first -= LB_WIDTH;
+    return w.first < 0 ? LB_DONE : LB_MORE;
+}
diff --git a/rust_mdbg_amd/csrc/sketch.hip b/rust_mdbg_amd/csrc/sketch.hip
--- a/rust_mdbg_amd/csrc/sketch.hip
+++ b/rust_mdbg_amd/csrc/sketch.hip
@@ -1,5 +1,6 @@
 #include "mdbg_dev.h"
 #include "bs_core.h"
+#include "lookback.h"
 
 enum { FMT_ASCII = 0, FMT_PLANES = 1 };
 constexpr int SCAN_GRAN_LOG = 6, SCAN_GRAN = 1 << SCAN_GRAN_LOG;
@@ -31,6 +32,11 @@
     u32 force_slow;
     u64* dbg;
     u32 stop_phase;
+    u64* lb_status;
+    u32* lb_ticket;
+    u64* out_hash; u32* out_pos; u32* out_read; u64 out_cap;
+    u64 m0;
+    u64* carry;
 };
 
 __device__ inline u32 find_read(const u64* __restrict__ off, u32 lo, u32 hi, u64 p) {
@@ -216,7 +222,56 @@
     if (n > a.slab_cap) atomicMax(a.over_max, n);
 }
 
-template <bool HPC, class Src>
+constexpr u32 LB_SHARDS = 64, LB_TICKET_STRIDE = 32;
+constexpr u32 LB_MISC = 24;
+__device__ inline void lb_store(u64* p, u64 w) { __hip_atomic_store(p, w, __ATOMIC_RELAXED, __HIP_MEMORY_SCOPE_AGENT); }
+__device__ inline void put_rec_direct(const SketchArgs& a, u64 idx, u64 hash, u32 pos, u32 read) {
+    if (idx < a.out_cap) { a.out_hash[idx] = hash; a.out_pos[idx] = pos; a.out_read[idx] = read; }
+}
+__device__ inline bool lb_resolve_wave(const u64* status, u32 tile, int lane, u64& prefix) {
+    LbWalk w; lb_walk_begin(w, tile);
+    for (;;) {
+        const int64_t t = w.first - lane;
+        const u64 word = t >= 0 ? __hip_atomic_load(status + t, __ATOMIC_RELAXED, __HIP_MEMORY_SCOPE_AGENT) : 0ull;
+        const u32 st = lb_state(word);
+        u64 take;
+        const int verdict = lb_decide(__ballot(st == LB_EMPTY), __ballot(st == LB_INCLUSIVE), __ballot(st == LB_POISON), lb_valid_mask(w), take);
+        u64 sum = 0;
+        if (verdict == LB_DONE || verdict == LB_MORE) {
+            sum = (take >> lane) & 1ull ? lb_value(word) : 0ull;
+            for (int d = 32; d; d >>= 1) sum += __shfl_xor(sum, d, 64);
+        }
+        const int r = lb_walk_step(w, verdict, sum);
+        if (r == LB_DONE) { prefix = w.prefix; return true; }
+        if (r == LB_FAIL) return false;
+        if (r == LB_WAIT) __builtin_amdgcn_s_sleep(LB_POLL_SLEEP);
+    }
+}
+__device__ inline void direct_give_up(const SketchArgs& a, u32 gt) { lb_store(a.lb_status + gt, lb_pack(LB_POISON, 0)); atomicMax(a.over_max, 1u); }
+__device__ inline bool direct_prefix(const SketchArgs& a, u32 gt, u32* misc, bool count_known, u32 n, u64& base) {
+    const int lane = threadIdx.x & 63;
+    if (threadIdx.x < 64) {
+        bool ok = true; u64 b = 0;
+        if (gt) {
+            if (count_known && lane == 0) lb_store(a.lb_status + gt, lb_publish_word(false, 0, n));
+            ok = lb_resolve_wave(a.lb_status, gt, lane, b);
+        }
+        if (lane == 0) {
+            if (!ok) direct_give_up(a, gt);
+            else if (count_known) { lb_store(a.lb_status + gt, lb_publish_word(true, b, n)); if (gt + 1 == a.n_tiles) *a.carry = a.m0 + b + n; }
+            misc[LB_MISC] = (u32)b; misc[LB_MISC + 1] = (u32)(b >> 32); misc[LB_MISC + 2] = ok ? 1u : 0u;
+        }
+    }
+    __syncthreads();
+    base = a.m0 + ((u64)misc[LB_MISC] | (u64)misc[LB_MISC + 1] << 32);
+    return misc[LB_MISC + 2] != 0u;
+}
+__device__ inline void direct_publish_late(const SketchArgs& a, u32 gt, u64 base, u32 n) {
+    lb_store(a.lb_status + gt, lb_publish_word(true, base - a.m0, n));
+    if (gt + 1 == a.n_tiles) *a.carry = base + n;
+}
+
+template <bool HPC, bool DIRECT, class Src>
 __device__ void slow_tile(const SketchArgs& a, const Src& src, u32 gt, Rec* slab, TileLds& S) {
     constexpr int TT = TILE_THREADS;
     const int tid = threadIdx.x % TT;
@@ -226,6 +281,8 @@
     const u64 first_base = a.offsets[0];
     u32* tmp = S.misc;
     if (tid == 0) atomicAdd(a.slow_total, 1ull);
+    u64 dbase = 0;
+    if constexpr (DIRECT) { if (!direct_prefix(a, gt, S.misc, false, 0u, dbase)) return; }
     u32 running = 0;
     for (u64 p0 = t_lo; p0 < t_hi; p0 += TT) {
         const u64 p = p0 + tid;
@@ -239,10 +296,10 @@
         }
         u32 total;
         const u32 rank = tile_excl_scan(sel, tmp, total);
-        if (sel) put_rec(a, slab, running + rank, hash, (u32)(start - rlo), r + a.read_base);
+        if (sel) { if constexpr (DIRECT) put_rec_direct(a, dbase + running + rank, hash, (u32)(start - rlo), r + a.read_base); else put_rec(a, slab, running + rank, hash, (u32)(start - rlo), r + a.read_base); }
         running += total;
     }
-    if (tid == 0) put_count(a, gt, running);
+    if (tid == 0) { put_count(a, gt, running); if constexpr (DIRECT) direct_publish_late(a, gt, dbase, running); }
 }
 
 constexpr int SYNC_KEEP = 8;
@@ -380,8 +437,9 @@
 struct CandOut { u64 hash; u32 pos, read; };
 
 #define MDBG_HOT(cond, value) (cond)
-template <int L, int SCHEME = 0, int WMAX = 1>
+template <int L, int SCHEME = 0, int WMAX = 1, bool DIRECT = false>
 __global__ __launch_bounds__(TILE_THREADS, SCHEME ? 5 : 6) void sketch_bs_kernel(SketchArgs a) {
+    static_assert(!DIRECT || SCHEME == 0, "the direct store belongs to the density scheme");
     constexpr int TT = TILE_THREADS, RW = TILE_RAW_WORDS, HW = TILE_HW, QCAP = TILE_QCAP, RS_CAP = TILE_RS_CAP, STAGE_AT = TILE_STAGE_AT;
     __shared__ TileLdsS<SCHEME> S;
     __shared__ __attribute__((aligned(16))) u64 S_t3[T3_WORDS];
@@ -392,8 +450,17 @@
     const int64_t n_pairs = (nb + 31) >> 5;
     const bool hpc = MDBG_HOT(a.hpc != 0, true);
     typedef u32 u32x4 __attribute__((ext_vector_type(4)));
-    const u32 wg = blockIdx.x, gt = a.tile0 + wg;
-    Rec* const slab = a.slab + (size_t)wg * a.slab_cap;
+    u32 wg = blockIdx.x;
+    if constexpr (DIRECT) {
+        __shared__ u32 s_ticket;
+        const u32 shard = blockIdx.x & (LB_SHARDS - 1u);
+        if (tid == 0) s_ticket = atomicAdd(a.lb_ticket + shard * LB_TICKET_STRIDE, 1u);
+        __syncthreads();
+        wg = (u32)__builtin_amdgcn_readfirstlane((int)(shard + LB_SHARDS * s_ticket));
+        if (wg >= a.n_tiles) { if (tid == 0) atomicMax(a.over_max, 1u); return; }
+    }
+    const u32 gt = a.tile0 + wg;
+    Rec* const slab = DIRECT ? nullptr : a.slab + (size_t)wg * a.slab_cap;
 #define MDBG_STAMP(i) do { if (a.dbg && tid == 0) a.dbg[(size_t)gt * 16 + (i)] = __builtin_readcyclecounter(); } while (0)
     MDBG_STAMP(0);
     const int64_t raw0 = (int64_t)gt * TILE_STRIDE - TILE_HALO;
@@ -560,8 +627,8 @@
     const bool true_start = raw0 <= first_base;
     auto run_slow_tile = [&]() {
         if constexpr (SCHEME == 0) {
-            if (a.fmt == FMT_ASCII) { AsciiSrc src{a.bases}; if (hpc) slow_tile<true>(a, src, gt, slab, S); else slow_tile<false>(a, src, gt, slab, S); }
-            else { PlaneSrc src{a.planes, a.exc_pos, a.exc_val, a.tile_flags && a.tile_flags[gt] ? a.n_exc : 0u}; if (hpc) slow_tile<true>(a, src, gt, slab, S); else slow_tile<false>(a, src, gt, slab, S); }
+            if (a.fmt == FMT_ASCII) { AsciiSrc src{a.bases}; if (hpc) slow_tile<true, DIRECT>(a, src, gt, slab, S); else slow_tile<false, DIRECT>(a, src, gt, slab, S); }
+            else { PlaneSrc src{a.planes, a.exc_pos, a.exc_val, a.tile_flags && a.tile_flags[gt] ? a.n_exc : 0u}; if (hpc) slow_tile<true, DIRECT>(a, src, gt, slab, S); else slow_tile<false, DIRECT>(a, src, gt, slab, S); }
         } else {
             if (a.fmt == FMT_ASCII) { AsciiSrc src{a.bases}; if (hpc) sync_slow_tile<true>(a, src, gt, slab, (u32(*)[SYNC_SLOW_THREADS])&S, sync_tmp); else sync_slow_tile<false>(a, src, gt, slab, (u32(*)[SYNC_SLOW_THREADS])&S, sync_tmp); }
             else { PlaneSrc src{a.planes, a.exc_pos, a.exc_val, a.tile_flags && a.tile_flags[gt] ? a.n_exc : 0u}; if (hpc) sync_slow_tile<true>(a, src, gt, slab, (u32(*)[SYNC_SLOW_THREADS])&S, sync_tmp); else sync_slow_tile<false>(a, src, gt, slab, (u32(*)[SYNC_SLOW_THREADS])&S, sync_tmp); }
@@ -984,6 +1051,13 @@
         const u32 left = count_words();
         MDBG_STAMP(5);
         if (MDBG_HOT(a.stop_phase == 5, false)) return 0u;
+        if constexpr (DIRECT) {
+            u64 dbase;
+            if (!direct_prefix(a, gt, S.misc, true, left, dbase)) return left;
+#pragma unroll
+            for (int i = 0; i < NR; ++i) if ((keep_ok >> i) & 1u) put_rec_direct(a, dbase + rank_of(keep_e[i]), keep[i].hash, keep[i].pos, keep[i].read);
+            return left;
+        }
 #pragma unroll
         for (int i = 0; i < NR; ++i) if ((keep_ok >> i) & 1u) {
             const u32 rank = rank_of(keep_e[i]);
@@ -996,8 +1070,10 @@
     const u32 n_cand = S.misc[17];
     if (MDBG_HOT(n_cand <= QCAP, true)) {
         const u32 nv = n_cand ? process_list(n_cand) : 0;
+        if constexpr (DIRECT) { if (!n_cand) { u64 dbase; (void)direct_prefix(a, gt, S.misc, true, 0u, dbase); } }
         if (tid == 0) { put_count(a, gt, nv, true); if (a.dbg) { a.dbg[(size_t)gt * 16 + 9] = n_cand; a.dbg[(size_t)gt * 16 + 10] = nv; } }
     } else {
+        if constexpr (DIRECT) { if (tid == 0) direct_give_up(a, gt); return; }
         __syncthreads();
         if constexpr (SCHEME == 1) {
             {
@@ -1270,6 +1346,26 @@
     }
 }
 
+struct ReadOffsetsArgs { const u32* mread; u64 m0; const u64* m1; u64 cap; u32 slot0, n_reads; u64* off; };
+__global__ __launch_bounds__(256) void read_offsets_kernel(ReadOffsetsArgs g) {
+    u64 m1 = *g.m1; if (m1 > g.cap) m1 = g.cap; if (m1 < g.m0) m1 = g.m0;
+    const u64 stride = (u64)gridDim.x * 256u, t = (u64)blockIdx.x * 256u + threadIdx.x;
+    const int64_t lo = (int64_t)g.slot0 - 1, hi = (int64_t)g.slot0 + g.n_reads;
+    for (u64 i = g.m0 + t; i < m1; i += stride) {
+        int64_t cur = (int64_t)g.mread[i], prev = i == g.m0 ? lo : (int64_t)g.mread[i - 1];
+        if (prev < lo) prev = lo;
+        if (cur > hi) cur = hi;
+        for (int64_t x = prev + 1; x <= cur; ++x) g.off[x] = i;
+    }
+    int64_t last = m1 > g.m0 ? (int64_t)g.mread[m1 - 1] : lo;
+    if (last < lo) last = lo;
+    for (int64_t x = last + 1 + (int64_t)t; x <= hi; x += (int64_t)stride) g.off[x] = m1;
+}
+void launch_read_offsets(const ReadOffsetsArgs& g, u64 room, hipStream_t s) {
+    const u64 nb = (room + 255) / 256;
+    hipLaunchKernelGGL(read_offsets_kernel, dim3((unsigned)(nb < 1 ? 1 : nb > 16384 ? 16384 : nb)), dim3(256), 0, s, g);
+}
+
 template <class Src>
 __global__ __launch_bounds__(256) void alphabet_rule_kernel(Src src, const u64* __restrict__ off, u32 n_reads, u32 l, u32 hpc,
                                                             unsigned long long* __restrict__ which) {
@@ -1329,7 +1425,7 @@
 }
 
 void launch_bread(const u64* offsets, u32 n_reads, u64 n_bases, u32 n_tiles, u32* bread, TileRec* recs, const SketchInit& init, hipStream_t s) {
-    const u32 n = n_tiles + 2;
+    const u32 n = n_tiles + 2 > init.zero_arr_n ? n_tiles + 2 : init.zero_arr_n;
     hipLaunchKernelGGL(tile_rec_kernel, dim3((n + 255) / 256), dim3(256), 0, s, offsets, n_reads, n_bases, n_tiles, bread, recs, init, (int64_t)TILE_STRIDE, (int64_t)TILE_HALO);
 }
 void launch_tile_flags(const u64* exc_pos, u32 n_exc, u32 n_tiles, u8* flags, hipStream_t s) {
@@ -1342,7 +1438,7 @@
     else hipLaunchKernelGGL(alphabet_rule_kernel<PlaneSrc>, g, b, 0, s, PlaneSrc{a.planes, a.exc_pos, a.exc_val, a.n_exc}, a.offsets, a.n_reads, a.l, a.hpc, which);
 }
 
-void launch_sketch(SketchArgs a, u32 n_tiles, hipStream_t s, hipEvent_t ev_begin, hipEvent_t ev_end) {
+void launch_sketch(SketchArgs a, u32 n_tiles, hipStream_t s, hipEvent_t ev_begin, hipEvent_t ev_end, bool direct = false) {
     if (!n_tiles) return;
     a.tile_end = a.tile0 + n_tiles;
     if (ev_begin) (void)hipEventRecord(ev_begin, s);
@@ -1354,6 +1450,14 @@
 #undef MDBG_W
             default: hipLaunchKernelGGL((sketch_bs_kernel<0, 1, 32>), dim3(n_tiles), dim3(TILE_THREADS), 0, s, a); break;
         }
+    }
+    else if (direct) switch (a.l) {
+#define MDBG_L(n) case n: hipLaunchKernelGGL((sketch_bs_kernel<n, 0, 1, true>), dim3(n_tiles), dim3(TILE_THREADS), 0, s, a); break;
+        MDBG_L(2) MDBG_L(3) MDBG_L(4) MDBG_L(5) MDBG_L(6) MDBG_L(7) MDBG_L(8) MDBG_L(9) MDBG_L(10) MDBG_L(11) MDBG_L(12) MDBG_L(13)
+        MDBG_L(14) MDBG_L(15) MDBG_L(16) MDBG_L(17) MDBG_L(18) MDBG_L(19) MDBG_L(20) MDBG_L(21) MDBG_L(22) MDBG_L(23) MDBG_L(24)
+        MDBG_L(25) MDBG_L(26) MDBG_L(27) MDBG_L(28) MDBG_L(29) MDBG_L(30) MDBG_L(31) MDBG_L(32)
+#undef MDBG_L
+        default: hipLaunchKernelGGL((sketch_bs_kernel<32, 0, 1, true>), dim3(n_tiles), dim3(TILE_THREADS), 0, s, a); break;
     }
     else switch (a.l) {
 #define MDBG_L(n) case n: hipLaunchKernelGGL((sketch_bs_kernel<n>), dim3(n_tiles), dim3(TILE_THREADS), 0, s, a); break;
diff --git a/rust_mdbg_amd/csrc/store.inc b/rust_mdbg_amd/csrc/store.inc
--- a/rust_mdbg_amd/csrc/store.inc
+++ b/rust_mdbg_amd/csrc/store.inc
@@ -20,12 +20,12 @@
 void store_append(mdbg_ctx* c, const Batch& b) { c->batches.push_back(b); c->n_slots = b.slot0 + b.n_reads; c->slot_end_m = b.m1; c->M = std::max(c->M, b.m1); }
 u64 store_reserve_region(mdbg_ctx* c, u64 n) { const u64 region = c->M; c->M += n; c->pending_m += n; return region; }
 void store_commit_region(mdbg_ctx* c, u64 n) { c->pending_m -= n; }
-struct StoreSnapshot { u64 M, slot_end_m; u32 n_slots; size_t n_batches; u64 n_reads, n_bases, n_tiles, n_slow_tiles; double ms_sketch, ms_tile; u64 n_tile_launches, n_tile_bases; };
-StoreSnapshot store_snapshot(const mdbg_ctx* c) { return {c->M, c->slot_end_m, c->n_slots, c->batches.size(), c->n_reads, c->n_bases, c->n_tiles, c->n_slow_tiles, c->ms_sketch, c->ms_tile, c->n_tile_launches, c->n_tile_bases}; }
+struct StoreSnapshot { u64 M, slot_end_m; u32 n_slots; size_t n_batches; u64 n_reads, n_bases, n_tiles, n_slow_tiles; double ms_sketch, ms_tile; u64 n_tile_launches, n_tile_bases; bool direct_last; };
+StoreSnapshot store_snapshot(const mdbg_ctx* c) { return {c->M, c->slot_end_m, c->n_slots, c->batches.size(), c->n_reads, c->n_bases, c->n_tiles, c->n_slow_tiles, c->ms_sketch, c->ms_tile, c->n_tile_launches, c->n_tile_bases, c->direct_last}; }
 void store_restore(mdbg_ctx* c, const StoreSnapshot& s) {
     c->M = s.M; c->n_slots = s.n_slots; c->slot_end_m = s.slot_end_m; c->batches.resize(s.n_batches);
     c->n_reads = s.n_reads; c->n_bases = s.n_bases; c->n_tiles = s.n_tiles; c->n_slow_tiles = s.n_slow_tiles;
-    c->ms_sketch = s.ms_sketch; c->ms_tile = s.ms_tile; c->n_tile_launches = s.n_tile_launches; c->n_tile_bases = s.n_tile_bases;
+    c->ms_sketch = s.ms_sketch; c->ms_tile = s.ms_tile; c->n_tile_launches = s.n_tile_launches; c->n_tile_bases = s.n_tile_bases; c->direct_last = s.direct_last;
 }
 struct StoreRollback { mdbg_ctx* const c; const StoreSnapshot s; explicit StoreRollback(mdbg_ctx* c_) : c(c_), s(store_snapshot(c_)) {} ~StoreRollback() { store_restore(c, s); } };
 void store_truncate(mdbg_ctx* c, size_t n_batches) {
```
